# circletile/smvp-toolkit

Measured on AMD Instinct MI355X. Metric: fp64 CSR SpMV GFLOP/s (2*nnz flop per product; achieved HBM GB/s in roofline), higher is better.
Workload: dtype f64; 1 GPU; memplus.mtx x944 block-diagonal (substitute for the SURVEY 8(d) random model; that model: roofline.frac_sur...; format=csr, kernel=csr_stream_owner<8, 5, false>, nnz=119085600, rows=16763552, exchange=none

## Files before the change

include/smvp_amd.h:

```cpp
#ifndef SMVP_AMD_H
#define SMVP_AMD_H

#include <stddef.h>
#include <stdint.h>
#include <stdio.h>

#ifdef __cplusplus
extern "C" {
#endif

#define SMVP_VERSION_MAJOR 0
#define SMVP_VERSION_MINOR 6
#define SMVP_VERSION_REVISION 4

enum {
    SMVP_OK = 0,
    SMVP_ERR_INVALID = 1,
    SMVP_ERR_NO_DEVICE = 2,
    SMVP_ERR_HIP = 3,
    SMVP_ERR_ALLOC = 4,
    SMVP_ERR_IO = 5,
    SMVP_ERR_UNSUPPORTED = 6,
    SMVP_MM_COULD_NOT_READ_FILE = 11,
    SMVP_MM_PREMATURE_EOF = 12,
    SMVP_MM_NOT_MTX = 13,
    SMVP_MM_NO_HEADER = 14,
    SMVP_MM_UNSUPPORTED_TYPE = 15,
    SMVP_MM_LINE_TOO_LONG = 16,
    SMVP_MM_COULD_NOT_WRITE_FILE = 17
};
const char *smvp_last_error(void);
const char *smvp_version_string(void);
int smvp_set_option(const char *name, int value);
int smvp_get_option(const char *name, int *value);

typedef struct smvp_coo {
    int row;
    int col;
    double val;
} smvp_coo_t;

typedef char smvp_mm_typecode[4];

typedef struct smvp_time_stats {
    double time_total, time_avg, time_stdev, time_min, time_max;
} smvp_time_stats_t;

int smvp_mm_read_banner(FILE *f, smvp_mm_typecode *matcode);
int smvp_mm_read_mtx_crd_size(FILE *f, int *rows, int *cols, int *nnz);
int smvp_mm_read_coo_entries(FILE *f, const smvp_mm_typecode matcode, int nnz, smvp_coo_t *out);
int smvp_mm_read_header_path(const char *path, smvp_mm_typecode *matcode, int *rows, int *cols, int *nnz);
int smvp_mm_read_coo_path(const char *path, smvp_coo_t *out, int capacity,
                          smvp_mm_typecode *matcode, int *rows, int *cols, int *nnz);

int smvp_mm_expanded_count(const smvp_mm_typecode matcode, const smvp_coo_t *coo, int nnz, int *count);
int smvp_mm_expand_symmetric(const smvp_mm_typecode matcode, const smvp_coo_t *coo, int nnz, int rows, int cols,
                             smvp_coo_t *out, int capacity, int *nnz_out);

int smvp_cache_write_csr(const char *cache_path, const char *mtx_path, const smvp_mm_typecode matcode, int flags,
                         int rows, int cols, int nnz, const int *row_ptr, const int *col_ind, const double *val);
int smvp_cache_read_header(const char *cache_path, const char *mtx_path, smvp_mm_typecode *matcode, int *flags,
                           int *rows, int *cols, int *nnz);
int smvp_cache_read_csr(const char *cache_path, int rows, int nnz, int *row_ptr, int *col_ind, double *val);
int smvp_coo_from_csr(int rows, const int *row_ptr, const int *col_ind, const double *val, smvp_coo_t *out);

int smvp_csr_from_coo(const smvp_coo_t *coo, int rows, int nnz,
                      int *row_ptr, int *col_ind, double *val);
int smvp_tjds_from_coo(const smvp_coo_t *coo, int rows, int cols, int nnz,
                       int *perm, int *start_pos, int start_pos_capacity,
                       int *row_ind, double *val,
                       int *num_diag, int *ref_num_tjdiag, int *last_diag_single);

int smvp_csr_from_coo_device(const smvp_coo_t *d_coo, int rows, int cols, int nnz,
                             int *d_row_ptr, int *d_col_ind, double *d_val, void *stream);
int smvp_tjds_from_coo_device(const smvp_coo_t *d_coo, int rows, int cols, int nnz,
                              int *d_perm, int *d_start_pos, int start_pos_capacity,
                              int *d_row_ind, double *d_val,
                              int *num_diag, int *ref_num_tjdiag, int *last_diag_single, void *stream);

int smvp_device_count(int *count);
int smvp_device_info(int device, char *name, size_t name_cap, int *compute_units,
                     size_t *hbm_bytes);

enum {
    SMVP_CSR_KERNEL_AUTO = 0,
    SMVP_CSR_KERNEL_VECTOR = 1,
    SMVP_CSR_KERNEL_STREAM = 2,
    SMVP_CSR_KERNEL_STREAM_CARRY = 3,
    SMVP_CSR_KERNEL_COLSWEEP = 4,
    SMVP_CSR_KERNEL_BINNED = 5
};
enum {
    SMVP_MEM_HOST = 0,
    SMVP_MEM_DEVICE = 1
};

typedef struct smvp_csr smvp_csr_t;
typedef struct smvp_tjds smvp_tjds_t;

int smvp_csr_create(smvp_csr_t **out, int device, int rows, int cols, int nnz,
                    const int *row_ptr, const int *col_ind, const double *val,
                    int mem_kind, const int *host_row_ptr);
int smvp_csr_create_block(smvp_csr_t **out, int device, int rows, int cols, int nnz,
                          const int *row_ptr, const int *col_ind, const double *val,
                          int mem_kind, const int *host_row_ptr, long long first_row);
int smvp_csr_set_kernel(smvp_csr_t *h, int kernel, int param);
int smvp_csr_get_kernel(const smvp_csr_t *h, int *kernel, int *param);
int smvp_csr_gather_spread(smvp_csr_t *h, double *spread);
int smvp_csr_far_share(smvp_csr_t *h, double *share);
int smvp_csr_spmv(smvp_csr_t *h, const double *d_x, double *d_y, void *stream);
int smvp_csr_describe(const smvp_csr_t *h, char *kernel_name, size_t cap, double *alg_bytes);
int smvp_csr_plan_launches(const smvp_csr_t *h, int *launches);
typedef struct smvp_plan_info {
    double matrix_bytes;
    double plan_bytes;
    double build_ms;
} smvp_plan_info_t;
int smvp_csr_plan_info(const smvp_csr_t *h, smvp_plan_info_t *out);
int smvp_csr_spmm(smvp_csr_t *h, int k, const double *d_X, long long ldx, double *d_Y, long long ldy, void *stream);
int smvp_csr_spmm_describe(const smvp_csr_t *h, int k, char *kernel_name, size_t cap, double *alg_bytes, smvp_plan_info_t *plan);
int smvp_csr_create_transposed(smvp_csr_t **out, const smvp_csr_t *h, void *stream);
int smvp_csr_device_arrays(const smvp_csr_t *h, const int **d_row_ptr, const int **d_col_ind, const double **d_val);
void smvp_csr_destroy(smvp_csr_t *h);

int smvp_tjds_create(smvp_tjds_t **out, int device, int rows, int cols, int nnz, int num_diag,
                     const int *perm, const int *start_pos, const int *row_ind,
                     const double *val, int mem_kind);
int smvp_tjds_set_x(smvp_tjds_t *h, const double *d_x, void *stream);
int smvp_tjds_zero_y(smvp_tjds_t *h, double *d_y, void *stream);
int smvp_tjds_spmv(smvp_tjds_t *h, double *d_y, void *stream);
enum {
    SMVP_TJDS_MODE_AUTO = 0,
    SMVP_TJDS_MODE_ATOMIC = 1,
    SMVP_TJDS_MODE_TWO_PHASE = 2,
    SMVP_TJDS_MODE_ROW_GATHER = 3
};
int smvp_tjds_set_mode(smvp_tjds_t *h, int mode);
int smvp_tjds_set_tile(smvp_tjds_t *h, int entries_per_tile);
int smvp_tjds_set_value_cache(smvp_tjds_t *h, int min_tiles);
int smvp_tjds_get_value_cache(const smvp_tjds_t *h, int *min_tiles, long long *cached_entries);
int smvp_tjds_set_ref_quirks(smvp_tjds_t *h, int enable, int ref_num_tjdiag, int last_diag_single);
int smvp_tjds_describe(const smvp_tjds_t *h, char *kernel_name, size_t cap, double *alg_bytes);
int smvp_tjds_plan_info(const smvp_tjds_t *h, smvp_plan_info_t *out);
int smvp_tjds_spmv_transposed(smvp_tjds_t *h, const double *d_x, double *d_y, void *stream);
int smvp_tjds_transposed_describe(const smvp_tjds_t *h, char *kernel_name, size_t cap, double *alg_bytes);
int smvp_tjds_spmm_transposed(smvp_tjds_t *h, int k, const double *d_X, long long ldx, double *d_Y, long long ldy, void *stream);
int smvp_tjds_spmm_transposed_describe(const smvp_tjds_t *h, int k, char *kernel_name, size_t cap, double *alg_bytes);
int smvp_tjds_spmm(smvp_tjds_t *h, int k, const double *d_X, long long ldx, double *d_Y, long long ldy, void *stream);
int smvp_tjds_spmm_describe(const smvp_tjds_t *h, int k, char *kernel_name, size_t cap, double *alg_bytes, smvp_plan_info_t *plan);
void smvp_tjds_destroy(smvp_tjds_t *h);

enum { SMVP_POWER_CONVERGED = 0, SMVP_POWER_MAX_STEPS = 1, SMVP_POWER_ZERO = 2, SMVP_POWER_NONFINITE = 3 };
typedef struct smvp_power_opts {
    unsigned struct_size;
    int max_steps;
    int check_every;
    double tol;
} smvp_power_opts_t;
void smvp_power_opts_default(smvp_power_opts_t *o);
typedef struct smvp_power_result {
    int steps;
    int reason;
    int index;
    double eigenvalue;
    double residual;
    double scale;
} smvp_power_result_t;
int smvp_csr_power_method(smvp_csr_t *h, const smvp_power_opts_t *opts, const double *d_x0, double *d_x,
                          smvp_power_result_t *result, double *lambda_each, double *residual_each, void *stream);
int smvp_tjds_power_method(smvp_tjds_t *h, const smvp_power_opts_t *opts, const double *d_x0, double *d_x,
                           smvp_power_result_t *result, double *lambda_each, double *residual_each, void *stream);

int smvp_vector_dot(int device, int n, const double *d_a, const double *d_b, double *result, void *stream);

enum { SMVP_CG_CONVERGED = 0, SMVP_CG_MAX_STEPS = 1, SMVP_CG_BREAKDOWN = 2, SMVP_CG_NONFINITE = 3 };
typedef struct smvp_cg_opts {
    unsigned struct_size;
    int max_steps;
    int check_every;
    double tol;
} smvp_cg_opts_t;
void smvp_cg_opts_default(smvp_cg_opts_t *o);
typedef struct smvp_cg_result {
    int steps;
    int updates;
    int reason;
    int pad;
    double rr;
    double bb;
} smvp_cg_result_t;
int smvp_csr_cg(smvp_csr_t *h, const smvp_cg_opts_t *opts, const double *d_b, const double *d_x0, double *d_x,
                smvp_cg_result_t *result, double *rr_each, double *sigma_each, void *stream);
int smvp_tjds_cg(smvp_tjds_t *h, const smvp_cg_opts_t *opts, const double *d_b, const double *d_x0, double *d_x,
                 smvp_cg_result_t *result, double *rr_each, double *sigma_each, void *stream);

int smvp_csr_diagonal(const smvp_csr_t *h, double *d_diag, void *stream);
int smvp_tjds_diagonal(const smvp_tjds_t *h, double *d_diag, void *stream);

typedef struct smvp_pcg_result {
    int steps;
    int updates;
    int reason;
    int pad;
    double rr;
    double rz;
    double bb;
} smvp_pcg_result_t;
int smvp_csr_pcg(smvp_csr_t *h, const smvp_cg_opts_t *opts, const double *d_b, const double *d_x0, double *d_x, const double *d_m,
                 smvp_pcg_result_t *result, double *rr_each, double *rz_each, double *sigma_each, void *stream);
int smvp_tjds_pcg(smvp_tjds_t *h, const smvp_cg_opts_t *opts, const double *d_b, const double *d_x0, double *d_x, const double *d_m,
                  smvp_pcg_result_t *result, double *rr_each, double *rz_each, double *sigma_each, void *stream);

int smvp_csr_cg_multi(smvp_csr_t *h, const smvp_cg_opts_t *opts, int k, const double *d_B, long long ldb, const double *d_X0,
                      long long ldx0, double *d_X, long long ldx, const double *d_m, smvp_pcg_result_t *results, double *rr_each,
                      double *rz_each, double *sigma_each, void *stream);
int smvp_tjds_cg_multi(smvp_tjds_t *h, const smvp_cg_opts_t *opts, int k, const double *d_B, long long ldb, const double *d_X0,
                       long long ldx0, double *d_X, long long ldx, const double *d_m, smvp_pcg_result_t *results, double *rr_each,
                       double *rz_each, double *sigma_each, void *stream);

enum { SMVP_TRSV_LOWER = 0, SMVP_TRSV_UPPER = 1 };
enum { SMVP_TRSV_DIAG_STORED = 0, SMVP_TRSV_DIAG_UNIT = 1 };
typedef struct smvp_trsv smvp_trsv_t;
typedef struct smvp_trsv_info {
    unsigned struct_size;
    int levels;
    int max_level_width;
    int launches;
    int chains;
    int chain_width;
    int missing_diagonals;
    int lanes_per_row;
    long long entries;
    double plan_bytes;
    double build_ms;
} smvp_trsv_info_t;
int smvp_csr_trsv_create(smvp_trsv_t **out, const smvp_csr_t *h, int uplo, int diag, void *stream);
int smvp_trsv_solve(smvp_trsv_t *t, const double *d_b, double *d_x, void *stream);
int smvp_trsv_info(const smvp_trsv_t *t, smvp_trsv_info_t *out);
int smvp_trsv_schedule(const smvp_trsv_t *t, int *level_ptr, int *order);
void smvp_trsv_destroy(smvp_trsv_t *t);
int smvp_csr_trsv_levels(int rows, const int *row_ptr, const int *col_ind, int uplo, int *level_of_row, int *levels);

enum { SMVP_TRSV_MAX_SWEEPS = 4096 };
// ... 207 lines not shown
```

smvp-toolkit_amd/csrc/smvp_common.h:

```cpp
#pragma once
#include "smvp_amd.h"

#include <cstdarg>
#include <cstdio>
#include <vector>

namespace smvp {
constexpr long long kMaxEntries = 2147483647ll - 65536;

int fail(int code, const char *fmt, ...) __attribute__((format(printf, 2, 3)));
void clear_error();
int option(const char *name, int fallback);

struct TrsvSchedule {
    std::vector<int> level_of_row, level_ptr, order;
    int levels = 0, max_level_width = 0, missing_diagonals = 0, max_row_entries = 0;
    long long off_entries = 0, diag_entries = 0;
};
struct TrsvLaunch {
    int first, last;
    bool chain;
};
int trsv_analyse(int rows, const int *row_ptr, const int *col_ind, int uplo, TrsvSchedule *out);
void trsv_launches(const std::vector<int> &level_ptr, int chain_width, std::vector<TrsvLaunch> *out, int *chains);
void trsv_ranges(int rows, const int *row_ptr, const int *col_ind, int uplo, int diag, std::vector<int> *begin, std::vector<int> *end,
                 long long *entries, int *longest);

int ilu0_check(const char *fn, int rows, const int *row_ptr, const int *col_ind, int *diag_pos, int *bad_row);

int lsqr_check_args(const char *fn, const void *h, const void *ht, bool needs_ht, const smvp_lsqr_opts_t *opts, const void *result,
                    const double *d_b);
}

struct ihipStream_t;
namespace smvp {
int build_row_inverse(const int *d_row_ind, int nnz, int rows, int *d_inv_ptr, int *d_inv_pos, ihipStream_t *stream);
int build_row_gather_plan(const int *d_row_ind, const int *d_start_pos, int num_diag, int nnz, int rows,
                          int *d_seg_ptr, int *d_pos, int *d_kcol, ihipStream_t *stream);
int build_colsweep_plan(const int *d_row_ptr, const int *d_col_ind, const double *d_val, int rows, int cols, int nnz, int strip_rows,
                        int parts, int chunk, int row_bits, int turn_cap, long long *d_strip_ptr, int *d_e_col, double *d_e_val,
                        unsigned short *d_e_row, ihipStream_t *stream);
int sort_tile_windows(const int *d_pos, int nnz, int tile, const int *d_start_pos, int num_diag, int slot_bits,
                      const double *d_val, int cache_min_tiles, int *d_pos_sorted, int *d_meta, int *d_cache_ptr,
                      double **d_val_cache, int *cached_total, ihipStream_t *stream);
int build_tile_half_streams(const int *d_pos, int nnz, int tile, const int *d_start_pos, int num_diag, const double *d_val,
                            int cache_min_tiles, unsigned *d_word32, int *d_cache_ptr, int *d_run_ptr,
                            double **d_val_cache, int **d_run_tab, unsigned short **d_group_run, int *cached_total,
                            int *runs_total, ihipStream_t *stream);
int build_column_offsets(const int *d_col_ind, int nnz, int tile, int *d_col_base, unsigned short *d_col16, int *fits,
                         ihipStream_t *stream);
int build_tile_overflow(const int *d_pos, const int *d_ovf_ptr, int total, int ntiles, int tile, int nnz,
                        const int *d_start_pos, int num_diag, const double *d_val, double *d_ovf_val, int *d_ovf_k, int positions,
                        ihipStream_t *stream);
}
```

smvp-toolkit_amd/csrc/smvp_convert_device.hip:

```cpp
#include "smvp_common.h"
#include "smvp_prim.h"
#include "smvp_tile_map.h"

#include <hip/hip_runtime.h>

#include <cstring>

#include <algorithm>
#include <vector>

#define HIP_TRY(expr)                                                                       \
    do {                                                                                    \
        hipError_t e_ = (expr);                                                             \
        if (e_ != hipSuccess)                                                               \
            return smvp::fail(SMVP_ERR_HIP, "%s failed: %s", #expr, hipGetErrorString(e_)); \
    } while (0)

namespace {

typedef unsigned long long u64;

struct Scratch {
    std::vector<void *> ptrs;
    ~Scratch()
// ... 800 lines not shown
                                                   unsigned short *__restrict__ e_row)
{
    const int i = blockIdx.x * 256 + threadIdx.x;
    if (i >= nnz)
        return;
    const long long a = strip_ptr[(unsigned)(key[i] >> 32) * (unsigned)parts + (unsigned)(key[i] & 0xffffffffu) / part_width];
    const long long first = a + ((long long)i - a) / chunk * chunk;
    const unsigned short mine = row_sorted[i];
    int turn = 0;
    for (long long q = first; q < i; ++q)
        turn += row_sorted[q] == mine ? 1 : 0;
    e_row[i] = (unsigned short)(mine | ((turn < turn_cap ? turn : turn_cap) << row_bits));
}

__global__ __launch_bounds__(256) void sweep_strip_bounds(const int *__restrict__ row_ptr, int rows, int strip_rows, int nstrips,
                                                          long long *__restrict__ strip_ptr)
{
    const int b = blockIdx.x * 256 + threadIdx.x;
    if (b > nstrips)
        return;
    const long long r = (long long)b * strip_rows;
    strip_ptr[b] = row_ptr[r < rows ? r : rows];
}

__global__ __launch_bounds__(256) void sweep_part_bounds(const u64 *__restrict__ key, const int *__restrict__ row_ptr, int rows, int nnz,
                                                         int strip_rows, int nstrips, int parts, unsigned part_width,
                                                         long long *__restrict__ stream_ptr)
{
    const int v = blockIdx.x * 256 + threadIdx.x;
    if (v > nstrips * parts)
        return;
    if (v == nstrips * parts) {
        stream_ptr[v] = nnz;
        return;
    }
    const int strip = v / parts, part = v % parts;
    const long long r0 = (long long)strip * strip_rows, r1 = r0 + strip_rows;
    long long lo = row_ptr[r0 < rows ? r0 : rows], hi = row_ptr[r1 < rows ? r1 : rows];
    const unsigned first_col = (unsigned)part * part_width;
    while (lo < hi) {
        const long long mid = (lo + hi) >> 1;
        if ((unsigned)(key[mid] & 0xffffffffu) < first_col)
            lo = mid + 1;
        else
            hi = mid;
    }
    stream_ptr[v] = lo;
}

}

namespace smvp {

int build_colsweep_plan(const int *d_row_ptr, const int *d_col_ind, const double *d_val, int rows, int cols, int nnz, int strip_rows,
                        int parts, int chunk, int row_bits, int turn_cap, long long *d_strip_ptr, int *d_e_col, double *d_e_val,
                        unsigned short *d_e_row, hipStream_t st)
{
    if (strip_rows < 1 || strip_rows > (1 << row_bits) || row_bits < 1 || row_bits > 15 || chunk < 64 ||
        turn_cap != (1 << (16 - row_bits)) - 1 || (parts != 1 && parts != 2 && parts != 4 && parts != 8))
        return smvp::fail(SMVP_ERR_INVALID, "build_colsweep_plan: bad strip shape");
    const unsigned part_width = (unsigned)std::max(1, (int)(((long long)std::max(cols, 1) + parts - 1) / parts));
    const int nstrips = (rows + strip_rows - 1) / strip_rows;
    hipLaunchKernelGGL(sweep_strip_bounds, dim3(blocks_for((long long)nstrips + 1)), dim3(256), 0, st, d_row_ptr, rows,
                       strip_rows, nstrips, d_strip_ptr);
    HIP_TRY(hipGetLastError());
    if (nnz > 0) {
        Scratch sc;
        u64 *k0, *k1;
        unsigned *i0, *i1;
        unsigned short *lr, *lr_sorted;
        HIP_TRY(sc.get(&k0, (size_t)nnz));
        HIP_TRY(sc.get(&k1, (size_t)nnz));
        HIP_TRY(sc.get(&i0, (size_t)nnz));
        HIP_TRY(sc.get(&i1, (size_t)nnz));
        HIP_TRY(sc.get(&lr, (size_t)nnz));
        HIP_TRY(sc.get(&lr_sorted, (size_t)nnz));
        hipLaunchKernelGGL(sweep_keys, dim3(blocks_for(nnz)), dim3(256), 0, st, d_row_ptr, d_col_ind, rows, nnz, strip_rows, k0, i0, lr);
        HIP_TRY(hipGetLastError());
        const unsigned bits = 32u + (unsigned)bits_for(nstrips + 1);
        size_t tmp_bytes = 0;
        HIP_TRY(smvp::prim::radix_sort_pairs(nullptr, tmp_bytes, k0, k1, i0, i1, (size_t)nnz, 0u, bits, st));
        char *tmp;
        HIP_TRY(sc.get(&tmp, tmp_bytes));
        HIP_TRY(smvp::prim::radix_sort_pairs(tmp, tmp_bytes, k0, k1, i0, i1, (size_t)nnz, 0u, bits, st));
        hipLaunchKernelGGL(sweep_gather, dim3(blocks_for(nnz)), dim3(256), 0, st, k1, i1, d_val, lr, nnz, d_e_col, d_e_val, lr_sorted);
        HIP_TRY(hipGetLastError());
        if (parts > 1) {
            hipLaunchKernelGGL(sweep_part_bounds, dim3(blocks_for((long long)nstrips * parts + 1)), dim3(256), 0, st, k1, d_row_ptr, rows, nnz,
                               strip_rows, nstrips, parts, part_width, d_strip_ptr);
            HIP_TRY(hipGetLastError());
        }
        hipLaunchKernelGGL(sweep_turns, dim3(blocks_for(nnz)), dim3(256), 0, st, k1, d_strip_ptr, lr_sorted, nnz, chunk, row_bits,
                           turn_cap, parts, part_width, d_e_row);
        HIP_TRY(hipGetLastError());
        HIP_TRY(hipStreamSynchronize(st));
    } else if (parts > 1) {
        HIP_TRY(hipMemsetAsync(d_strip_ptr, 0, sizeof(long long) * ((size_t)nstrips * parts + 1), st));
    }
    HIP_TRY(hipStreamSynchronize(st));
    return SMVP_OK;
}

}

namespace {

__global__ __launch_bounds__(256) void tile_column_spans(const int *__restrict__ col_ind, int nnz, int tile,
                                                         int *__restrict__ col_base, int *__restrict__ narrow)
{
    __shared__ int lo_s[4], hi_s[4];
    const long long s = (long long)blockIdx.x * tile;
    int lo = 0x7fffffff, hi = -1;
    for (int i = threadIdx.x; i < tile && s + i < nnz; i += 256) {
        const int c = col_ind[s + i];
        lo = c < lo ? c : lo;
        hi = c > hi ? c : hi;
    }
#pragma unroll
    for (int off = 32; off > 0; off >>= 1) {
        const int ol = __shfl_down(lo, off, 64), oh = __shfl_down(hi, off, 64);
        lo = ol < lo ? ol : lo;
        hi = oh > hi ? oh : hi;
    }
    if ((threadIdx.x & 63) == 0) {
        lo_s[threadIdx.x >> 6] = lo;
        hi_s[threadIdx.x >> 6] = hi;
    }
    __syncthreads();
    if (threadIdx.x == 0) {
        for (int w = 1; w < 4; ++w) {
            lo = lo_s[w] < lo ? lo_s[w] : lo;
            hi = hi_s[w] > hi ? hi_s[w] : hi;
        }
        const bool fits = hi < 0 || hi - lo < 65536;
        col_base[blockIdx.x] = !fits ? -1 : (hi < 0 ? 0 : lo);
        if (fits)
            atomicAdd(narrow, 1);
    }
}

__global__ __launch_bounds__(256) void column_offsets(const int *__restrict__ col_ind, int nnz, int tile,
                                                      const int *__restrict__ col_base, unsigned short *__restrict__ col16)
{
    const int j = blockIdx.x * 256 + threadIdx.x;
    if (j < nnz) {
        const int b = j / tile, s = b * tile;
        const int base = col_base[b];
        const bool lane_order = tile == smvp::kCol16LaneOrderTile && base >= 0 && (long long)s + tile <= (long long)nnz;
        const int at = lane_order ? s + smvp::col16_slot(j - s, tile / 256) : j;
        col16[at] = base < 0 ? (unsigned short)0 : (unsigned short)(col_ind[j] - base);
    }
}

}

namespace smvp {

int build_column_offsets(const int *d_col_ind, int nnz, int tile, int *d_col_base, unsigned short *d_col16, int *fits,
                         hipStream_t st)
{
    *fits = 0;
    if (nnz <= 0)
        return SMVP_OK;
    const int ntiles = (int)(((long long)nnz + tile - 1) / tile);
    Scratch sc;
    int *narrow;
    HIP_TRY(sc.get(&narrow, 1));
    HIP_TRY(hipMemsetAsync(narrow, 0, sizeof(int), st));
    hipLaunchKernelGGL(tile_column_spans, dim3((unsigned)ntiles), dim3(256), 0, st, d_col_ind, nnz, tile, d_col_base, narrow);
    HIP_TRY(hipGetLastError());
    int h_narrow = 0;
    HIP_TRY(hipMemcpyAsync(&h_narrow, narrow, sizeof(int), hipMemcpyDeviceToHost, st));
    HIP_TRY(hipStreamSynchronize(st));
    if (2 * (long long)h_narrow < (long long)ntiles)
        return SMVP_OK;
    hipLaunchKernelGGL(column_offsets, dim3(blocks_for(nnz)), dim3(256), 0, st, d_col_ind, nnz, tile, d_col_base, d_col16);
    HIP_TRY(hipGetLastError());
    HIP_TRY(hipStreamSynchronize(st));
    *fits = 1;
    return SMVP_OK;
}

}
```

smvp-toolkit_amd/csrc/smvp_engine.hip:

```cpp
#include "smvp_engine.h"

#include <cmath>
#include <cstring>

using smvp::check_block_operands;
using smvp::check_device_indices;
using smvp::DeviceScope;
using smvp::kMaxEntries;
using smvp::refuse_capture;
using smvp::TjdsSource;
using smvp::to_device;
using smvp::upload;
using smvp::usable_device;
using smvp::wall_ms;

int smvp::usable_device(int device)
{
    int n = 0;
    if (hipGetDeviceCount(&n) != hipSuccess || n <= 0)
        return smvp::fail(SMVP_ERR_NO_DEVICE, "no HIP device is visible (this engine has no CPU path)");
    if (device < 0 || device >= n)
        return smvp::fail(SMVP_ERR_INVALID, "device %d out of range (%d visible)", device, n);
    return SMVP_OK;
}


struct TilePlan {
    int ntiles = 0;
    int *d_tile_row = nullptr;
    int *d_tile_next = nullptr;
    unsigned short *d_col16 = nullptr;
    int *d_col_base = nullptr;
    int col16_tile = 0;
    unsigned short *d_row_rel = nullptr;
    int *d_carry_row = nullptr;
    double *d_carry = nullptr;
    int *d_pos_sorted = nullptr, *d_meta = nullptr, *d_ovf_ptr = nullptr, *d_ovf_k = nullptr;
    double *d_ovf_val = nullptr;
    int *d_cache_ptr = nullptr;
    double *d_val_cache = nullptr;
    int cached_total = 0, ovf_total = 0;
    unsigned short *d_group_run = nullptr;
    unsigned *d_word32 = nullptr;
    int *d_run_ptr = nullptr, *d_run_tab = nullptr;
    int runs_total = 0;
    int sweep_alternate = 1, sweep_backward = 0;
    int read_once = 0;
};

struct SweepPlan {
    int rb = 0, per_launch = 0;
    int parts = 1;
    int g = 0;
    long long *d_ptr = nullptr;
    int *d_col = nullptr;
    double *d_val = nullptr;
    unsigned short *d_row = nullptr;
    double *d_part = nullptr;
};

struct BinnedSide {
    smvp::BinnedPlan bin;
    smvp_csr *near = nullptr;
    hipStream_t side = nullptr;
    hipEvent_t ev_fork = nullptr, ev_join = nullptr;
};

struct SpmmPlan {
    int *d_order = nullptr;
    bool planned = false;
    double build_ms = 0.0;
};

struct smvp_csr {
    int device = 0;
    int rows = 0, cols = 0, nnz = 0;
    long long row0 = 0;
    int *d_row_ptr = nullptr;
    int *d_col_ind = nullptr;
    double *d_val = nullptr;
    bool own_row_ptr = false, own_col_ind = false, own_val = false;
    std::vector<int> h_row_ptr;
    int max_row_len = 0;

    int flavor = smvp::kFlavorCsr;
    TjdsSource src;
    int cache_min_tiles = 2;
    bool plain_only = false;

    int kernel = SMVP_CSR_KERNEL_AUTO;
    int lanes_per_row = 64;
    int vpt = 4;
    bool tile_chosen = false;
    double spread = -2.0;
    double far_share = -2.0;
    double plan_build_ms = 0.0;

    TilePlan tile;
    SweepPlan sweep;
    BinnedSide binned;
    SpmmPlan spmm;
};

namespace {

void free_tile_plan(TilePlan *p)
{
    for (void *q : {(void *)p->d_tile_row, (void *)p->d_tile_next, (void *)p->d_col16, (void *)p->d_col_base, (void *)p->d_row_rel,
                    (void *)p->d_carry_row, (void *)p->d_carry, (void *)p->d_pos_sorted, (void *)p->d_meta, (void *)p->d_ovf_ptr,
                    (void *)p->d_ovf_k, (void *)p->d_ovf_val, (void *)p->d_cache_ptr, (void *)p->d_val_cache, (void *)p->d_group_run,
                    (void *)p->d_word32, (void *)p->d_run_ptr, (void *)p->d_run_tab})
        if (q)
            (void)hipFree(q);
    *p = TilePlan{};
}

void free_sweep_plan(SweepPlan *p)
{
    for (void *q : {(void *)p->d_ptr, (void *)p->d_col, (void *)p->d_val, (void *)p->d_row, (void *)p->d_part})
        if (q)
            (void)hipFree(q);
    *p = SweepPlan{};
}

void free_binned_side(BinnedSide *p)
{
    smvp_csr_destroy(p->near);
    smvp::free_binned_plan(&p->bin);
    if (p->side)
        (void)hipStreamDestroy(p->side);
    for (hipEvent_t e : {p->ev_fork, p->ev_join})
        if (e)
            (void)hipEventDestroy(e);
    *p = BinnedSide{};
}

void free_spmm_plan(SpmmPlan *p)
{
    if (p->d_order)
        (void)hipFree(p->d_order);
    *p = SpmmPlan{};
}

inline bool tile_ordered(int flavor) { return flavor == smvp::kFlavorTjdsS || flavor == smvp::kFlavorTjdsH; }
inline bool runs_on_tile_plan(int k) { return k != SMVP_CSR_KERNEL_VECTOR && k != SMVP_CSR_KERNEL_COLSWEEP && k != SMVP_CSR_KERNEL_BINNED; }
inline int owner_flavor(const smvp_csr *h) { return h->tile.d_col16 ? smvp::kFlavorCsr16 : h->flavor; }
inline double csr_matrix_bytes(const smvp_csr *h) { return 12.0 * h->nnz + 4.0 * (h->rows + 1.0); }
inline int sweep_strip_rows(const SweepPlan &s) { return (s.parts == smvp::kSweepXcdParts ? s.rb : s.rb * s.parts) / smvp::kSweepWaves; }

constexpr int kSweepMaxRb = 20480;
double sweep_rate(int rb)
{
    const struct { double lg, rate; } pts[] = {{10.0, 0.70}, {11.0, 0.80}, {12.0, 0.86}, {13.0, 1.0}, {14.32, 1.10}};
    constexpr int N = (int)(sizeof pts / sizeof pts[0]);
    const double lg = std::log2((double)std::max(rb, 1));
    if (lg <= pts[0].lg)
        return pts[0].rate * std::max(0.25, lg / pts[0].lg);
    for (int i = 0; i + 1 < N; ++i)
        if (lg <= pts[i + 1].lg)
            return pts[i].rate + (pts[i + 1].rate - pts[i].rate) * (lg - pts[i].lg) / (pts[i + 1].lg - pts[i].lg);
    return pts[N - 1].rate;
}

void choose_sweep_shape(int rows, int cols, int nnz, int want_rb, int *rb, int *per_launch)
{
    const double mean = rows > 0 ? std::max(1.0, (double)nnz / rows) : 1.0;
    int floor_rb = 1024;
    while (floor_rb < 8192 && (double)floor_rb * mean * 160.0 < (double)cols)
        floor_rb <<= 1;
    auto generations = [](int nrb) { return (nrb + 255) / 256; };
    std::vector<int> heights;
    for (int hgt : {kSweepMaxRb, 16384, 8192, 4096, 2048, 1024})
        if (hgt >= floor_rb)
            heights.push_back(hgt);
    for (int g = 1; g <= 16 && rows > 0; ++g) {
        const long long want = ((long long)rows + 256ll * g - 1) / (256ll * g);
        const int h4 = (int)std::min<long long>(kSweepMaxRb, (want + 3) / 4 * 4);
        if (h4 >= std::max(1024, floor_rb / 2))
            heights.push_back(h4);
    }
    int r = floor_rb;
    double best = -1.0;
    int best_gen = 1 << 30;
    for (int hgt : heights) {
        const int nrb = (rows + hgt - 1) / hgt;
        const int gen = std::max(1, generations(nrb));
        const double score = (double)nrb / (gen * 256.0) * sweep_rate(hgt);
        if (score > best * 1.01 || (score > best * 0.99 && gen < best_gen)) {
            best = std::max(best, score);
            best_gen = gen;
            r = hgt;
        }
    }
    if (want_rb > 0)
        r = want_rb;
    const int nrb = (rows + r - 1) / r;
    const int gen = std::max(1, generations(nrb));
    *rb = r;
    *per_launch = std::max(1, (nrb + gen - 1) / gen);
}

constexpr int kSweepPartsShift = 24, kSweepChunksShift = 26;
inline int sweep_param_rb(int param) { return param & ((1 << kSweepPartsShift) - 1); }
inline int sweep_param_parts(int param) { return 1 << ((param >> kSweepPartsShift) & 3); }
inline int sweep_param_chunks(int param) { const int c = (param >> kSweepChunksShift) & 3; return c == 3 ? 4 : c; }
bool sweep_param_ok(int param)
{
    const int rb = sweep_param_rb(param), parts = sweep_param_parts(param);
    if (param < 0 || (param >> (kSweepChunksShift + 2)) != 0)
        return false;
    if (rb == 0)
        return true;
    if (parts == smvp::kSweepXcdParts)
        return rb >= 256 && rb % 4 == 0 && rb <= kSweepMaxRb;
    return rb >= 256 && rb % 4 == 0 && (long long)rb * parts <= kSweepMaxRb;
}

int build_sweep_plan(smvp_csr *h, int want)
{
    SweepPlan &s = h->sweep;
    free_sweep_plan(&s);
    const int want_rb = sweep_param_rb(want);
    s.parts = sweep_param_parts(want);
    const bool xcd = s.parts == smvp::kSweepXcdParts;
    if (xcd) {
        int rb = want_rb;
        if (rb == 0) {
            const long long per_gen_max = 32ll * kSweepMaxRb;
            const long long gens = std::max<long long>(1, ((long long)h->rows + per_gen_max - 1) / per_gen_max);
            rb = (int)std::min<long long>(kSweepMaxRb, std::max<long long>(256, (((long long)h->rows + 32 * gens - 1) / (32 * gens) + 3) / 4 * 4));
        }
        s.rb = rb;
        s.per_launch = 256;
    } else {
        choose_sweep_shape(h->rows, h->cols, h->nnz, want_rb, &s.rb, &s.per_launch);
        while (s.parts > 1 && (long long)s.rb * s.parts > kSweepMaxRb)
            s.parts >>= 1;
    }
    const int strip_rows = sweep_strip_rows(s);
    s.g = smvp::sweep_chunks_in_flight(strip_rows, sweep_param_chunks(want));
    if (const hipError_t pe = smvp::prepare_csr_colsweep(); pe != hipSuccess)
        return smvp::fail(SMVP_ERR_HIP, "the column sweep cannot have its LDS: %s", hipGetErrorString(pe));
    const int nstrips = (h->rows + strip_rows - 1) / strip_rows;
    const size_t n = (size_t)std::max(h->nnz, 4);
    if (hipMalloc((void **)&s.d_ptr, ((size_t)nstrips * s.parts + 2) * sizeof(long long)) != hipSuccess ||
        hipMalloc((void **)&s.d_col, n * sizeof(int)) != hipSuccess ||
        hipMalloc((void **)&s.d_val, n * sizeof(double)) != hipSuccess ||
        hipMalloc((void **)&s.d_row, n * sizeof(unsigned short)) != hipSuccess ||
        (xcd && hipMalloc((void **)&s.d_part, sizeof(double) * smvp::kSweepXcdParts * (size_t)std::max(h->rows, 1)) != hipSuccess))
        return smvp::fail(SMVP_ERR_ALLOC, "cannot allocate the column-sweep plan (%d entries)", h->nnz);
    return smvp::build_colsweep_plan(h->d_row_ptr, h->d_col_ind, h->d_val, h->rows, h->cols, h->nnz, strip_rows, s.parts, smvp::kSweepChunk,
                                     smvp::kSweepRowBits, smvp::kSweepTurnCap, s.d_ptr, s.d_col, s.d_val, s.d_row, nullptr);
}

constexpr int kSpreadSamples = 64;
double csr_gather_spread(const smvp_csr *h)
{
    if ((long long)h->nnz < (long long)kSpreadSamples * smvp::kSpreadSpan || !h->d_col_ind)
        return -1.0;
    int *d_bits = nullptr;
    if (hipMalloc((void **)&d_bits, sizeof(int) * kSpreadSamples) != hipSuccess)
        return -1.0;
    int bits[kSpreadSamples];
    hipError_t e = smvp::launch_csr_line_spread(h->d_col_ind, h->nnz, kSpreadSamples, d_bits, nullptr);
    if (e == hipSuccess)
        e = hipMemcpy(bits, d_bits, sizeof bits, hipMemcpyDeviceToHost);
    (void)hipFree(d_bits);
    if (e != hipSuccess) {
        (void)hipGetLastError();
        return -1.0;
    }
    const double m = 512.0 * 1024.0;
    double lines = 0.0;
    for (int b : bits)
        lines += -m * std::log(std::max(1.0 - b / m, 1.0 / m));
    return std::min(1.0, lines / ((double)kSpreadSamples * smvp::kSpreadSpan));
}

constexpr double kSweepMinSpread = 0.6;

double measured_spread(smvp_csr *h)
{
    if (h->spread < -1.5)
        h->spread = h->flavor == smvp::kFlavorCsr ? csr_gather_spread(h) : -1.0;
    return h->spread;
}

double measured_far_share(smvp_csr *h)
{
    if (h->far_share < -1.5) {
        double share = -1.0;
        if (h->flavor != smvp::kFlavorCsr ||
            smvp::csr_far_share(h->d_row_ptr, h->d_col_ind, h->rows, h->nnz, smvp::kBinNearBand, h->row0, &share, nullptr) != SMVP_OK) {
            (void)hipGetLastError();
            share = -1.0;
        }
        h->far_share = share;
    }
    return h->far_share;
}

bool sweep_suits(smvp_csr *h)
{
    if (h->plain_only || h->flavor != smvp::kFlavorCsr || h->nnz < 4 * 1024 * 1024 || h->rows < 4096)
        return false;
    const double mean = (double)h->nnz / h->rows;
    if (mean < 4.0 || (double)h->cols * 8.0 < 8.0 * 1024 * 1024 || 8192.0 * mean * 160.0 < (double)h->cols ||
        (double)h->max_row_len > 256.0 * mean)
        return false;
    return measured_spread(h) >= kSweepMinSpread;
}

constexpr double kBinnedMinSpread = 0.2, kBinnedMinFarShare = 0.1;
bool binned_suits(smvp_csr *h)
{
    if (h->plain_only || h->flavor != smvp::kFlavorCsr || h->nnz < 4 * 1024 * 1024 || h->rows < 4096 ||
        (double)h->cols * 8.0 < 16.0 * 1024 * 1024)
        return false;
    return measured_spread(h) >= kBinnedMinSpread && measured_far_share(h) >= kBinnedMinFarShare;
}

int try_column_offsets(smvp_csr *h)
{
    if (h->flavor != smvp::kFlavorCsr || h->kernel != SMVP_CSR_KERNEL_STREAM || h->vpt < 4 || h->nnz <= 0 ||
        smvp::option("csr_col16", 1) == 0)
        return SMVP_OK;
    std::vector<int> tiles;
    if (!h->tile_chosen && h->nnz >= 12 * 1024 * 1024)
        tiles.push_back(2048);
    tiles.push_back(smvp::kStreamBlock * h->vpt);
    const size_t max_tiles = ((size_t)h->nnz + 1023) / 1024 + 1;
    int *col_base = nullptr;
    unsigned short *col16 = nullptr;
    int rc = SMVP_OK;
    if (hipMalloc((void **)&col_base, max_tiles * sizeof(int)) != hipSuccess ||
        hipMalloc((void **)&col16, ((size_t)h->nnz + 8) * sizeof(unsigned short)) != hipSuccess)
        rc = smvp::fail(SMVP_ERR_ALLOC, "cannot allocate the 16-bit column offsets (%d entries)", h->nnz);
    for (size_t i = 0; i < tiles.size() && rc == SMVP_OK; ++i) {
        int fits = 0;
        rc = smvp::build_column_offsets(h->d_col_ind, h->nnz, tiles[i], col_base, col16, &fits, nullptr);
        if (rc == SMVP_OK && fits) {
            h->vpt = tiles[i] / smvp::kStreamBlock;
            h->tile.d_col_base = col_base;
            h->tile.d_col16 = col16;
            h->tile.col16_tile = tiles[i];
            return SMVP_OK;
        }
    }
    (void)hipGetLastError();
    for (void *p : {(void *)col16, (void *)col_base})
        if (p)
            (void)hipFree(p);
    return rc;
}

constexpr double kSweepAlternateMinBytes = 256.0 * 1024 * 1024;

constexpr double kReadOnceMinBytes = 1024.0 * 1024 * 1024;

int build_tile_plan_parts(smvp_csr *h)
{
    TilePlan &t = h->tile;
    free_tile_plan(&t);
    if (int rc = try_column_offsets(h))
        return rc;
    const int tile = smvp::kStreamBlock * h->vpt;
    const long long nnz = h->nnz;
    const int ntiles = (int)std::max<long long>(1, (nnz + tile - 1) / tile);
    std::vector<int> tile_row((size_t)ntiles + 1), carry_row((size_t)ntiles), tile_next((size_t)ntiles);
    const int *rp = h->h_row_ptr.data();
    int r = 0;
    for (int b = 0; b < ntiles; ++b) {
        const long long s = (long long)b * tile;
        const long long e = std::min(s + tile, nnz);
        while (r < h->rows && rp[r] < s)
            ++r;
        tile_row[(size_t)b] = r;
        const long long first = r < h->rows ? rp[r] : nnz;
        carry_row[(size_t)b] = (std::min(first, e) > s) ? r - 1 : -1;
    }
    tile_row[(size_t)ntiles] = h->rows;
    for (int b = 0; b < ntiles; ++b)
        tile_next[(size_t)b] = rp[tile_row[(size_t)b + 1]];
    if (int rc = upload(&t.d_tile_row, tile_row))
        return rc;
    if (h->kernel == SMVP_CSR_KERNEL_STREAM) {
        if (int rc = upload(&t.d_tile_next, tile_next))
            return rc;
        if (h->rows > 0 && smvp::option("csr_rowrel", 1) != 0) {
            std::vector<unsigned short> rel((size_t)h->rows);
            for (int b = 0; b < ntiles; ++b) {
                const long long s0 = (long long)b * tile;
                for (int rr = tile_row[(size_t)b]; rr < tile_row[(size_t)b + 1]; ++rr)
                    rel[(size_t)rr] = (unsigned short)(rp[rr] - s0);
            }
            if (int rc = upload(&t.d_row_rel, rel))
                return rc;
        }
    } else {
        if (int rc = upload(&t.d_carry_row, carry_row))
            return rc;
        HIP_TRY(hipMalloc((void **)&t.d_carry, std::max(ntiles, 1) * sizeof(double)));
        HIP_TRY(hipMemset(t.d_carry, 0, std::max(ntiles, 1) * sizeof(double)));
    }
    t.ntiles = ntiles;
    const int alternate = smvp::option("csr_sweep_alternate", -1);
    const double product_bytes = 12.0 * (double)h->nnz + 12.0 * h->rows + 8.0 * h->cols;
    t.sweep_alternate = alternate < 0 ? product_bytes > kSweepAlternateMinBytes : alternate != 0;
    const int read_once = smvp::option("csr_read_once", -1);
    t.read_once = h->flavor != smvp::kFlavorCsr ? 0 : read_once < 0 ? product_bytes > kReadOnceMinBytes : read_once != 0;
    if (tile_ordered(h->flavor)) {
        std::vector<int> ovf_ptr((size_t)ntiles + 1, 0);
        for (int b = 0; b < ntiles; ++b) {
            const long long e = std::min((long long)(b + 1) * tile, nnz);
            const bool owns = tile_row[(size_t)b] != tile_row[(size_t)b + 1];
            ovf_ptr[(size_t)b + 1] = ovf_ptr[(size_t)b] + (owns ? (int)(tile_next[(size_t)b] - e) : 0);
        }
        const int total = ovf_ptr[(size_t)ntiles];
        t.ovf_total = total;
        if (int rc = upload(&t.d_ovf_ptr, ovf_ptr))
            return rc;
        const size_t n = (size_t)std::max(h->nnz, 4), m = (size_t)std::max(total, 4);
        const bool half = h->flavor == smvp::kFlavorTjdsH;
        const TjdsSource &src = h->src;
        if (hipMalloc((void **)&t.d_ovf_val, m * sizeof(double)) != hipSuccess ||
            hipMalloc((void **)&t.d_ovf_k, m * sizeof(int)) != hipSuccess ||
            hipMalloc((void **)&t.d_cache_ptr, ((size_t)ntiles + 2) * sizeof(int)) != hipSuccess ||
            hipMalloc(half ? (void **)&t.d_word32 : (void **)&t.d_pos_sorted, n * sizeof(int)) != hipSuccess ||
            hipMalloc(half ? (void **)&t.d_run_ptr : (void **)&t.d_meta, (half ? (size_t)ntiles + 2 : n) * sizeof(int)) != hipSuccess)
            return smvp::fail(SMVP_ERR_ALLOC, "cannot allocate the tile-ordered TJDS streams");
        if (int rc = half ? smvp::build_tile_half_streams(src.pos, h->nnz, tile, src.start_pos, src.num_diag, h->d_val, h->cache_min_tiles,
                                                          t.d_word32, t.d_cache_ptr, t.d_run_ptr, &t.d_val_cache, &t.d_run_tab,
                                                          &t.d_group_run, &t.cached_total, &t.runs_total, nullptr)
                          : smvp::sort_tile_windows(src.pos, h->nnz, tile, src.start_pos, src.num_diag, smvp::kSlotBits, h->d_val,
                                                    h->cache_min_tiles, t.d_pos_sorted, t.d_meta, t.d_cache_ptr, &t.d_val_cache,
                                                    &t.cached_total, nullptr))
            return rc;
        if (int rc = smvp::build_tile_overflow(src.pos, t.d_ovf_ptr, total, ntiles, tile, h->nnz, src.start_pos, src.num_diag, h->d_val,
                                               t.d_ovf_val, t.d_ovf_k, src.unit_operand ? 1 : 0, nullptr))
            return rc;
    }
    return SMVP_OK;
}

int build_tile_plan(smvp_csr *h)
{
    const int rc = build_tile_plan_parts(h);
    if (rc != SMVP_OK)
        free_tile_plan(&h->tile);
    return rc;
}

int pow2_at_least(double v)
{
    int p = 2;
    while (p < 64 && p < v)
        p <<= 1;
    return p;
}

constexpr int kOwnerMaxRow = 16 * 1024;

bool choose_csr_kernel(smvp_csr *h, int kernel, int param)
{
    const double mean = h->rows > 0 ? (double)h->nnz / h->rows : 0.0;
    if (kernel == SMVP_CSR_KERNEL_AUTO)
        kernel = h->max_row_len > kOwnerMaxRow ? SMVP_CSR_KERNEL_STREAM_CARRY
                 : sweep_suits(h)              ? SMVP_CSR_KERNEL_COLSWEEP
                 : binned_suits(h)             ? SMVP_CSR_KERNEL_BINNED
                                               : SMVP_CSR_KERNEL_STREAM;
    if (kernel == SMVP_CSR_KERNEL_STREAM && param != 0 && param != 256 && param != 1024 && param != 2048)
        return false;
    if (kernel == SMVP_CSR_KERNEL_STREAM_CARRY && param != 0 && param != 1024 && param != 2048)
        return false;
    if (kernel == SMVP_CSR_KERNEL_COLSWEEP && !sweep_param_ok(param))
        return false;
    if (kernel == SMVP_CSR_KERNEL_BINNED && param < 0)
        return false;
    h->kernel = kernel;
    if (kernel == SMVP_CSR_KERNEL_COLSWEEP || kernel == SMVP_CSR_KERNEL_BINNED)
        return true;
    if (kernel == SMVP_CSR_KERNEL_VECTOR) {
        h->lanes_per_row = param > 0 ? param : pow2_at_least(mean);
    } else {
        int tile = param > 0 ? param : 0;
        h->tile_chosen = param > 0;
        if (tile == 0) {
            tile = (kernel == SMVP_CSR_KERNEL_STREAM && h->nnz < 512 * 1024) ? 256 : 1024;
            if ((tile_ordered(h->flavor)) && tile == 1024 && h->nnz >= 12 * 1024 * 1024)
                tile = 2048;
        }
        h->vpt = tile / smvp::kStreamBlock;
    }
    return true;
}

}

static int csr_create_impl(smvp_csr_t **out, int device, int rows, int cols, int nnz, const int *row_ptr, const int *col_ind, const double *val,
                           int mem_kind, const int *host_row_ptr, int flavor, const TjdsSource *src = nullptr, bool plain_only = false,
                           long long first_row = 0);

static int build_binned(smvp_csr *h, int band)
{
    free_binned_side(&h->binned);
    if (hipError_t le = smvp::binned_reserve_lds(); le != hipSuccess) {
        (void)hipGetLastError();
        return smvp::fail(SMVP_ERR_UNSUPPORTED, "the binned plan needs 154 KB of LDS per workgroup: %s", hipGetErrorString(le));
    }
    const bool window = smvp::option("binned_near", 0) == 0;
    if (int rc = smvp::build_binned_plan(h->d_row_ptr, h->d_col_ind, h->d_val, h->rows, h->cols, h->nnz, band, h->row0, window, &h->binned.bin, nullptr))
        return rc;
    if (h->binned.bin.nw.on) {
        if (smvp::option("binned_overlap", 1) != 0 && h->binned.bin.nf > 0) {
            HIP_TRY(hipStreamCreateWithFlags(&h->binned.side, hipStreamNonBlocking));
            HIP_TRY(hipEventCreateWithFlags(&h->binned.ev_fork, hipEventDisableTiming));
            HIP_TRY(hipEventCreateWithFlags(&h->binned.ev_join, hipEventDisableTiming));
        }
        return SMVP_OK;
    }
    return csr_create_impl(&h->binned.near, h->device, h->rows, h->cols, h->binned.bin.nnz_near, h->binned.bin.near_ptr, h->binned.bin.near_col, h->binned.bin.near_val,
                           SMVP_MEM_DEVICE, nullptr, smvp::kFlavorCsr, nullptr, true, h->row0);
}

static int plan_csr(smvp_csr *h, int kernel, int param, bool silent_fallback)
{
    if (!choose_csr_kernel(h, kernel, param))
        return smvp::fail(SMVP_ERR_INVALID, "entries per tile must be 256 (stream only), 1024 or 2048 for the kernel "
                                            "this matrix resolves to (column sweep: 256 ... 20480 rows per block, a multiple of 4; binned: the near band, >= 0)");
    const double t0 = wall_ms();
    free_sweep_plan(&h->sweep);
    free_binned_side(&h->binned);
    int rc = SMVP_OK;
    if (runs_on_tile_plan(h->kernel)) {
        rc = build_tile_plan(h);
    } else {
        free_tile_plan(&h->tile);
        if (h->kernel != SMVP_CSR_KERNEL_VECTOR)
            rc = h->kernel == SMVP_CSR_KERNEL_COLSWEEP ? build_sweep_plan(h, param) : build_binned(h, param);
        if (rc != SMVP_OK) {
            const std::string why = smvp_last_error();
            (void)hipGetLastError();
            free_sweep_plan(&h->sweep);
            free_binned_side(&h->binned);
            h->spread = -1.0;
            choose_csr_kernel(h, SMVP_CSR_KERNEL_STREAM, 0);
            const int tile_rc = build_tile_plan(h);
            rc = silent_fallback ? tile_rc : smvp::fail(rc, "%s", why.c_str());
        }
    }
    h->plan_build_ms = wall_ms() - t0;
    return rc;
}

static int csr_create_impl(smvp_csr_t **out, int device, int rows, int cols, int nnz, const int *row_ptr, const int *col_ind, const double *val,
                           int mem_kind, const int *host_row_ptr, int flavor, const TjdsSource *src, bool plain_only, long long first_row)
{
    const bool plain = flavor == smvp::kFlavorCsr;
    if (!out || rows < 0 || cols < 0 || nnz < 0 || !row_ptr ||
        (nnz > 0 && ((!col_ind && !tile_ordered(flavor)) || !val)))
        return smvp::fail(SMVP_ERR_INVALID, "smvp_csr_create: bad argument");
    if (mem_kind != SMVP_MEM_HOST && mem_kind != SMVP_MEM_DEVICE)
        return smvp::fail(SMVP_ERR_INVALID, "smvp_csr_create: bad mem_kind");
    if (nnz > kMaxEntries)
        return smvp::fail(SMVP_ERR_UNSUPPORTED, "smvp_csr_create: %d entries: shard blocks this large by rows", nnz);
    if (int rc = usable_device(device))
        return rc;
    DeviceScope on(device);

    smvp_csr *h = new smvp_csr;
    h->device = device;
    h->flavor = flavor;
    h->plain_only = plain_only;
    h->row0 = first_row;
    if (src)
        h->src = *src;
    if (h->src.unit_operand)
        h->cache_min_tiles = 0;
    h->rows = rows, h->cols = cols, h->nnz = nnz;
    h->h_row_ptr.resize((size_t)rows + 1);
    int rc = SMVP_OK;
    if (mem_kind == SMVP_MEM_HOST || host_row_ptr) {
        memcpy(h->h_row_ptr.data(), mem_kind == SMVP_MEM_HOST ? row_ptr : host_row_ptr, sizeof(int) * ((size_t)rows + 1));
    } else if (hipMemcpy(h->h_row_ptr.data(), row_ptr, sizeof(int) * ((size_t)rows + 1), hipMemcpyDeviceToHost) != hipSuccess) {
        rc = smvp::fail(SMVP_ERR_HIP, "smvp_csr_create: cannot read row_ptr back from the device");
    }
    if (rc == SMVP_OK) {
        const std::vector<int> &rp = h->h_row_ptr;
        bool ok = rp[0] == 0 && rp[(size_t)rows] == nnz;
        for (int r = 0; r < rows && ok; ++r) {
            ok = rp[(size_t)r] <= rp[(size_t)r + 1];
            h->max_row_len = std::max(h->max_row_len, rp[(size_t)r + 1] - rp[(size_t)r]);
        }
        if (!ok)
            rc = smvp::fail(SMVP_ERR_INVALID, "smvp_csr_create: row_ptr is not a non-decreasing 0..nnz sequence");
    }
    if (rc == SMVP_OK && mem_kind == SMVP_MEM_HOST) {
        for (int j = 0; j < nnz; ++j)
            if (col_ind[j] < 0 || col_ind[j] >= cols) {
                rc = smvp::fail(SMVP_ERR_INVALID, "smvp_csr_create: col_ind[%d] = %d outside [0, %d)", j, col_ind[j], cols);
                break;
            }
    }
    if (rc == SMVP_OK && mem_kind == SMVP_MEM_DEVICE &&
        (((uintptr_t)col_ind | (plain ? (uintptr_t)val : 0)) & 15u) != 0)
        rc = smvp::fail(SMVP_ERR_INVALID, "smvp_csr_create: adopted device arrays must be 16-byte aligned");
    if (rc == SMVP_OK && mem_kind == SMVP_MEM_DEVICE && col_ind)
        rc = check_device_indices(col_ind, nnz, cols, "smvp_csr_create: col_ind");
    if (rc == SMVP_OK)
        rc = to_device(&h->d_row_ptr, row_ptr, (size_t)rows + 1, mem_kind, &h->own_row_ptr);
    if (rc == SMVP_OK && col_ind)
        rc = to_device(&h->d_col_ind, col_ind, (size_t)nnz, mem_kind, &h->own_col_ind);
    if (rc == SMVP_OK)
        rc = to_device(&h->d_val, val, (size_t)nnz, mem_kind, &h->own_val);
    if (rc == SMVP_OK) {
        const double t0 = wall_ms();
        rc = plan_csr(h, plain ? SMVP_CSR_KERNEL_AUTO : SMVP_CSR_KERNEL_STREAM, 0, true);
        h->plan_build_ms = wall_ms() - t0;
    }
    if (rc != SMVP_OK) {
        smvp_csr_destroy(h);
        return rc;
    }
    *out = h;
    return SMVP_OK;
}

int smvp::csr_create_tjds(smvp_csr_t **out, int device, int rows, int cols, int nnz, const int *d_row_ptr, const int *d_col_ind,
                          const double *d_val, int flavor, const TjdsSource &src)
{
    return csr_create_impl(out, device, rows, cols, nnz, d_row_ptr, d_col_ind, d_val, SMVP_MEM_DEVICE, nullptr, flavor, &src);
}

bool smvp::csr_value_cache(const smvp_csr_t *h, int *min_tiles, long long *cached_entries)
{
    const bool on = h && tile_ordered(h->flavor);
    if (min_tiles)
        *min_tiles = on ? h->cache_min_tiles : 0;
    if (cached_entries)
        *cached_entries = on ? h->tile.cached_total : 0;
    return on;
}

int smvp::csr_replan_value_cache(smvp_csr_t *h, int min_tiles)
{
    h->cache_min_tiles = min_tiles;
    return build_tile_plan(h);
}

extern "C" int smvp_csr_create(smvp_csr_t **out, int device, int rows, int cols, int nnz,
                               const int *row_ptr, const int *col_ind, const double *val,
                               int mem_kind, const int *host_row_ptr)
{
    return csr_create_impl(out, device, rows, cols, nnz, row_ptr, col_ind, val, mem_kind, host_row_ptr, smvp::kFlavorCsr);
}

extern "C" int smvp_csr_create_block(smvp_csr_t **out, int device, int rows, int cols, int nnz,
                                     const int *row_ptr, const int *col_ind, const double *val,
                                     int mem_kind, const int *host_row_ptr, long long first_row)
{
    if (first_row < 0)
        return smvp::fail(SMVP_ERR_INVALID, "smvp_csr_create_block: first_row < 0");
    return csr_create_impl(out, device, rows, cols, nnz, row_ptr, col_ind, val, mem_kind, host_row_ptr, smvp::kFlavorCsr, nullptr,
                           false, first_row);
}

extern "C" int smvp_csr_far_share(smvp_csr_t *h, double *share)
{
    if (!h || !share)
        return smvp::fail(SMVP_ERR_INVALID, "smvp_csr_far_share: bad argument");
    DeviceScope on(h->device);
    *share = measured_far_share(h);
    return SMVP_OK;
}

extern "C" int smvp_csr_set_kernel(smvp_csr_t *h, int kernel, int param)
{
    if (!h)
        return smvp::fail(SMVP_ERR_INVALID, "null handle");
    if (h->flavor != smvp::kFlavorCsr && kernel != SMVP_CSR_KERNEL_STREAM)
        return smvp::fail(SMVP_ERR_UNSUPPORTED, "this matrix flavour runs on the stream kernel only");
    if (kernel < SMVP_CSR_KERNEL_AUTO || kernel > SMVP_CSR_KERNEL_BINNED)
        return smvp::fail(SMVP_ERR_INVALID, "unknown CSR kernel %d", kernel);
    if (kernel == SMVP_CSR_KERNEL_VECTOR && param != 0 &&
        (param < 2 || param > 64 || (param & (param - 1)) != 0))
        return smvp::fail(SMVP_ERR_INVALID, "lanes per row must be a power of two in [2, 64]");
    DeviceScope on(h->device);
    h->spread = h->far_share = -2.0;
    return plan_csr(h, kernel, param, false);
}

extern "C" int smvp_csr_get_kernel(const smvp_csr_t *h, int *kernel, int *param)
{
    if (!h)
        return smvp::fail(SMVP_ERR_INVALID, "null handle");
    if (kernel)
        *kernel = h->kernel;
    if (param)
        *param = h->kernel == SMVP_CSR_KERNEL_VECTOR ? h->lanes_per_row
                 : h->kernel == SMVP_CSR_KERNEL_COLSWEEP ? (h->sweep.rb | ((h->sweep.parts == 8 ? 3 : h->sweep.parts == 4 ? 2 : h->sweep.parts == 2 ? 1 : 0) << kSweepPartsShift))
                 : h->kernel == SMVP_CSR_KERNEL_BINNED   ? h->binned.bin.band
                                                         : h->vpt * smvp::kStreamBlock;
    return SMVP_OK;
}

extern "C" int smvp_csr_gather_spread(smvp_csr_t *h, double *spread)
{
    if (!h || !spread)
        return smvp::fail(SMVP_ERR_INVALID, "smvp_csr_gather_spread: bad argument");
    DeviceScope on(h->device);
    *spread = measured_spread(h);
    return SMVP_OK;
}

static int fill_owner_launch(const smvp_csr_t *h, const double *d_x, double *d_y, unsigned long long *stamps, smvp::OwnerLaunch *out)
{
    if (h->tile.d_col16 && h->tile.col16_tile != smvp::kStreamBlock * h->vpt)
        return smvp::fail(SMVP_ERR_INVALID, "the 16-bit column offsets were laid out for %d-entry tiles, the launch has %d-entry tiles",
                          h->tile.col16_tile, smvp::kStreamBlock * h->vpt);
    smvp::OwnerLaunch &l = *out;
    l.row_ptr = h->d_row_ptr, l.col_ind = h->d_col_ind, l.val = h->d_val, l.x = d_x, l.y = d_y;
    l.tile_row = h->tile.d_tile_row, l.tile_next = h->tile.d_tile_next;
    l.pos = h->src.pos, l.start_pos = h->src.start_pos;
    if (tile_ordered(h->flavor)) {
        l.pos = h->tile.d_pos_sorted, l.col_ind = h->tile.d_meta;
        l.ovf_ptr = h->tile.d_ovf_ptr, l.ovf_val = h->tile.d_ovf_val, l.ovf_k = h->tile.d_ovf_k;
        l.cache_ptr = h->tile.d_cache_ptr, l.val_cache = h->tile.d_val_cache;
        l.word32 = h->tile.d_word32, l.group_run = h->tile.d_group_run, l.run_ptr = h->tile.d_run_ptr, l.run_tab = h->tile.d_run_tab;
    }
    l.stamps = stamps;
    l.rows = h->rows, l.nnz = h->nnz, l.ntiles = h->tile.ntiles;
    l.col16 = h->tile.d_col16, l.col_base = h->tile.d_col_base;
    l.row_rel = h->tile.d_row_rel;
    l.read_once = h->tile.read_once;
    l.unit_x = h->src.unit_operand ? 1 : 0;
    return SMVP_OK;
}

int smvp::csr_repeat_grid(const smvp_csr_t *h)
{
    if (!h || h->kernel != SMVP_CSR_KERNEL_STREAM || !h->tile.d_tile_row || h->rows <= 0)
        return 0;
    DeviceScope on(h->device);
    return smvp::owner_repeat_grid(h->vpt, owner_flavor(h), h->tile.ntiles);
}

int smvp::csr_spmv_repeat(smvp_csr_t *h, const double *d_x, double *d_y, void *stream, unsigned long long *stamps, int reps, int grid,
                          unsigned *ctl_words, bool first_of_run, unsigned long long patience)
{
    DeviceScope on(h->device);
    smvp::OwnerLaunch l{};
    if (int rc = fill_owner_launch(h, d_x, d_y, stamps, &l))
        return rc;
    const hipError_t e = smvp::launch_csr_stream_owner_repeat(h->vpt, owner_flavor(h), l, reps, grid, ctl_words,
                                                              first_of_run, patience, (hipStream_t)stream);
    if (e != hipSuccess)
        return smvp::fail(SMVP_ERR_HIP, "repeating CSR launch failed: %s", hipGetErrorString(e));
    return SMVP_OK;
}

static int launched(hipError_t e)
{
    return e == hipSuccess ? (int)SMVP_OK : smvp::fail(SMVP_ERR_HIP, "CSR launch failed: %s", hipGetErrorString(e));
}

int smvp::csr_spmv_stamped(smvp_csr_t *h, const double *d_x, double *d_y, void *stream, unsigned long long *stamps)
{
    if (!h || (h->rows > 0 && !d_y) || (h->nnz > 0 && !d_x))
        return smvp::fail(SMVP_ERR_INVALID, "smvp_csr_spmv: bad argument");
    if ((h->kernel == SMVP_CSR_KERNEL_COLSWEEP && !h->sweep.d_ptr) || (h->kernel == SMVP_CSR_KERNEL_BINNED && !h->binned.near && !h->binned.bin.nw.on) ||
        (runs_on_tile_plan(h->kernel) && !h->tile.d_tile_row))
        return smvp::fail(SMVP_ERR_INVALID, "smvp_csr_spmv: the handle has no launch plan (a re-plan failed earlier)");
    DeviceScope on(h->device);
    hipStream_t st = (hipStream_t)stream;
    hipError_t e;
    if (h->kernel == SMVP_CSR_KERNEL_BINNED) {
        if (h->binned.bin.nw.on && h->binned.side) {
            HIP_TRY(hipEventRecord(h->binned.ev_fork, st));
            HIP_TRY(hipStreamWaitEvent(h->binned.side, h->binned.ev_fork, 0));
            if (int rc = launched(smvp::launch_binned_products(h->binned.bin, d_x, h->binned.side)))
                return rc;
            int rc = SMVP_OK;
            hipError_t je = hipEventRecord(h->binned.ev_join, h->binned.side);
            if (je == hipSuccess) {
                rc = launched(smvp::launch_near_window(h->binned.bin.nw, d_x, d_y, st));
                je = hipStreamWaitEvent(st, h->binned.ev_join, 0);
            }
            if (je != hipSuccess) {
                (void)hipStreamSynchronize(h->binned.side);
                return smvp::fail(SMVP_ERR_HIP, "joining the binned plan's side stream failed: %s", hipGetErrorString(je));
            }
            if (rc != SMVP_OK)
                return rc;
            return launched(smvp::launch_binned_sums(h->binned.bin, d_y, st));
        }
        if (h->binned.bin.nw.on) {
            if (int rc = launched(smvp::launch_near_window(h->binned.bin.nw, d_x, d_y, st)))
                return rc;
        } else if (int rc = smvp::csr_spmv_stamped(h->binned.near, d_x, d_y, stream, nullptr))
            return rc;
        if (int rc = launched(smvp::launch_binned_products(h->binned.bin, d_x, st)))
            return rc;
        e = smvp::launch_binned_sums(h->binned.bin, d_y, st);
    } else if (h->kernel == SMVP_CSR_KERNEL_COLSWEEP)
        e = smvp::launch_csr_colsweep(h->sweep.d_ptr, h->sweep.d_col, h->sweep.d_val, h->sweep.d_row, d_x, d_y, h->rows,
                                      sweep_strip_rows(h->sweep), h->sweep.parts, h->sweep.per_launch, h->sweep.g, h->sweep.d_part, st);
    else if (h->kernel == SMVP_CSR_KERNEL_VECTOR)
        e = smvp::launch_csr_vector(h->lanes_per_row, h->d_row_ptr, h->d_col_ind, h->d_val, d_x, d_y, h->rows, st);
    else if (h->kernel == SMVP_CSR_KERNEL_STREAM) {
        smvp::OwnerLaunch l{};
        if (int rc = fill_owner_launch(h, d_x, d_y, stamps, &l))
            return rc;
        l.backward = h->tile.sweep_backward;
        h->tile.sweep_backward = h->tile.sweep_alternate ? !l.backward : 0;
        e = smvp::launch_csr_stream_owner(h->vpt, owner_flavor(h), l, st);
    } else
        e = smvp::launch_csr_stream(h->vpt, h->d_row_ptr, h->d_col_ind, h->d_val, d_x, d_y, h->tile.d_tile_row,
                                    h->tile.d_carry_row, h->tile.d_carry, h->rows, h->nnz, h->tile.ntiles, st);
    return launched(e);
}

extern "C" int smvp_csr_spmv(smvp_csr_t *h, const double *d_x, double *d_y, void *stream)
{
    return smvp::csr_spmv_stamped(h, d_x, d_y, stream, nullptr);
}

static smvp::HandleProduct csr_product(smvp_csr_t *h, void *stream)
{
    return [h, stream](const double *x, double *y) { return smvp_csr_spmv(h, x, y, stream); };
}

static int refuse_tjds_flavor(const char *fn, const smvp_csr_t *h)
{
    if (h->flavor != smvp::kFlavorCsr)
        return smvp::fail(SMVP_ERR_UNSUPPORTED, "%s: plain CSR handles only (this one belongs to a TJDS matrix)", fn);
    return SMVP_OK;
}

extern "C" int smvp_csr_power_method(smvp_csr_t *h, const smvp_power_opts_t *opts, const double *d_x0, double *d_x,
                                     smvp_power_result_t *result, double *lambda_each, double *residual_each, void *stream)
{
    if (int rc = smvp::power_check_args("smvp_csr_power_method", h, opts, result))
        return rc;
    if (int rc = refuse_tjds_flavor("smvp_csr_power_method", h))
        return rc;
    return smvp::power_run("smvp_csr_power_method", h->device, h->rows, h->cols, opts, d_x0, d_x, result, lambda_each, residual_each, stream,
                           csr_product(h, stream));
}

extern "C" int smvp_csr_cg(smvp_csr_t *h, const smvp_cg_opts_t *opts, const double *d_b, const double *d_x0, double *d_x,
                           smvp_cg_result_t *result, double *rr_each, double *sigma_each, void *stream)
{
    if (int rc = smvp::cg_check_args("smvp_csr_cg", h, opts, result, d_b, smvp::Precond::none, {}))
        return rc;
    if (int rc = refuse_tjds_flavor("smvp_csr_cg", h))
        return rc;
    return smvp::cg_run("smvp_csr_cg", h->device, h->rows, h->cols, opts, d_b, d_x0, d_x, result, rr_each, sigma_each, stream,
                        csr_product(h, stream));
}

extern "C" int smvp_csr_pcg(smvp_csr_t *h, const smvp_cg_opts_t *opts, const double *d_b, const double *d_x0, double *d_x,
                            const double *d_m, smvp_pcg_result_t *result, double *rr_each, double *rz_each, double *sigma_each,
                            void *stream)
{
    const smvp::KrylovPrecond M{nullptr, d_m, nullptr};
    if (int rc = smvp::cg_check_args("smvp_csr_pcg", h, opts, result, d_b, smvp::Precond::diagonal, M))
        return rc;
    if (int rc = refuse_tjds_flavor("smvp_csr_pcg", h))
        return rc;
    return smvp::cg_run("smvp_csr_pcg", h->device, h->rows, h->cols, opts, d_b, d_x0, d_x, smvp::Precond::diagonal, M, result, rr_each, rz_each,
                        sigma_each, stream, csr_product(h, stream));
}

extern "C" int smvp_csr_pcg_tri(smvp_csr_t *h, const smvp_cg_opts_t *opts, const double *d_b, const double *d_x0, double *d_x,
                                smvp_trsv_t *first, const double *d_m, smvp_trsv_t *second, smvp_pcg_result_t *result, double *rr_each,
                                double *rz_each, double *sigma_each, void *stream)
{
    const smvp::KrylovPrecond M{first, d_m, second};
    if (int rc = smvp::cg_check_args("smvp_csr_pcg_tri", h, opts, result, d_b, smvp::Precond::stored, M))
        return rc;
    if (int rc = refuse_tjds_flavor("smvp_csr_pcg_tri", h))
        return rc;
    return smvp::cg_run("smvp_csr_pcg_tri", h->device, h->rows, h->cols, opts, d_b, d_x0, d_x, smvp::Precond::stored, M, result, rr_each, rz_each,
                        sigma_each, stream, csr_product(h, stream));
}

extern "C" int smvp_csr_diagonal(const smvp_csr_t *h, double *d_diag, void *stream)
{
    if (!h || (h->rows > 0 && !d_diag))
        return smvp::fail(SMVP_ERR_INVALID, "smvp_csr_diagonal: null %s", !h ? "handle" : "d_diag");
    if (int rc = refuse_tjds_flavor("smvp_csr_diagonal", h))
        return rc;
    DeviceScope on(h->device);
    const hipError_t e = smvp::launch_csr_diagonal(pow2_at_least(h->rows > 0 ? (double)h->nnz / h->rows : 0.0), h->d_row_ptr, h->d_col_ind,
                                                   h->d_val, d_diag, h->rows, h->cols, h->row0, (hipStream_t)stream);
    if (e != hipSuccess)
        return smvp::fail(SMVP_ERR_HIP, "smvp_csr_diagonal: launch failed: %s", hipGetErrorString(e));
    return SMVP_OK;
}

smvp::CsrView smvp::csr_view(const smvp_csr_t *h)
{
    return {h->device, h->rows, h->cols, h->nnz, h->flavor, h->row0, h->d_row_ptr, h->d_col_ind, h->d_val, h->h_row_ptr.data()};
}

extern "C" int smvp_csr_bicgstab(smvp_csr_t *h, const smvp_bicgstab_opts_t *opts, const double *d_b, const double *d_x0, double *d_x,
                                 smvp_bicgstab_result_t *result, double *rr_each, double *ss_each, void *stream)
{
    if (int rc = smvp::bicgstab_check_args("smvp_csr_bicgstab", h, opts, result, d_b))
        return rc;
    if (int rc = refuse_tjds_flavor("smvp_csr_bicgstab", h))
        return rc;
    return smvp::bicgstab_run("smvp_csr_bicgstab", h->device, h->rows, h->cols, opts, d_b, d_x0, d_x, nullptr, result, rr_each, ss_each, stream,
                              csr_product(h, stream));
}

extern "C" int smvp_csr_pbicgstab(smvp_csr_t *h, const smvp_bicgstab_opts_t *opts, const double *d_b, const double *d_x0, double *d_x,
                                  smvp_trsv_t *first, const double *d_m, smvp_trsv_t *second, smvp_bicgstab_result_t *result,
                                  double *rr_each, double *ss_each, void *stream)
{
    const smvp::KrylovPrecond M{first, d_m, second};
    if (int rc = smvp::pbicgstab_check_args("smvp_csr_pbicgstab", h, opts, result, d_b, M))
        return rc;
    if (int rc = refuse_tjds_flavor("smvp_csr_pbicgstab", h))
        return rc;
    return smvp::bicgstab_run("smvp_csr_pbicgstab", h->device, h->rows, h->cols, opts, d_b, d_x0, d_x, &M, result, rr_each, ss_each, stream,
                              csr_product(h, stream));
}

extern "C" int smvp_csr_gmres(smvp_csr_t *h, const smvp_gmres_opts_t *opts, const double *d_b, const double *d_x0, double *d_x,
                              smvp_trsv_t *first, const double *d_m, smvp_trsv_t *second, smvp_gmres_result_t *result, double *rr_each,
                              double *restart_each, void *stream)
{
    if (int rc = smvp::gmres_check_args("smvp_csr_gmres", h, opts, result, d_b))
        return rc;
    if (int rc = refuse_tjds_flavor("smvp_csr_gmres", h))
        return rc;
    return smvp::gmres_run("smvp_csr_gmres", h->device, h->rows, h->cols, opts, d_b, d_x0, d_x, smvp::KrylovPrecond{first, d_m, second}, result,
                           rr_each, restart_each, stream, csr_product(h, stream));
}

extern "C" int smvp_csr_lsqr(smvp_csr_t *h, smvp_csr_t *ht, const smvp_lsqr_opts_t *opts, const double *d_b, const double *d_x0, double *d_x,
                             smvp_lsqr_result_t *result, double *rnorm_each, double *arnorm_each, void *stream)
{
    const char *fn = "smvp_csr_lsqr";
    if (int rc = smvp::lsqr_check_args(fn, h, ht, true, opts, result, d_b))
        return rc;
    for (const smvp_csr_t *a : {(const smvp_csr_t *)h, (const smvp_csr_t *)ht}) {
        if (int rc = refuse_tjds_flavor(fn, a))
            return rc;
        if (a->row0 != 0)
            return smvp::fail(SMVP_ERR_UNSUPPORTED, "%s: %s is a row block (first_row = %lld): whole matrices only", fn, a == h ? "h" : "ht", a->row0);
    }
    if (ht->rows != h->cols || ht->cols != h->rows || ht->nnz != h->nnz)
        return smvp::fail(SMVP_ERR_INVALID, "%s: ht is %d x %d with %d entries, the transpose of h (%d x %d, %d entries) is not", fn, ht->rows,
                          ht->cols, ht->nnz, h->rows, h->cols, h->nnz);
    if (ht->device != h->device)
        return smvp::fail(SMVP_ERR_INVALID, "%s: ht lives on device %d, h on device %d", fn, ht->device, h->device);
    return smvp::lsqr_run(fn, h->device, h->rows, h->cols, opts, d_b, d_x0, d_x, result, rnorm_each, arnorm_each, stream, csr_product(h, stream),
                          csr_product(ht, stream));
}

int smvp::csr_stamp_slots(const smvp_csr_t *h)
{
    return h && h->kernel == SMVP_CSR_KERNEL_STREAM && h->tile.d_tile_row ? smvp::owner_stamp_slots(h->tile.ntiles, h->flavor) : 0;
}

std::string smvp::csr_owner_kernel_name(const smvp_csr_t *h)
{
    char name[64];
    snprintf(name, sizeof name, "csr_stream_owner<%d, %d, false>", h ? h->vpt : 0, h ? owner_flavor(h) : 0);
    return name;
}

extern "C" int smvp_csr_describe(const smvp_csr_t *h, char *kernel_name, size_t cap, double *alg_bytes)
{
    if (!h)
        return smvp::fail(SMVP_ERR_INVALID, "null handle");
    if (kernel_name && cap) {
        if (h->kernel == SMVP_CSR_KERNEL_BINNED && h->binned.bin.nw.on)
            snprintf(kernel_name, cap, "csr_binned: csr_near_window + csr_binned_far_products<2> + csr_binned_far_sums<%d, %d, 2>", h->binned.bin.slots,
                     h->binned.bin.threads_b);
        else if (h->kernel == SMVP_CSR_KERNEL_BINNED)
            snprintf(kernel_name, cap, "csr_binned: %s + csr_binned_far_products<2> + csr_binned_far_sums<%d, %d, 2>",
                     smvp::csr_owner_kernel_name(h->binned.near).c_str(), h->binned.bin.slots, h->binned.bin.threads_b);
        else if (h->kernel == SMVP_CSR_KERNEL_COLSWEEP)
            if (h->sweep.parts == smvp::kSweepXcdParts)
                snprintf(kernel_name, cap, "csr_colsweep<%d> (8 column parts, one per XCD) + sweep_combine", h->sweep.g);
            else if (h->sweep.parts > 1)
                snprintf(kernel_name, cap, "csr_colsweep<%d> (%d column parts)", h->sweep.g, h->sweep.parts);
            else
                snprintf(kernel_name, cap, "csr_colsweep<%d>", h->sweep.g);
        else if (h->kernel == SMVP_CSR_KERNEL_VECTOR)
            snprintf(kernel_name, cap, "csr_vector_rows<%d>", h->lanes_per_row);
        else if (h->kernel == SMVP_CSR_KERNEL_STREAM)
            snprintf(kernel_name, cap, "%s", smvp::csr_owner_kernel_name(h).c_str());
        else
            snprintf(kernel_name, cap, "csr_stream_tiles<%d>", h->vpt);
    }
    if (alg_bytes)
        *alg_bytes = csr_matrix_bytes(h) + 8.0 * h->cols + 8.0 * h->rows;
    return SMVP_OK;
}

extern "C" int smvp_csr_plan_launches(const smvp_csr_t *h, int *launches)
{
    if (!h || !launches)
        return smvp::fail(SMVP_ERR_INVALID, "smvp_csr_plan_launches: bad argument");
    *launches = 1;
    if (h->kernel == SMVP_CSR_KERNEL_COLSWEEP && h->sweep.rb > 0 && h->sweep.per_launch > 0) {
        const bool xcd = h->sweep.parts == smvp::kSweepXcdParts;
        const int nwg = (h->rows + h->sweep.rb - 1) / h->sweep.rb * (xcd ? smvp::kSweepXcdParts : 1);
        *launches = std::max(1, (nwg + h->sweep.per_launch - 1) / h->sweep.per_launch) + (xcd ? 1 : 0);
    } else if (h->kernel == SMVP_CSR_KERNEL_STREAM_CARRY && h->tile.ntiles > 1) {
        *launches = 2;
    } else if (h->kernel == SMVP_CSR_KERNEL_BINNED && h->binned.bin.nw.on) {
        *launches = 1 + (h->binned.bin.nw.n_out > 0 ? 1 : 0) + (h->binned.bin.nf > 0 ? 2 : 0);
    } else if (h->kernel == SMVP_CSR_KERNEL_BINNED && h->binned.near) {
        int near = 1;
        (void)smvp_csr_plan_launches(h->binned.near, &near);
        *launches = near + (h->binned.bin.nf > 0 ? 2 : 0);
    }
    return SMVP_OK;
}

double smvp::csr_plan_bytes(const smvp_csr_t *h)
{
    const double n = h->nnz, t = h->tile.ntiles;
    if (h->kernel == SMVP_CSR_KERNEL_BINNED)
        return (double)h->binned.bin.plan_bytes + (h->binned.near ? smvp::csr_plan_bytes(h->binned.near) : 0.0);
    if (h->kernel == SMVP_CSR_KERNEL_COLSWEEP) {
        const bool xcd = h->sweep.parts == smvp::kSweepXcdParts;
        const int strip_rows = std::max(1, sweep_strip_rows(h->sweep));
        return 14.0 * n + 8.0 * ((double)((h->rows + strip_rows - 1) / strip_rows) * h->sweep.parts + 2) + (xcd ? 64.0 * h->rows : 0.0);
    }
    if (h->kernel == SMVP_CSR_KERNEL_VECTOR)
        return 0.0;
    double b = 4.0 * (t + 1) + 4.0 * t;
    if (h->kernel == SMVP_CSR_KERNEL_STREAM_CARRY)
        b += 8.0 * t;
    if (h->tile.d_col16)
        b += 2.0 * n + 4.0 * (n / 1024 + 1);
    if (h->tile.d_row_rel)
        b += 2.0 * h->rows;
    if (tile_ordered(h->flavor)) {
        b += 4.0 * (t + 1) + 12.0 * h->tile.ovf_total + 4.0 * (t + 2) + 8.0 * h->tile.cached_total;
        b += h->flavor == smvp::kFlavorTjdsH ? 4.0 * n + 4.0 * (t + 2) + 8.0 * h->tile.runs_total + 2.0 * (n / 32 + 1) : 8.0 * n;
    }
    return b;
}

extern "C" int smvp_csr_plan_info(const smvp_csr_t *h, smvp_plan_info_t *out)
{
    if (!h || !out)
        return smvp::fail(SMVP_ERR_INVALID, "smvp_csr_plan_info: bad argument");
    out->matrix_bytes = csr_matrix_bytes(h);
    out->plan_bytes = smvp::csr_plan_bytes(h);
    out->build_ms = h->plan_build_ms;
    return SMVP_OK;
}

static int csr_spmm_enqueue(smvp_csr_t *h, int k, const double *d_X, long long ldx, double *d_Y, long long ldy, hipStream_t st)
{
    if (!h->spmm.planned) {
        if (int rc = refuse_capture(st, "smvp_csr_spmm: the first call on a handle builds its plan and cannot be captured "
                                        "(call it once outside the capture)"))
            return rc;
        const double t0 = wall_ms();
        int *order = h->spmm.d_order;
        if (h->rows > 0 && !order && hipMalloc((void **)&order, sizeof(int) * (size_t)h->rows) != hipSuccess)
            return smvp::fail(SMVP_ERR_ALLOC, "smvp_csr_spmm: cannot allocate the plan (%d rows)", h->rows);
        h->spmm.d_order = order;
        if (int rc = smvp::build_spmm_order(h->d_row_ptr, h->rows, h->max_row_len, h->spmm.d_order, st))
            return rc;
        h->spmm.planned = true;
        h->spmm.build_ms = wall_ms() - t0;
    }
    const hipError_t e = smvp::launch_csr_spmm(h->d_row_ptr, h->d_col_ind, h->d_val, h->spmm.d_order, d_X, ldx, d_Y, ldy, h->rows, k, st);
    if (e != hipSuccess)
        return smvp::fail(SMVP_ERR_HIP, "smvp_csr_spmm: launch failed: %s", hipGetErrorString(e));
    return SMVP_OK;
}

extern "C" int smvp_csr_spmm(smvp_csr_t *h, int k, const double *d_X, long long ldx, double *d_Y, long long ldy, void *stream)
{
    if (!h)
        return smvp::fail(SMVP_ERR_INVALID, "smvp_csr_spmm: null handle");
    if (h->flavor != smvp::kFlavorCsr)
        return smvp::fail(SMVP_ERR_UNSUPPORTED, "smvp_csr_spmm: plain CSR handles only (this one belongs to a TJDS matrix)");
    if (int rc = check_block_operands("smvp_csr_spmm", k, d_X, ldx, h->cols, d_Y, ldy, h->rows, h->nnz))
        return rc;
    DeviceScope on(h->device);
    return csr_spmm_enqueue(h, k, d_X, ldx, d_Y, ldy, (hipStream_t)stream);
}

extern "C" int smvp_csr_cg_multi(smvp_csr_t *h, const smvp_cg_opts_t *opts, int k, const double *d_B, long long ldb, const double *d_X0,
                                 long long ldx0, double *d_X, long long ldx, const double *d_m, smvp_pcg_result_t *results, double *rr_each,
                                 double *rz_each, double *sigma_each, void *stream)
{
    if (int rc = smvp::cg_multi_check_args("smvp_csr_cg_multi", h, opts, results, d_B))
        return rc;
    if (int rc = refuse_tjds_flavor("smvp_csr_cg_multi", h))
        return rc;
    return smvp::cg_multi_run("smvp_csr_cg_multi", h->device, h->rows, h->cols, opts, k, d_B, ldb, d_X0, ldx0, d_X, ldx, d_m, results, rr_each,
                              rz_each, sigma_each, stream, [h, k, stream](const double *X, long long ldX, double *Y, long long ldY) {
                                  return csr_spmm_enqueue(h, k, X, ldX, Y, ldY, (hipStream_t)stream);
                              });
}

extern "C" int smvp_csr_spmm_describe(const smvp_csr_t *h, int k, char *kernel_name, size_t cap, double *alg_bytes, smvp_plan_info_t *plan)
{
    if (!h)
        return smvp::fail(SMVP_ERR_INVALID, "smvp_csr_spmm_describe: null handle");
    if (h->flavor != smvp::kFlavorCsr)
        return smvp::fail(SMVP_ERR_UNSUPPORTED, "smvp_csr_spmm_describe: plain CSR handles only");
    if (k < 1)
        return smvp::fail(SMVP_ERR_INVALID, "smvp_csr_spmm_describe: k = %d (need k >= 1)", k);
    if (kernel_name && cap)
        smvp::spmm_kernel_name(k, kernel_name, cap);
    if (alg_bytes)
        *alg_bytes = csr_matrix_bytes(h) + 8.0 * k * ((double)h->cols + h->rows);
    if (plan) {
        plan->matrix_bytes = csr_matrix_bytes(h);
        plan->plan_bytes = h->spmm.planned ? 4.0 * h->rows : 0.0;
        plan->build_ms = h->spmm.planned ? h->spmm.build_ms : 0.0;
    }
    return SMVP_OK;
}

extern "C" int smvp_csr_device_arrays(const smvp_csr_t *h, const int **d_row_ptr, const int **d_col_ind, const double **d_val)
{
    if (!h)
        return smvp::fail(SMVP_ERR_INVALID, "smvp_csr_device_arrays: null handle");
    if (h->flavor != smvp::kFlavorCsr)
        return smvp::fail(SMVP_ERR_UNSUPPORTED, "smvp_csr_device_arrays: plain CSR handles only (this one belongs to a TJDS matrix)");
    if (d_row_ptr)
        *d_row_ptr = h->d_row_ptr;
    if (d_col_ind)
        *d_col_ind = h->d_col_ind;
    if (d_val)
        *d_val = h->d_val;
    return SMVP_OK;
}

extern "C" int smvp_csr_create_transposed(smvp_csr_t **out, const smvp_csr_t *h, void *stream)
{
    if (out)
        *out = nullptr;
    if (!out || !h)
        return smvp::fail(SMVP_ERR_INVALID, "smvp_csr_create_transposed: null %s", out ? "handle" : "out");
    if (h->flavor != smvp::kFlavorCsr)
        return smvp::fail(SMVP_ERR_UNSUPPORTED, "smvp_csr_create_transposed: plain CSR handles only (this one belongs to a TJDS matrix)");
    DeviceScope on(h->device);
    hipStream_t st = (hipStream_t)stream;
    if (int rc = refuse_capture(st, "smvp_csr_create_transposed: allocates and synchronises, so it cannot be captured "
                                    "(the stream is capturing)"))
        return rc;
    const int t_rows = h->cols, t_cols = h->rows, nnz = h->nnz;
    int *t_row_ptr = nullptr, *t_col_ind = nullptr;
    double *t_val = nullptr;
    smvp_coo_t *coo = nullptr;
    auto release = [&]() {
        for (void *p : {(void *)t_row_ptr, (void *)t_col_ind, (void *)t_val, (void *)coo})
            if (p)
                (void)hipFree(p);
    };
    if (hipMalloc((void **)&t_row_ptr, sizeof(int) * ((size_t)t_rows + 4)) != hipSuccess ||
        hipMalloc((void **)&t_col_ind, sizeof(int) * std::max<size_t>((size_t)nnz, 4)) != hipSuccess ||
        hipMalloc((void **)&t_val, sizeof(double) * std::max<size_t>((size_t)nnz, 4)) != hipSuccess ||
        hipMalloc((void **)&coo, sizeof(smvp_coo_t) * std::max<size_t>((size_t)nnz, 4)) != hipSuccess) {
        (void)hipGetLastError();
        release();
        return smvp::fail(SMVP_ERR_ALLOC, "smvp_csr_create_transposed: cannot allocate the transposed arrays and the entry list (%d entries)", nnz);
    }
    int rc = SMVP_OK;
    const hipError_t e = smvp::launch_csr_swapped_coo(h->d_row_ptr, h->d_col_ind, h->d_val, h->rows, nnz, coo, st);
    if (e != hipSuccess)
        rc = smvp::fail(SMVP_ERR_HIP, "smvp_csr_create_transposed: launch failed: %s", hipGetErrorString(e));
    if (rc == SMVP_OK) {
        rc = smvp_csr_from_coo_device(coo, t_rows, t_cols, nnz, t_row_ptr, t_col_ind, t_val, stream);
        if (rc == SMVP_ERR_HIP && strstr(smvp_last_error(), "out of memory")) {
            (void)hipGetLastError();
            rc = smvp::fail(SMVP_ERR_ALLOC, "smvp_csr_create_transposed: cannot allocate the sort's buffers (%d entries)", nnz);
        }
    }
    if (rc != SMVP_OK)
        (void)hipStreamSynchronize(st);
    (void)hipFree(coo);
    coo = nullptr;
    smvp_csr_t *t = nullptr;
    if (rc == SMVP_OK) {
        rc = csr_create_impl(&t, h->device, t_rows, t_cols, nnz, t_row_ptr, t_col_ind, t_val, SMVP_MEM_DEVICE, nullptr, smvp::kFlavorCsr);
        if (rc == SMVP_ERR_HIP && strstr(smvp_last_error(), "out of memory")) {
            (void)hipGetLastError();
            rc = smvp::fail(SMVP_ERR_ALLOC, "smvp_csr_create_transposed: cannot allocate the transposed handle's plan (%d entries)", nnz);
        }
    }
// ... 29 lines not shown
```

smvp-toolkit_amd/csrc/smvp_error.cpp:

```cpp
#include "smvp_common.h"

#include <atomic>
#include <cstring>

namespace {
thread_local char g_err[512] = "";
}

namespace smvp {
int fail(int code, const char *fmt, ...)
{
    va_list ap;
    va_start(ap, fmt);
    vsnprintf(g_err, sizeof g_err, fmt, ap);
    va_end(ap);
    return code;
}
void clear_error() { g_err[0] = '\0'; }
}

extern "C" const char *smvp_last_error(void) { return g_err; }

extern "C" const char *smvp_version_string(void)
{
    static char v[32];
    snprintf(v, sizeof v, "%d.%d.%d", SMVP_VERSION_MAJOR, SMVP_VERSION_MINOR, SMVP_VERSION_REVISION);
    return v;
}

namespace {
struct Option { const char *name; std::atomic<int> value; };
Option g_options[] = {
    {"csr_col16", {-1}},
    {"csr_rowrel", {-1}},
    {"csr_read_once", {-1}},
    {"csr_sweep_alternate", {-1}},
    {"binned_near", {-1}},
    {"binned_overlap", {-1}},
    {"tjds_index", {-1}},
    {"sharded_threads", {-1}},
    {"trsv_chain_width", {-1}},
    {"trsv_lanes_by_mean", {-1}},
    {"mm_threads", {-1}},
};
Option *find_option(const char *name)
{
    if (name)
        for (Option &o : g_options)
            if (!strcmp(o.name, name))
                return &o;
    return nullptr;
}
}

namespace smvp {
int option(const char *name, int fallback)
{
    const Option *o = find_option(name);
    const int v = o ? o->value.load(std::memory_order_relaxed) : -1;
    return v < 0 ? fallback : v;
}
}

extern "C" int smvp_set_option(const char *name, int value)
{
    Option *o = find_option(name);
    if (!o)
        return smvp::fail(SMVP_ERR_INVALID, "smvp_set_option: no option called '%s'", name ? name : "(null)");
    o->value.store(value < 0 ? -1 : value, std::memory_order_relaxed);
    return SMVP_OK;
}

extern "C" int smvp_get_option(const char *name, int *value)
{
    const Option *o = find_option(name);
    if (!o || !value)
        return smvp::fail(SMVP_ERR_INVALID, "smvp_get_option: no option called '%s'", name ? name : "(null)");
    *value = o->value.load(std::memory_order_relaxed);
    return SMVP_OK;
}
```

smvp-toolkit_amd/csrc/smvp_kernels.h:

```cpp
#pragma once
#include <hip/hip_runtime.h>

#include "smvp_amd.h"
#include "smvp_tile_map.h"

namespace smvp {

constexpr int kVectorBlock = 256;
constexpr int kStreamBlock = 256;
constexpr int kLongRow = 32;
constexpr int kStreamOver = 1024;
constexpr int kStreamTileGroup = 64;
constexpr int kTjdsTileGroup = 32;
constexpr int kSweepBlock = 256;
constexpr int kSweepWaves = kSweepBlock / 64;
constexpr int kSweepUnroll = 4;
constexpr int kSweepChunk = 64 * kSweepUnroll;
constexpr int kSweepXcdParts = 8;
constexpr int kSweepRowBits = 13;
constexpr int kSweepTurnCap = (1 << (16 - kSweepRowBits)) - 1;
constexpr int kTjdsBlock = 256;
constexpr int kTjdsDiagChunk = 8;

constexpr int kSpmmMaxVectors = 16;
constexpr int kSpmmBlockRows = 4096;
int build_spmm_order(const int *row_ptr, int rows, int longest_row, int *order, hipStream_t stream);
hipError_t launch_csr_spmm(const int *row_ptr, const int *col_ind, const double *val, const int *order, const double *X,
                           long long ldx, double *Y, long long ldy, int rows, int k, hipStream_t stream);
int build_tjds_spmm_plan(const int *row_ind, const int *start_pos, const int *perm, int num_diag, int nnz, int rows, int *ptr,
                         int *pos, int *col, int *order, hipStream_t stream);
hipError_t launch_tjds_spmm(const int *ptr, const int *pos, const int *col, const double *val, const int *order, const double *X,
                            long long ldx, double *Y, long long ldy, int rows, int k, hipStream_t stream);
hipError_t launch_tjds_transposed(const int *start_pos, const int *row_ind, const double *val, const int *perm, const double *x,
                                  double *y, int cols, int num_diag, hipStream_t stream);
hipError_t launch_tjds_spmm_transposed(const int *start_pos, const int *row_ind, const double *val, const int *perm, const double *X,
                                       long long ldx, double *Y, long long ldy, int cols, int num_diag, int k, hipStream_t stream);
void spmm_kernel_name(int k, char *name, size_t cap);
void tjds_spmm_kernel_name(int k, char *name, size_t cap);
void tjds_spmm_transposed_kernel_name(int k, char *name, size_t cap);
const char *tjds_transposed_kernel_name();

hipError_t launch_csr_diagonal(int lanes_per_row, const int *row_ptr, const int *col_ind, const double *val, double *d, int rows,
                               int cols, long long first_row, hipStream_t stream);
hipError_t launch_tjds_diagonal(const int *start_pos, const int *row_ind, const double *val, const int *perm, double *d, int rows,
                                int cols, int num_diag, hipStream_t stream);
hipError_t launch_csr_swapped_coo(const int *row_ptr, const int *col_ind, const double *val, int rows, int nnz, smvp_coo_t *coo,
                                  hipStream_t stream);

hipError_t launch_csr_vector(int lanes_per_row, const int *row_ptr, const int *col_ind, const double *val,
                             const double *x, double *y, int rows, hipStream_t stream);
hipError_t launch_csr_stream(int vpt, const int *row_ptr, const int *col_ind, const double *val,
                             const double *x, double *y, const int *tile_row, const int *carry_row,
                             double *carry, int rows, int nnz, int ntiles, hipStream_t stream);
inline int tile_group(int ntiles, int wanted = kStreamTileGroup) { return tile_group_of(ntiles, wanted); }
constexpr int kFlavorCsr = 0;
constexpr int kFlavorTjdsK = 2;
constexpr int kFlavorTjdsS = 3;
constexpr int kFlavorTjdsH = 4;
constexpr int kFlavorCsr16 = 5;
constexpr int kSlotBits = 11;

struct OwnerLaunch {
    const int *row_ptr = nullptr, *col_ind = nullptr;
    const double *val = nullptr, *x = nullptr;
    double *y = nullptr;
    const int *tile_row = nullptr, *tile_next = nullptr;
    const int *pos = nullptr;
    const int *start_pos = nullptr;
    unsigned long long *stamps = nullptr;
    const int *ovf_ptr = nullptr, *ovf_k = nullptr;
    const double *ovf_val = nullptr;
    const int *cache_ptr = nullptr;
    const double *val_cache = nullptr;
    const unsigned short *col16 = nullptr;
    const int *col_base = nullptr;
    const unsigned short *group_run = nullptr;
    const unsigned *word32 = nullptr;
    int unit_x = 0;
    const int *run_ptr = nullptr, *run_tab = nullptr;
    const unsigned short *row_rel = nullptr;
    int rows = 0, nnz = 0, ntiles = 0;
    int read_once = 0;
    int backward = 0;
};
hipError_t launch_csr_stream_owner(int vpt, int flavor, const OwnerLaunch &l, hipStream_t stream);
void debug_owner_phases();
void debug_binned_phases();
int owner_stamp_slots(int ntiles, int flavor);
constexpr int kRepeatCtlWords = 32 * 66;
constexpr unsigned kRepeatPatienceDefaultUs = 50000;
int owner_repeat_grid(int vpt, int flavor, int ntiles);
hipError_t launch_csr_stream_owner_repeat(int vpt, int flavor, const OwnerLaunch &l, int reps, int grid, unsigned *ctl_words,
                                          bool first_of_run, unsigned long long patience_ticks, hipStream_t stream);
inline unsigned long long repeat_patience_ticks(int us) { return us < 0 ? 0ull : 100ull * (unsigned)(us ? us : (int)kRepeatPatienceDefaultUs); }
hipError_t launch_stamp_reduce(const unsigned long long *stamps, int slots_per_product, int products,
                               unsigned long long *first_last, hipStream_t stream);
hipError_t launch_tjds_products(const int *start_pos, const double *val, const double *x_perm, double *prod,
                                const int4 *work, int nwork, int cols, hipStream_t stream);
hipError_t launch_tjds_scatter(bool operand_by_row, const int *start_pos, const int *row_ind, const double *val,
                               const double *x_perm, double *y, const int4 *work, int nwork, int cols,
                               hipStream_t stream);
hipError_t launch_tjds_permute(const int *perm, const double *x, double *x_perm, int cols, hipStream_t stream);
hipError_t launch_find_out_of_range(const int *a, long long n, int limit, int *bad, hipStream_t stream);
hipError_t launch_normalize_max(double *v, long long n, unsigned long long *scratch, hipStream_t stream);
hipError_t launch_fill(double *p, double v, long long n, hipStream_t stream);

hipError_t launch_csr_colsweep(const long long *strip_ptr, const int *e_col, const double *e_val, const unsigned short *e_row,
                               const double *x, double *y, int rows, int strip_rows, int parts, int per_launch, int g, double *ypart,
                               hipStream_t stream);
hipError_t prepare_csr_colsweep();
int sweep_chunks_in_flight(int strip_rows, int asked);
constexpr int kSpreadSpan = 64 * 1024;
hipError_t launch_csr_line_spread(const int *col_ind, long long nnz, int samples, int *distinct, hipStream_t stream);

constexpr int kBinColBits = 14;
constexpr int kBinSlots = 8192;
constexpr int kBinRowCap = 1024;
constexpr int kBinBucket = kBinSlots - kBinRowCap;
constexpr int kBinThreads = 1024;
constexpr int kBinShiftCap = 1024;
constexpr int kBinNearBand = 4096;

struct BinnedStream {
    int groups = 0, padded = 0, cells = 0;
    unsigned short *word = nullptr;
    int *chunk = nullptr;
    int *ptr = nullptr;
    int *shift_ptr = nullptr;
    int *shift = nullptr;
};

constexpr int kNwRowBlock = 8192;
constexpr int kNwBand = 4096;
constexpr int kNwShortCap = 16;
constexpr int kNwLongCap = 1024;
struct NearWindow {
    bool on = false;
    int rows = 0, cols = 0, nblocks = 0, n_out = 0;
    long long row0 = 0;
    long long slots = 0;
    int *wave_ptr = nullptr;
    int *wave_n1 = nullptr, *wave_n2 = nullptr;
    unsigned short *perm16 = nullptr;
    double *sval = nullptr;
    unsigned short *sword = nullptr;
    int *blk_long_ptr = nullptr;
    unsigned short *long_row16 = nullptr;
    int *out_row = nullptr, *out_ptr = nullptr, *out_col = nullptr;
    double *out_val = nullptr;
    size_t plan_bytes = 0;
};
void free_near_window(NearWindow *p);
int build_near_window(const int *near_ptr, const int *near_col, const double *near_val, const int *capped, int rows, int cols,
                      int nnz_near, int band, long long row0, NearWindow *out, hipStream_t stream);
hipError_t launch_near_window(const NearWindow &p, const double *x, double *y, hipStream_t stream);

struct BinnedPlan {
    int band = kBinNearBand;
    long long row0 = 0;
    int rows = 0, cols = 0, nnz = 0, nnz_near = 0, nf = 0;
    int ncb = 0, nrb = 0, q = 1, nfr = 0, splits = 1;
    int slots = kBinSlots, threads_b = kBinThreads;
    int *near_ptr = nullptr, *near_col = nullptr;
    double *near_val = nullptr;
    NearWindow nw;
    double *a_val = nullptr;
    BinnedStream a, b;
    double *bins = nullptr;
    int *fr_row = nullptr, *fr_ptr = nullptr, *blk_fr = nullptr;
    int4 *b_desc = nullptr;
    unsigned *fr32 = nullptr;
    size_t plan_bytes = 0;
};
void free_binned_plan(BinnedPlan *p);
int build_binned_plan(const int *d_row_ptr, const int *d_col_ind, const double *d_val, int rows, int cols, int nnz, int band,
                      long long row0, bool near_window, BinnedPlan *out, hipStream_t stream);
hipError_t binned_reserve_lds();
hipError_t near_window_reserve_lds();
hipError_t launch_binned_products(const BinnedPlan &p, const double *x, hipStream_t stream);
hipError_t launch_binned_sums(const BinnedPlan &p, double *y, hipStream_t stream);
int csr_far_share(const int *d_row_ptr, const int *d_col_ind, int rows, int nnz, int band, long long row0, double *share, hipStream_t stream);

template <int N>
__device__ __forceinline__ double dpp_row_shl(double v)
{
    int lo = __double2loint(v), hi = __double2hiint(v);
    lo = __builtin_amdgcn_update_dpp(0, lo, 0x100 + N, 0xf, 0xf, true);
    hi = __builtin_amdgcn_update_dpp(0, hi, 0x100 + N, 0xf, 0xf, true);
    return __hiloint2double(hi, lo);
}

__device__ __forceinline__ double wave_sum_dpp(double v)
{
#if defined(__HIP_DEVICE_COMPILE__) && !defined(__GFX9__)
#error "wave_sum_dpp: four DPP rows of 16 lanes = one wave64 (gfx9 / CDNA only)"
#endif
    v += dpp_row_shl<8>(v);
    v += dpp_row_shl<4>(v);
    v += dpp_row_shl<2>(v);
    v += dpp_row_shl<1>(v);
    const int lo = __double2loint(v), hi = __double2hiint(v);
    double r[4];
#pragma unroll
    for (int k = 0; k < 4; ++k)
        r[k] = __hiloint2double(__builtin_amdgcn_readlane(hi, 16 * k), __builtin_amdgcn_readlane(lo, 16 * k));
    return (r[0] + r[1]) + (r[2] + r[3]);
}

template <int WIDTH>
__device__ __forceinline__ double shfl_down_sum(double v)
{
#pragma unroll
    for (int off = WIDTH / 2; off > 0; off >>= 1)
        v += __shfl_down(v, off, WIDTH);
    return v;
}

}
```

smvp-toolkit_amd/csrc/smvp_owner.hip:

```cpp
#include "smvp_owner_kernel.h"

#include <cstdio>

namespace smvp {

__attribute__((used)) __device__ double shfl_any_width(double v, int width) { return __shfl_down(v, 1, width); }

constexpr int kRepeatMaxShards = 32;
constexpr unsigned kRepeatAbort = 0x80000000u;

struct RepeatCtl {
    unsigned *sticky = nullptr;
    unsigned *shard = nullptr;
    unsigned *top = nullptr;
    unsigned *go = nullptr;
    unsigned long long *stamps = nullptr;
    int reps = 0, grid_virtual = 0, slots_per_product = 0;
    int shards = 1;
    unsigned long long patience = 0;
};

template <int VPT, int FLAVOR>
__global__ __launch_bounds__(kStreamBlock) void csr_stream_owner_repeat(
    const int *__restrict__ row_ptr, const int *__restrict__ col_ind, const double *__restrict__ val,
    const double *__restrict__ x, double *__restrict__ y, const int *__restrict__ tile_row,
    const int *__restrict__ tile_next, int rows, int nnz_arg, int ntiles, int tile_group_arg, const OwnerExtra ex, const RepeatCtl ctl)
{
    __shared__ unsigned go;
    const int t = threadIdx.x;
    const unsigned nwg = gridDim.x, me = blockIdx.x;
    const unsigned S = (unsigned)ctl.shards;
    const unsigned sh = me % S;
    const unsigned members = (nwg - sh + S - 1) / S;
    const unsigned arrivals = S > 1 ? (nwg < S ? nwg : S) : nwg;
    unsigned long long *stamp = ctl.stamps + 2 * ((size_t)me * (kStreamBlock / 64) + (t >> 6));
    if (t == 0) {
        go = __hip_atomic_load(ctl.sticky, __ATOMIC_RELAXED, __HIP_MEMORY_SCOPE_AGENT) ? 0u : 1u;
        if (!go)
            atomicOr(ctl.top, kRepeatAbort);
    }
    __syncthreads();
    if (!go)
        return;
    for (int rep = 0; rep < ctl.reps; ++rep) {
        __syncthreads();
        if (t == 0) {
            const unsigned gen = (unsigned)rep + 1u;
            const unsigned long long t0 = wall_clock64();
            unsigned seen = 0;
            if (S > 1) {
                const unsigned before = atomicAdd(ctl.shard + 32 * sh, 1u);
                if (before + 1u == members * gen) {
                    const unsigned tb = atomicAdd(ctl.top, 1u);
                    if ((tb & ~kRepeatAbort) + 1u == arrivals * gen)
                        for (unsigned q = 0; q < S; ++q)
                            __hip_atomic_fetch_max(ctl.go + 32 * q, gen, __ATOMIC_RELAXED, __HIP_MEMORY_SCOPE_AGENT);
                }
                for (;;) {
                    const unsigned g = __hip_atomic_load(ctl.go + 32 * sh, __ATOMIC_RELAXED, __HIP_MEMORY_SCOPE_AGENT);
                    if (g >= gen && g != kRepeatAbort)
                        break;
                    if (g == kRepeatAbort) {
                        seen = kRepeatAbort;
                        break;
                    }
                    if (wall_clock64() - t0 > ctl.patience) {
                        atomicOr(ctl.top, kRepeatAbort);
                        __hip_atomic_store(ctl.sticky, 1u, __ATOMIC_RELAXED, __HIP_MEMORY_SCOPE_AGENT);
                        for (unsigned q = 0; q < S; ++q)
                            __hip_atomic_fetch_max(ctl.go + 32 * q, kRepeatAbort, __ATOMIC_RELAXED, __HIP_MEMORY_SCOPE_AGENT);
                        seen = kRepeatAbort;
                        break;
                    }
                    __builtin_amdgcn_s_sleep(2);
                }
            } else {
                atomicAdd(ctl.top, 1u);
                for (;;) {
                    seen = __hip_atomic_load(ctl.top, __ATOMIC_RELAXED, __HIP_MEMORY_SCOPE_AGENT);
                    if ((seen & kRepeatAbort) || (seen & ~kRepeatAbort) >= arrivals * gen)
                        break;
                    if (wall_clock64() - t0 > ctl.patience) {
                        atomicOr(ctl.top, kRepeatAbort);
                        __hip_atomic_store(ctl.sticky, 1u, __ATOMIC_RELAXED, __HIP_MEMORY_SCOPE_AGENT);
                        seen = kRepeatAbort;
                        break;
                    }
                    __builtin_amdgcn_s_sleep(1);
                }
            }
            go = seen & kRepeatAbort ? 0u : 1u;
        }
        __syncthreads();
        if (!go)
            return;
        if ((t & 63) == 0)
            stamp[0] = wall_clock64();
        for (int vb = (int)me; vb < ctl.grid_virtual; vb += (int)nwg) {
            if (vb != (int)me)
                __syncthreads();
            int salt = 0;
            asm volatile("" : "+v"(salt));
            owner_body<VPT, FLAVOR, false>(row_ptr, col_ind, val, x, y, tile_row, tile_next, rows, nnz_arg, ntiles, tile_group_arg, ex, vb, salt);
        }
        asm volatile("s_waitcnt vmcnt(0)" ::: "memory");
        if ((t & 63) == 0)
            stamp[1] = wall_clock64();
        stamp += 2 * (size_t)ctl.slots_per_product;
    }
}

__global__ __launch_bounds__(256) void stamp_reduce(const unsigned long long *__restrict__ stamps, int slots_per_product,
                                                    unsigned long long *__restrict__ first_last)
{
    __shared__ unsigned long long lo_s[256 / 64], hi_s[256 / 64];
    const unsigned long long *s = stamps + (size_t)blockIdx.x * slots_per_product * 2;
    unsigned long long lo = ~0ull, hi = 0ull;
    for (int i = threadIdx.x; i < slots_per_product; i += 256) {
        const unsigned long long f = s[2 * i], l = s[2 * i + 1];
        lo = f < lo ? f : lo;
        hi = l > hi ? l : hi;
    }
#pragma unroll
    for (int off = 32; off > 0; off >>= 1) {
        const unsigned long long ol = __shfl_down(lo, off, 64), oh = __shfl_down(hi, off, 64);
        lo = ol < lo ? ol : lo;
        hi = oh > hi ? oh : hi;
    }
    if ((threadIdx.x & 63) == 0) {
        lo_s[threadIdx.x >> 6] = lo;
        hi_s[threadIdx.x >> 6] = hi;
    }
    __syncthreads();
    if (threadIdx.x == 0) {
        for (int w = 1; w < 256 / 64; ++w) {
            lo = lo_s[w] < lo ? lo_s[w] : lo;
            hi = hi_s[w] > hi ? hi_s[w] : hi;
        }
        first_last[2 * blockIdx.x] = lo;
        first_last[2 * blockIdx.x + 1] = hi;
    }
}

static unsigned owner_grid(int ntiles, int group) { return tile_grid_of(ntiles, group); }

static int flavor_group(int flavor) { return flavor == kFlavorTjdsS || flavor == kFlavorTjdsH ? kTjdsTileGroup : kStreamTileGroup; }

int owner_stamp_slots(int ntiles, int flavor)
{
    return (int)owner_grid(ntiles, tile_group(ntiles, flavor_group(flavor))) * (kStreamBlock / 64);
}

hipError_t launch_csr_stream_owner(int vpt, int flavor, const OwnerLaunch &l, hipStream_t stream)
{
    if (l.rows <= 0)
        return hipSuccess;
    const int group = tile_group(l.ntiles, flavor_group(flavor));
    const dim3 grid(owner_grid(l.ntiles, group));
    OwnerExtra ex = owner_extra_of(l, l.stamps);
    ex.back_grid = l.backward ? (int)grid.x : 0;
#define SMVP_OWNER_ST(V, F, S)                                                                                     \
    hipLaunchKernelGGL((csr_stream_owner<V, F, S>), grid, dim3(kStreamBlock), 0, stream, l.row_ptr, l.col_ind, l.val, \
                       l.x, l.y, l.tile_row, l.tile_next, l.rows, l.nnz, l.ntiles, group, ex)
#define SMVP_OWNER(V, F)                  \
    if (vpt == V && flavor == F) {        \
        if (l.stamps)                     \
            SMVP_OWNER_ST(V, F, true);    \
        else                              \
            SMVP_OWNER_ST(V, F, false);   \
        return hipGetLastError();         \
    }
#ifdef SMVP_PHASE_STAMPS
    SMVP_OWNER_CSR_FORMS(SMVP_OWNER)
#else
    if (flavor == kFlavorCsr || flavor == kFlavorCsr16)
        return launch_owner_csr(vpt, flavor, l, ex, grid.x, group, stream);
#endif
    SMVP_OWNER_TJDS_FORMS(SMVP_OWNER)
#undef SMVP_OWNER
#undef SMVP_OWNER_ST
    return hipErrorInvalidValue;
}

template <int V, int F>
static int repeat_capacity()
{
    int per_cu = 0, dev = 0, cus = 0;
    if (hipOccupancyMaxActiveBlocksPerMultiprocessor(&per_cu, csr_stream_owner_repeat<V, F>, kStreamBlock, 0) != hipSuccess ||
        hipGetDevice(&dev) != hipSuccess || hipDeviceGetAttribute(&cus, hipDeviceAttributeMultiprocessorCount, dev) != hipSuccess) {
        (void)hipGetLastError();
        return 0;
    }
    return per_cu > 1 ? (per_cu - 1) * cus * 3 / 4 : 0;
}

int owner_repeat_grid(int vpt, int flavor, int ntiles)
{
    if (ntiles <= 0)
        return 0;
    int cap = 0;
#define X(V, F)                     \
    if (vpt == V && flavor == F)    \
        cap = repeat_capacity<V, F>();
    SMVP_OWNER_REPEAT_FORMS(X)
#undef X
    if (cap <= 0)
        return 0;
    const int full = (int)owner_grid(ntiles, tile_group(ntiles, flavor_group(flavor)));
    return full <= cap ? full : 0;
}

hipError_t launch_csr_stream_owner_repeat(int vpt, int flavor, const OwnerLaunch &l, int reps, int grid, unsigned *ctl_words,
                                          bool first_of_run, unsigned long long patience_ticks, hipStream_t stream)
{
    if (l.rows <= 0)
        return hipSuccess;
    const int group = tile_group(l.ntiles, flavor_group(flavor));
    RepeatCtl ctl{};
    ctl.sticky = ctl_words;
    ctl.shard = ctl_words + 32, ctl.go = ctl_words + 32 * (1 + kRepeatMaxShards), ctl.top = ctl_words + kRepeatCtlWords - 32;
    ctl.shards = grid <= 24 ? 1 : grid <= 640 ? 8 : 16;
    ctl.stamps = l.stamps;
    ctl.reps = reps, ctl.grid_virtual = (int)owner_grid(l.ntiles, group), ctl.slots_per_product = grid * (kStreamBlock / 64);
    ctl.patience = patience_ticks;
    if (reps <= 0 || grid <= 0 || ctl.grid_virtual <= 0 || !ctl.stamps || !ctl_words)
        return hipErrorInvalidValue;
    static_assert(kRepeatCtlWords == 32 * (2 + 2 * kRepeatMaxShards), "sticky + shards + go words + top, one 128-byte line each");
    hipError_t e = first_of_run ? hipMemsetAsync(ctl_words, 0, sizeof(unsigned) * kRepeatCtlWords, stream)
                                : hipMemsetAsync(ctl_words + 32, 0, sizeof(unsigned) * (kRepeatCtlWords - 32), stream);
    if (e != hipSuccess)
        return e;
    const OwnerExtra ex = owner_extra_of(l, nullptr);
#define X(V, F)                                                                                                                    \
    if (vpt == V && flavor == F) {                                                                                                 \
        hipLaunchKernelGGL((csr_stream_owner_repeat<V, F>), dim3((unsigned)grid), dim3(kStreamBlock), 0, stream, l.row_ptr, l.col_ind, \
                           l.val, l.x, l.y, l.tile_row, l.tile_next, l.rows, l.nnz, l.ntiles, group, ex, ctl);                     \
        return hipGetLastError();                                                                                                  \
    }
    SMVP_OWNER_REPEAT_FORMS(X)
#undef X
    return hipErrorInvalidValue;
}

#ifdef SMVP_PHASE_STAMPS
void debug_owner_phases()
{
    unsigned long long h[8] = {0, 0, 0, 0, 0, 0, 0, 0}, z[8] = {0, 0, 0, 0, 0, 0, 0, 0};
    if (hipMemcpyFromSymbol(h, HIP_SYMBOL(g_owner_phase), sizeof h) != hipSuccess || h[7] == 0)
        return;
    const double n = (double)h[7];
    fprintf(stderr, "[owner dbg] mean us per workgroup over %.0f: loads + gathers + LDS writes %.2f | barrier %.2f | lane-per-row sums %.2f | "
                    "barrier %.2f | long rows %.2f\n", n, h[0] * 0.01 / n, h[1] * 0.01 / n, h[2] * 0.01 / n, h[3] * 0.01 / n, h[4] * 0.01 / n);
    (void)hipMemcpyToSymbol(HIP_SYMBOL(g_owner_phase), z, sizeof z);
}
#else
void debug_owner_phases() {}
#endif

hipError_t launch_stamp_reduce(const unsigned long long *stamps, int slots_per_product, int products,
                               unsigned long long *first_last, hipStream_t stream)
{
    if (products <= 0)
        return hipSuccess;
    hipLaunchKernelGGL(stamp_reduce, dim3(products), dim3(256), 0, stream, stamps, slots_per_product, first_last);
    return hipGetLastError();
}

}
```

smvp-toolkit_amd/csrc/smvp_owner_csr.hip:

```cpp
#include "smvp_owner_kernel.h"

namespace smvp {

#ifdef SMVP_PHASE_STAMPS
hipError_t launch_owner_csr(int, int, const OwnerLaunch &, const OwnerExtra &, unsigned, int, hipStream_t) { return hipErrorInvalidValue; }
#else
hipError_t launch_owner_csr(int vpt, int flavor, const OwnerLaunch &l, const OwnerExtra &ex, unsigned grid_x, int group, hipStream_t stream)
{
    const dim3 grid(grid_x);
#define SMVP_OWNER_ST(K, V, F, S)                                                                                  \
    hipLaunchKernelGGL((K<V, F, S>), grid, dim3(kStreamBlock), 0, stream, l.row_ptr, l.col_ind, l.val, \
                       l.x, l.y, l.tile_row, l.tile_next, l.rows, l.nnz, l.ntiles, group, ex)
#define SMVP_OWNER(K, V, F)               \
    if (vpt == V && flavor == F) {        \
        if (l.stamps)                     \
            SMVP_OWNER_ST(K, V, F, true); \
        else                              \
            SMVP_OWNER_ST(K, V, F, false);\
        return hipGetLastError();         \
    }
#define SMVP_OWNER_ONCE(V, F) SMVP_OWNER(read_once::csr_stream_owner, V, F)
#define SMVP_OWNER_PLAIN(V, F) SMVP_OWNER(csr_stream_owner, V, F)
    if (l.read_once) {
        SMVP_OWNER_CSR_WIDE_FORMS(SMVP_OWNER_ONCE)
    }
    SMVP_OWNER_CSR_FORMS(SMVP_OWNER_PLAIN)
#undef SMVP_OWNER_PLAIN
#undef SMVP_OWNER_ONCE
#undef SMVP_OWNER
#undef SMVP_OWNER_ST
    return hipErrorInvalidValue;
}
#endif

}
```

smvp-toolkit_amd/csrc/smvp_owner_kernel.h:

```cpp
#pragma once
#include "smvp_kernels.h"

namespace smvp {


typedef int int4v __attribute__((ext_vector_type(4)));
typedef int int2v __attribute__((ext_vector_type(2)));
typedef double double2v __attribute__((ext_vector_type(2)));

struct OwnerExtra {
    const int *pos = nullptr;
    const int *start_pos = nullptr;
    const int *ovf_ptr = nullptr;
    const double *ovf_val = nullptr;
    const int *ovf_k = nullptr;
    const int *cache_ptr = nullptr;
    const double *val_cache = nullptr;
    const unsigned short *col16 = nullptr;
    const int *col_base = nullptr;
    const unsigned *word32 = nullptr;
    const unsigned short *group_run = nullptr;
    const int *run_ptr = nullptr;
    const int *run_tab = nullptr;
    int unit_x = 0;
    const unsigned short *row_rel = nullptr;
    unsigned long long *stamps = nullptr;
    int back_grid = 0;
};

inline OwnerExtra owner_extra_of(const OwnerLaunch &l, unsigned long long *stamps)
{
    OwnerExtra ex{};
    ex.pos = l.pos, ex.start_pos = l.start_pos, ex.ovf_ptr = l.ovf_ptr, ex.ovf_val = l.ovf_val, ex.ovf_k = l.ovf_k;
    ex.cache_ptr = l.cache_ptr, ex.val_cache = l.val_cache;
    ex.col16 = l.col16, ex.col_base = l.col_base;
    ex.unit_x = l.unit_x, ex.word32 = l.word32, ex.group_run = l.group_run, ex.run_ptr = l.run_ptr, ex.run_tab = l.run_tab;
    ex.row_rel = l.row_rel;
    ex.stamps = stamps;
    return ex;
}

struct OwnerArgs {
    const int *__restrict__ col_ind;
    const double *__restrict__ val;
    const double *__restrict__ x;
    const int *__restrict__ pos;
    const int *__restrict__ start_pos;
    const double *__restrict__ ovf_val;
    const int *__restrict__ ovf_k;
    int unit_x;
};

template <int FLAVOR>
__device__ __forceinline__ double owner_product_slow(const OwnerArgs &a, long long j)
{
    if constexpr (FLAVOR == kFlavorCsr || FLAVOR == kFlavorCsr16)
        return a.val[j] * a.x[a.col_ind[j]];
    else if constexpr (FLAVOR == kFlavorTjdsK)
        return a.val[a.pos[j]] * a.x[a.col_ind[j]];
    else {
        const int p = a.pos[j];
        return a.val[p] * a.x[p - a.start_pos[(unsigned)a.col_ind[j] >> kSlotBits]];
    }
}

template <int FLAVOR>
__device__ __forceinline__ double owner_overflow_product(const OwnerArgs &a, int ovf_base, int e, int i)
{
    if constexpr (FLAVOR == kFlavorTjdsS || FLAVOR == kFlavorTjdsH)
        return a.unit_x ? a.val[a.ovf_k[ovf_base + i]] : a.ovf_val[ovf_base + i] * a.x[a.ovf_k[ovf_base + i]];
    else
        return owner_product_slow<FLAVOR>(a, (long long)e + i);
}

#ifdef SMVP_PHASE_STAMPS
[[maybe_unused]] static __device__ unsigned long long g_owner_phase[8];
#define SMVP_PHASE(n)                                                                        \
    do {                                                                                     \
        if (threadIdx.x == 0 && (blockIdx.x & 127) == 5) {                                   \
            const unsigned long long now_ = wall_clock64();                                  \
            if ((n) > 0)                                                                     \
                atomicAdd(&g_owner_phase[(n)-1], now_ - phase_prev_);                        \
            else                                                                             \
                atomicAdd(&g_owner_phase[7], 1ull);                                          \
            phase_prev_ = now_;                                                              \
        }                                                                                    \
    } while (0)
#else
#define SMVP_PHASE(n) do { } while (0)
#endif

#ifndef SMVP_TJDS_NEUTRALISE
#define SMVP_TJDS_NEUTRALISE 0
#endif

template <int VPT, int FLAVOR, bool STAMPED, bool STREAMED = false>
__device__ __forceinline__ void owner_body(
    const int *__restrict__ row_ptr, const int *__restrict__ col_ind, const double *__restrict__ val,
    const double *__restrict__ x, double *__restrict__ y, const int *__restrict__ tile_row,
    const int *__restrict__ tile_next, int rows, int nnz_arg, int ntiles, int tile_group_arg, const OwnerExtra &ex, const int block, const int lane_salt = 0)
{
    const OwnerArgs a = {col_ind, val, x, ex.pos, ex.start_pos, ex.ovf_val, ex.ovf_k, FLAVOR == kFlavorTjdsH ? ex.unit_x : 0};
    constexpr int TILE = kStreamBlock * VPT;
    constexpr int QCAP = (TILE + kStreamOver) / kLongRow + 1;
    constexpr bool CSR = FLAVOR == kFlavorCsr || FLAVOR == kFlavorCsr16;
    constexpr bool COL16 = FLAVOR == kFlavorCsr16;
    constexpr bool HALF = FLAVOR == kFlavorTjdsH;
    constexpr bool TJDS = FLAVOR == kFlavorTjdsK || FLAVOR == kFlavorTjdsS || HALF;
    constexpr bool SORTED = FLAVOR == kFlavorTjdsS || HALF;
    static_assert(TILE <= (1 << kSlotBits), "slot bits");
    __shared__ double prod[TILE + kStreamOver];
    __shared__ int long_rows[QCAP];
    __shared__ int long_a[QCAP];
    __shared__ int long_z[QCAP];
    __shared__ int long_count;
    __shared__ double wave_sum[kStreamBlock / 64];

    const int t = threadIdx.x;
#ifdef SMVP_PHASE_STAMPS
    unsigned long long phase_prev_ = 0;
#endif
    unsigned long long *stamp = nullptr;
    if constexpr (STAMPED) {
        stamp = ex.stamps + 2 * ((size_t)block * (kStreamBlock / 64) + (t >> 6));
        if ((t & 63) == 0)
            stamp[0] = wall_clock64();
    }
#define SMVP_OWNER_EXIT()                                         \
    do {                                                          \
        if constexpr (STAMPED) {                                  \
            asm volatile("s_waitcnt vmcnt(0)" ::: "memory");      \
            if ((t & 63) == 0)                                    \
                stamp[1] = wall_clock64();                        \
        }                                                         \
        return;                                                   \
    } while (0)

    const int b = tile_of_block_swept(block, tile_group_arg, ex.back_grid);
    if (b >= ntiles)
        SMVP_OWNER_EXIT();
    const int nnz = nnz_arg;
    const long long s = (long long)b * TILE;

    const int e0 = (t >> 6) * (64 * VPT) + (VPT > 1 ? 2 : 1) * (t & 63) + lane_salt;
    auto lane_entry = [e0](int k) { return e0 + 128 * (k >> 1) + (k & 1); };
    const long long j0 = s + e0;
    int c[VPT];
    int pj[VPT];
    double v[VPT];
    const bool full_tile = s + TILE <= (long long)nnz;
    int grp[HALF ? VPT : 1];
    int run0 = 0;
    int2 run_tbl = make_int2(0, 0);
    if constexpr (HALF) {
        if (full_tile) {
            run0 = ex.run_ptr[b];
            const int nruns = ex.run_ptr[b + 1] - run0;
            const int ln = t & 63;
            if (ln < nruns)
                run_tbl = reinterpret_cast<const int2 *>(ex.run_tab)[run0 + ln];
        }
    }
    if constexpr (HALF) {
        if (full_tile) {
#pragma unroll
            for (int k = 0; k < VPT; ++k) {
                if constexpr (VPT == 1) {
                    pj[k] = (int)ex.word32[s + k * kStreamBlock + t];
                } else {
                    pj[k] = (int)__builtin_nontemporal_load(ex.word32 + s + k * kStreamBlock + t);
                }
                const unsigned gw = reinterpret_cast<const unsigned *>(ex.group_run)[((size_t)b * (TILE / 32) + k * (kStreamBlock / 32) +
                                                                                     2 * __builtin_amdgcn_readfirstlane(t >> 6)) >> 1];
                grp[k] = (t & 32) ? (int)(gw >> 16) : (int)(gw & 0xffffu);
            }
        }
    } else if constexpr (SORTED) {
        if (full_tile) {
#pragma unroll
            for (int k = 0; k < VPT; ++k) {
                if constexpr (VPT > 1) {
                    pj[k] = __builtin_nontemporal_load(a.pos + s + k * kStreamBlock + t);
                    c[k] = __builtin_nontemporal_load(a.col_ind + s + k * kStreamBlock + t);
                } else {
                    pj[k] = a.pos[s + k * kStreamBlock + t];
                    c[k] = a.col_ind[s + k * kStreamBlock + t];
                }
            }
        }
    } else if (full_tile) {
        if constexpr (VPT >= 4) {
            auto load_cols = [&]() {
#pragma unroll
                for (int k = 0; k < VPT; k += 2)
                    *reinterpret_cast<int2 *>(&c[k]) = *reinterpret_cast<const int2 *>(a.col_ind + s + lane_entry(k));
            };
            if constexpr (COL16) {
                const int base = ex.col_base[b];
                if (base >= 0) {
                    if constexpr (VPT == 8) {
                        const unsigned short *mine = ex.col16 + s + ((t >> 6) * (64 * VPT) + (t & 63) * VPT + lane_salt);
                        unsigned w[VPT / 2];
                        if constexpr (STREAMED)
                            *reinterpret_cast<int4v *>(w) = __builtin_nontemporal_load(reinterpret_cast<const int4v *>(mine));
                        else
                            *reinterpret_cast<int4v *>(w) = *reinterpret_cast<const int4v *>(mine);
#pragma unroll
                        for (int k = 0; k < VPT; k += 2)
                            c[k] = base + (int)(w[k / 2] & 0xffffu), c[k + 1] = base + (int)(w[k / 2] >> 16);
                    } else {
#pragma unroll
                        for (int k = 0; k < VPT; k += 2) {
                            const unsigned w = *reinterpret_cast<const unsigned *>(ex.col16 + s + lane_entry(k));
                            c[k] = base + (int)(w & 0xffffu), c[k + 1] = base + (int)(w >> 16);
                        }
                    }
                } else {
                    load_cols();
                }
            } else {
                load_cols();
            }
            if constexpr (TJDS) {
#pragma unroll
                for (int k = 0; k < VPT; k += 2)
                    *reinterpret_cast<int2v *>(&pj[k]) = __builtin_nontemporal_load(reinterpret_cast<const int2v *>(a.pos + s + lane_entry(k)));
            }
            if constexpr (CSR) {
#pragma unroll
                for (int k = 0; k < VPT; k += 2) {
                    if constexpr (STREAMED)
                        *reinterpret_cast<double2v *>(&v[k]) = __builtin_nontemporal_load(reinterpret_cast<const double2v *>(a.val + s + lane_entry(k)));
                    else
                        *reinterpret_cast<double2 *>(&v[k]) = *reinterpret_cast<const double2 *>(a.val + s + lane_entry(k));
                }
            }
        } else {
            c[0] = a.col_ind[j0];
            if constexpr (TJDS)
                pj[0] = a.pos[j0];
            if constexpr (CSR)
                v[0] = a.val[j0];
        }
    }
    const int rlo = tile_row[b];
    const int rhi = tile_row[b + 1];
    if (rlo == rhi)
        SMVP_OWNER_EXIT();
    SMVP_PHASE(0);
    const int lo = (int)s;
    const int e = (int)(s + TILE < (long long)nnz ? s + TILE : (long long)nnz);
    const int zend = tile_next[b];
    const int ext = zend - e;
    const unsigned short *__restrict__ row_rel = ex.row_rel;
    auto row_bounds = [&](int r, int &ra, int &rz) {
        if (row_rel) {
            ra = row_rel[r];
            rz = r + 1 < rhi ? (int)row_rel[r + 1] : zend - lo;
        } else {
            ra = row_ptr[r] - lo;
            rz = row_ptr[r + 1] - lo;
        }
    };
    const bool giant = ext > kStreamOver;
    if (t == 0)
        long_count = 0;
    const bool over0 = !giant && t < ext;
    double p[VPT];
    double po = 0.0;
    int rp_a = 0, rp_b = 0, rp_a2 = 0, rp_b2 = 0;
    int ovf_base = 0, cache0 = 0, in_place = 0;
    if constexpr (SORTED) {
        ovf_base = ex.ovf_ptr[b];
        cache0 = ex.cache_ptr[b];
        in_place = (e - lo) - (ex.cache_ptr[b + 1] - cache0);
    }
    if constexpr (SORTED) {
        if (full_tile && rlo + t < rhi)
            row_bounds(rlo + t, rp_a, rp_b);
        if (full_tile && rlo + t + kStreamBlock < rhi)
            row_bounds(rlo + t + kStreamBlock, rp_a2, rp_b2);
        int co = 0;
        double vo = 0.0;
        const bool unit_x = HALF && ex.unit_x;
        if (over0 && !(SMVP_TJDS_NEUTRALISE & 8)) {
            co = a.ovf_k[ovf_base + t];
            if (!unit_x)
                vo = a.ovf_val[ovf_base + t];
        }
        if (full_tile) {
            int slot[VPT];
#pragma unroll
            for (int k = 0; k < VPT; ++k) {
                if constexpr (HALF)
                    c[k] = (int)((unsigned)pj[k] >> 16), pj[k] &= 0xffff;
                slot[k] = c[k] & ((1 << kSlotBits) - 1);
                if constexpr (HALF) {
                    const int r = grp[k] + (((c[k] >> kSlotBits) - grp[k]) & 31);
                    int base = __shfl(run_tbl.x, r & 63), sub = __shfl(run_tbl.y, r & 63);
                    if (r >= 64) {
                        const int2 w = reinterpret_cast<const int2 *>(ex.run_tab)[run0 + r];
                        base = w.x, sub = w.y;
                    }
                    pj[k] += base;
                    c[k] = pj[k] - sub;
                } else {
                    c[k] = pj[k] - a.start_pos[(unsigned)c[k] >> kSlotBits];
                }
            }
            double xk[VPT];
#pragma unroll
            for (int k = 0; k < VPT; ++k) {
                const int idx = k * kStreamBlock + t;
                const double *src = idx < in_place ? a.val + pj[k] : ex.val_cache + (cache0 + (idx - in_place));
                if ((SMVP_TJDS_NEUTRALISE & 2) && idx < in_place)
                    v[k] = 1.0;
                else if ((SMVP_TJDS_NEUTRALISE & 4) && idx >= in_place)
                    v[k] = 1.0;
                else
                    v[k] = *src;
            }
            double xo = 0.0;
            if (unit_x) {
#pragma unroll
                for (int k = 0; k < VPT; ++k)
                    xk[k] = 1.0;
                if (over0)
                    vo = a.val[co], xo = 1.0;
            } else {
#pragma unroll
                for (int k = 0; k < VPT; ++k)
                    xk[k] = (SMVP_TJDS_NEUTRALISE & 1) ? 1.0 : a.x[c[k]];
                xo = over0 && !(SMVP_TJDS_NEUTRALISE & 8) ? a.x[co] : 0.0;
            }
#pragma unroll
            for (int k = 0; k < VPT; ++k)
                prod[slot[k]] = v[k] * xk[k];
            po = vo * xo;
        } else {
            for (int k = 0; k < VPT; ++k) {
                const int idx = k * kStreamBlock + t;
                if (s + idx < (long long)nnz) {
                    if constexpr (HALF) {
                        const unsigned w32 = ex.word32[s + idx];
                        const int m = (int)(w32 >> 16), g = ex.group_run[(size_t)b * (TILE / 32) + (idx >> 5)];
                        const int r = g + (((m >> kSlotBits) - g) & 31);
                        const int2 w = reinterpret_cast<const int2 *>(ex.run_tab)[ex.run_ptr[b] + r];
                        const int pw = w.x + (int)(w32 & 0xffffu);
                        const double vv = idx < in_place ? a.val[pw] : ex.val_cache[cache0 + (idx - in_place)];
                        prod[m & ((1 << kSlotBits) - 1)] = unit_x ? vv : vv * a.x[pw - w.y];
                    } else {
                        const int pw = a.pos[s + idx];
                        const double vv = idx < in_place ? a.val[pw] : ex.val_cache[cache0 + (idx - in_place)];
                        const int m = a.col_ind[s + idx];
                        prod[m & ((1 << kSlotBits) - 1)] = vv * a.x[pw - a.start_pos[(unsigned)m >> kSlotBits]];
                    }
                }
            }
            if (over0)
                po = unit_x ? a.val[co] : vo * a.x[co];
        }
    } else if (full_tile) {
        if (rlo + t < rhi)
            row_bounds(rlo + t, rp_a, rp_b);
        if (rlo + t + kStreamBlock < rhi)
            row_bounds(rlo + t + kStreamBlock, rp_a2, rp_b2);
        int co = 0, pjo = 0;
        double vo = 0.0;
        if (over0) {
            co = a.col_ind[e + t];
            if constexpr (TJDS)
                pjo = a.pos[e + t];
            if constexpr (CSR)
                vo = a.val[e + t];
        }
        double xk[VPT];
        if constexpr (TJDS) {
#pragma unroll
            for (int k = 0; k < VPT; ++k)
                v[k] = a.val[pj[k]];
            if (over0)
                vo = a.val[pjo];
        }
#pragma unroll
        for (int k = 0; k < VPT; ++k)
            xk[k] = a.x[c[k]];
        const double xo = over0 ? a.x[co] : 0.0;
#pragma unroll
        for (int k = 0; k < VPT; ++k)
            p[k] = v[k] * xk[k];
        po = vo * xo;
    } else {
#pragma unroll
        for (int k = 0; k < VPT; ++k)
            p[k] = (s + lane_entry(k) < (long long)nnz) ? owner_product_slow<FLAVOR>(a, s + lane_entry(k)) : 0.0;
        if (over0)
            po = owner_product_slow<FLAVOR>(a, e + t);
    }
    if constexpr (!SORTED) {
        if constexpr (VPT >= 2) {
#pragma unroll
            for (int k = 0; k < VPT; k += 2)
                *reinterpret_cast<double2 *>(&prod[lane_entry(k)]) = make_double2(p[k], p[k + 1]);
        } else {
            prod[t] = p[0];
        }
    }
    if (over0)
        prod[e - lo + t] = po;
    if (!giant)
        for (int i = t + kStreamBlock; i < ext; i += kStreamBlock)
            prod[e - lo + i] = owner_overflow_product<FLAVOR>(a, ovf_base, e, i);
    SMVP_PHASE(1);
    __syncthreads();
    SMVP_PHASE(2);

    const int last = rhi - 1;
    auto finish_row = [&](int r, int ra, int rz) {
        if (rz - ra <= kLongRow) {
            double acc = 0.0;
            for (int i = ra; i < rz; i += 4) {
                const double v0 = prod[i], v1 = prod[i + 1 < rz ? i + 1 : i], v2 = prod[i + 2 < rz ? i + 2 : i],
                             v3 = prod[i + 3 < rz ? i + 3 : i];
                acc += v0;
                if (i + 1 < rz)
                    acc += v1;
                if (i + 2 < rz)
                    acc += v2;
                if (i + 3 < rz)
                    acc += v3;
            }
            if constexpr (VPT == 1)
                y[r] = acc;
            else
                __builtin_nontemporal_store(acc, &y[r]);
        } else {
            const int q = atomicAdd(&long_count, 1);
            long_rows[q] = r;
            long_a[q] = ra;
            long_z[q] = rz;
        }
    };
    int r_next = rlo + t;
    if (full_tile) {
        if (r_next < rhi && !(giant && r_next == last))
            finish_row(r_next, rp_a, rp_b);
        r_next += kStreamBlock;
        if (r_next < rhi && !(giant && r_next == last))
            finish_row(r_next, rp_a2, rp_b2);
        r_next += kStreamBlock;
    }
    for (int r = r_next; r < rhi; r += kStreamBlock) {
        if (giant && r == last)
            continue;
        int ra, rz;
        row_bounds(r, ra, rz);
        finish_row(r, ra, rz);
    }
    SMVP_PHASE(3);
    __syncthreads();
    SMVP_PHASE(4);

    const int nlong = long_count;
    const int lane = t & 63;
    for (int q = t >> 6; q < nlong; q += kStreamBlock / 64) {
        const int zq = long_z[q];
        double acc = 0.0;
        for (int i = long_a[q] + lane; i < zq; i += 64)
            acc += prod[i];
        acc = wave_sum_dpp(acc);
        if (lane == 0)
            y[long_rows[q]] = acc;
    }
    SMVP_PHASE(5);

    if (giant) {
        const int ra = row_ptr[last];
        double acc = 0.0;
        for (int i = ra - lo + t; i < e - lo; i += kStreamBlock)
            acc += prod[i];
        for (int j = e + t; j < zend; j += 4 * kStreamBlock) {
            double pg[4];
#pragma unroll
            for (int u = 0; u < 4; ++u) {
                const int jj = j + u * kStreamBlock;
                pg[u] = jj < zend ? owner_overflow_product<FLAVOR>(a, ovf_base, e, jj - e) : 0.0;
            }
#pragma unroll
            for (int u = 0; u < 4; ++u)
                acc += pg[u];
        }
        acc = shfl_down_sum<64>(acc);
        if (lane == 0)
            wave_sum[t >> 6] = acc;
        __syncthreads();
        if (t == 0) {
            double total = 0.0;
#pragma unroll
            for (int w = 0; w < kStreamBlock / 64; ++w)
                total += wave_sum[w];
            y[last] = total;
        }
    }
    SMVP_OWNER_EXIT();
#undef SMVP_OWNER_EXIT
}

template <int VPT, int FLAVOR, bool STAMPED>
__global__ __launch_bounds__(kStreamBlock) void csr_stream_owner(
    const int *__restrict__ row_ptr, const int *__restrict__ col_ind, const double *__restrict__ val,
    const double *__restrict__ x, double *__restrict__ y, const int *__restrict__ tile_row,
    const int *__restrict__ tile_next, int rows, int nnz_arg, int ntiles, int tile_group_arg, const OwnerExtra ex)
{
    owner_body<VPT, FLAVOR, STAMPED>(row_ptr, col_ind, val, x, y, tile_row, tile_next, rows, nnz_arg, ntiles, tile_group_arg, ex,
                                     (int)blockIdx.x);
}

namespace read_once {
template <int VPT, int FLAVOR, bool STAMPED>
__global__ __launch_bounds__(kStreamBlock) void csr_stream_owner(
    const int *__restrict__ row_ptr, const int *__restrict__ col_ind, const double *__restrict__ val,
    const double *__restrict__ x, double *__restrict__ y, const int *__restrict__ tile_row,
    const int *__restrict__ tile_next, int rows, int nnz_arg, int ntiles, int tile_group_arg, const OwnerExtra ex)
{
    owner_body<VPT, FLAVOR, STAMPED, true>(row_ptr, col_ind, val, x, y, tile_row, tile_next, rows, nnz_arg, ntiles, tile_group_arg, ex,
                                           (int)blockIdx.x);
}
}

#define SMVP_OWNER_CSR_WIDE_FORMS(X) X(4, kFlavorCsr) X(8, kFlavorCsr) X(4, kFlavorCsr16) X(8, kFlavorCsr16)
#define SMVP_OWNER_CSR_FORMS(X) X(1, kFlavorCsr) SMVP_OWNER_CSR_WIDE_FORMS(X)
#define SMVP_OWNER_TJDS_TILE_FORMS(X) \
    X(1, kFlavorTjdsS) X(4, kFlavorTjdsS) X(8, kFlavorTjdsS) X(1, kFlavorTjdsH) X(4, kFlavorTjdsH) X(8, kFlavorTjdsH)
#define SMVP_OWNER_TJDS_FORMS(X) X(1, kFlavorTjdsK) X(4, kFlavorTjdsK) X(8, kFlavorTjdsK) SMVP_OWNER_TJDS_TILE_FORMS(X)
#define SMVP_OWNER_REPEAT_FORMS(X) SMVP_OWNER_CSR_FORMS(X) SMVP_OWNER_TJDS_TILE_FORMS(X)

hipError_t launch_owner_csr(int vpt, int flavor, const OwnerLaunch &l, const OwnerExtra &ex, unsigned grid_x, int group, hipStream_t stream);

}
```

smvp-toolkit_amd/csrc/smvp_tile_map.h:

```cpp
#pragma once

#if defined(__HIPCC__)
#define SMVP_HOST_DEVICE __host__ __device__
#else
#define SMVP_HOST_DEVICE
#endif

namespace smvp {

inline int tile_group_of(int ntiles, int wanted)
{
    const int fit = ntiles / 64;
    return fit < 1 ? 1 : (fit < wanted ? fit : wanted);
}

inline unsigned tile_grid_of(int ntiles, int group) { return (unsigned)((ntiles + 8 * group - 1) / (8 * group)) * 8u * group; }

SMVP_HOST_DEVICE inline __attribute__((always_inline)) int tile_of_block(int block, int group)
{
    const int xcd = block & 7, seq = block >> 3;
    return (seq / group) * (8 * group) + xcd * group + seq % group;
}

SMVP_HOST_DEVICE inline __attribute__((always_inline)) int tile_of_block_swept(int block, int group, int back_grid)
{
    return tile_of_block(back_grid ? back_grid - 1 - block : block, group);
}

SMVP_HOST_DEVICE inline __attribute__((always_inline)) int tile_lane_entry(int t, int k, int vpt)
{
    return (t >> 6) * (64 * vpt) + 2 * (t & 63) + 128 * (k >> 1) + (k & 1);
}

constexpr int kCol16LaneOrderTile = 2048;
SMVP_HOST_DEVICE inline __attribute__((always_inline)) int col16_slot(int o, int vpt)
{
    const int chunk = 64 * vpt;
    const int w = o / chunk, q = o % chunk, l = (q % 128) / 2, k = 2 * (q / 128) + (q & 1);
    return w * chunk + l * vpt + k;
}

}
```

smvp-toolkit_amd/python/smvp_toolkit_amd/__init__.py:

```python
import ctypes as C
import os

import numpy as np

_HERE = os.path.dirname(os.path.abspath(__file__))
PKG_ROOT = os.path.dirname(os.path.dirname(_HERE))
REPO_ROOT = os.path.dirname(PKG_ROOT)
LIB_PATH = os.environ.get("SMVP_LIB_PATH") or os.path.join(PKG_ROOT, "lib", "libsmvp_amd.so")
CLI_PATH = os.path.join(PKG_ROOT, "bin", "smvp-toolkit-cli")

OK = 0
ERR_INVALID, ERR_NO_DEVICE, ERR_HIP, ERR_ALLOC, ERR_IO, ERR_UNSUPPORTED = 1, 2, 3, 4, 5, 6
MM_COULD_NOT_READ_FILE, MM_PREMATURE_EOF, MM_NOT_MTX, MM_NO_HEADER, MM_UNSUPPORTED_TYPE = 11, 12, 13, 14, 15
CSR_KERNEL_AUTO, CSR_KERNEL_VECTOR, CSR_KERNEL_STREAM, CSR_KERNEL_STREAM_CARRY, CSR_KERNEL_COLSWEEP = 0, 1, 2, 3, 4
CSR_KERNEL_BINNED = 5
MEM_HOST, MEM_DEVICE = 0, 1
SYNTH_MEMPLUS_SHAPED, SYNTH_UNIFORM = 1, 2
TJDS_MODE_AUTO, TJDS_MODE_ATOMIC, TJDS_MODE_TWO_PHASE, TJDS_MODE_ROW_GATHER = 0, 1, 2, 3
TIMING_AUTO, TIMING_EVENTS, TIMING_DEVICE, TIMING_DEVICE_GRAPH = 0, 1, 2, 3
MAX_ENTRIES = 2 ** 31 - 1 - 65536

COO_DTYPE = np.dtype([("row", "<i4"), ("col", "<i4"), ("val", "<f8")], align=True)


def set_option(name, value):
    _check(lib().smvp_set_option(name.encode(), -1 if value is None else int(value)), "smvp_set_option")


def get_option(name):
    v = C.c_int()
    _check(lib().smvp_get_option(name.encode(), C.byref(v)), "smvp_get_option")
    return v.value


class option:

    def __init__(self, name, value):
        self.name, self.value = name, value

    def __enter__(self):
        self.old = get_option(self.name)
        set_option(self.name, self.value)
        return self

    def __exit__(self, *exc):
        set_option(self.name, self.old)
        return False


def sweep_parts(rows_per_block, parts, chunks=0):
    return int(rows_per_block) | ({1: 0, 2: 1, 4: 2, 8: 3}[int(parts)] << 24) | ({0: 0, 1: 1, 2: 2, 4: 3}[int(chunks)] << 26)


class TimeStats(C.Structure):
    _fields_ = [(n, C.c_double) for n in ("time_total", "time_avg", "time_stdev", "time_min", "time_max")]


class RunOpts(C.Structure):
    _fields_ = [("struct_size", C.c_uint), ("device", C.c_int), ("csr_kernel", C.c_int), ("csr_param", C.c_int),
                ("tjds_ref_quirks", C.c_int), ("convert_on_device", C.c_int), ("ngpus", C.c_int),
                ("iterate", C.c_int), ("normalize", C.c_int), ("tjds_mode", C.c_int), ("timing", C.c_int),
                ("shard_exchange", C.c_int), ("repeat_patience_us", C.c_int), ("x", C.c_void_p)]


class PlanInfo(C.Structure):
    _fields_ = [("matrix_bytes", C.c_double), ("plan_bytes", C.c_double), ("build_ms", C.c_double)]


class RunInfo(C.Structure):
    _fields_ = [("timing", C.c_int), ("graph_replays", C.c_int), ("wall_ms", C.c_double), ("device_clock_khz", C.c_double),
                ("repeat_launches", C.c_int), ("repeat_gave_up", C.c_int)]


class ShardOpts(C.Structure):
    _fields_ = [("struct_size", C.c_uint), ("chunks", C.c_int), ("balance", C.c_int), ("exchange", C.c_int)]


class PowerOpts(C.Structure):
    _fields_ = [("struct_size", C.c_uint), ("max_steps", C.c_int), ("check_every", C.c_int), ("tol", C.c_double)]


class PowerResult(C.Structure):
    _fields_ = [("steps", C.c_int), ("reason", C.c_int), ("index", C.c_int), ("eigenvalue", C.c_double),
                ("residual", C.c_double), ("scale", C.c_double)]


class CgOpts(C.Structure):
    _fields_ = [("struct_size", C.c_uint), ("max_steps", C.c_int), ("check_every", C.c_int), ("tol", C.c_double)]


class CgResult(C.Structure):
    _fields_ = [("steps", C.c_int), ("updates", C.c_int), ("reason", C.c_int), ("pad", C.c_int), ("rr", C.c_double), ("bb", C.c_double)]


class PcgResult(C.Structure):
    _fields_ = [("steps", C.c_int), ("updates", C.c_int), ("reason", C.c_int), ("pad", C.c_int), ("rr", C.c_double), ("rz", C.c_double),
                ("bb", C.c_double)]


class BicgstabOpts(C.Structure):
    _fields_ = [("struct_size", C.c_uint), ("max_steps", C.c_int), ("check_every", C.c_int), ("tol", C.c_double)]


class BicgstabResult(C.Structure):
    _fields_ = [("steps", C.c_int), ("full", C.c_int), ("half", C.c_int), ("reason", C.c_int), ("rr", C.c_double), ("bb", C.c_double)]


class GmresOpts(C.Structure):
    _fields_ = [("struct_size", C.c_uint), ("max_steps", C.c_int), ("check_every", C.c_int), ("restart", C.c_int), ("tol", C.c_double)]


class GmresResult(C.Structure):
    _fields_ = [("steps", C.c_int), ("cycles", C.c_int), ("columns", C.c_int), ("reason", C.c_int), ("rr", C.c_double), ("bb", C.c_double)]


class LsqrOpts(C.Structure):
    _fields_ = [("struct_size", C.c_uint), ("max_steps", C.c_int), ("check_every", C.c_int), ("pad", C.c_int), ("tol", C.c_double),
                ("atol", C.c_double)]


class LsqrResult(C.Structure):
    _fields_ = [("steps", C.c_int), ("updates", C.c_int), ("reason", C.c_int), ("pad", C.c_int), ("rnorm", C.c_double),
                ("arnorm", C.c_double), ("anorm", C.c_double), ("bnorm", C.c_double)]


class TrsvInfo(C.Structure):
    _fields_ = [("struct_size", C.c_uint), ("levels", C.c_int), ("max_level_width", C.c_int), ("launches", C.c_int), ("chains", C.c_int),
                ("chain_width", C.c_int), ("missing_diagonals", C.c_int), ("lanes_per_row", C.c_int), ("entries", C.c_longlong),
                ("plan_bytes", C.c_double), ("build_ms", C.c_double)]


class Ilu0Info(C.Structure):
    _fields_ = [("struct_size", C.c_uint), ("levels", C.c_int), ("max_level_width", C.c_int), ("launches", C.c_int), ("chains", C.c_int),
                ("chain_width", C.c_int), ("lanes_per_row", C.c_int), ("entries", C.c_longlong), ("pivots", C.c_longlong),
                ("plan_bytes", C.c_double), ("build_ms", C.c_double)]


POWER_CONVERGED, POWER_MAX_STEPS, POWER_ZERO, POWER_NONFINITE = 0, 1, 2, 3
TRSV_LOWER, TRSV_UPPER = 0, 1
TRSV_DIAG_STORED, TRSV_DIAG_UNIT = 0, 1
CG_CONVERGED, CG_MAX_STEPS, CG_BREAKDOWN, CG_NONFINITE = 0, 1, 2, 3
BICGSTAB_CONVERGED, BICGSTAB_MAX_STEPS, BICGSTAB_BREAKDOWN, BICGSTAB_NONFINITE = 0, 1, 2, 3
GMRES_CONVERGED, GMRES_MAX_STEPS, GMRES_BREAKDOWN, GMRES_NONFINITE = 0, 1, 2, 3
LSQR_CONVERGED, LSQR_LEAST_SQUARES, LSQR_MAX_STEPS, LSQR_NONFINITE = 0, 1, 2, 3
GATHER_NONE, GATHER_OVERLAPPED, GATHER_AFTER = 0, 1, 2
EXCHANGE_RCCL, EXCHANGE_COPIES, EXCHANGE_DIRECT, EXCHANGE_AUTO = 0, 1, 2, 3
EXCHANGE_NAMES = {EXCHANGE_RCCL: "rccl", EXCHANGE_COPIES: "copies", EXCHANGE_DIRECT: "direct", EXCHANGE_AUTO: "auto"}


class SmvpError(RuntimeError):
    def __init__(self, code, where, msg=None):
        self.code = code
        if msg is None:
            msg = lib().smvp_last_error().decode(errors="replace")
        super().__init__("%s failed with status %d: %s" % (where, code, msg))


def _check_entries(nnz, where):
    if nnz > MAX_ENTRIES:
        raise SmvpError(ERR_UNSUPPORTED, where, "%d entries: more than the %d a matrix may hold" % (nnz, MAX_ENTRIES))


_lib = None

EXPORTS = [
    "smvp_last_error", "smvp_version_string", "smvp_set_option", "smvp_get_option",
    "smvp_mm_read_banner", "smvp_mm_read_mtx_crd_size", "smvp_mm_read_coo_entries",
    "smvp_mm_read_header_path", "smvp_mm_read_coo_path", "smvp_mm_expanded_count", "smvp_mm_expand_symmetric",
# ... 1158 lines not shown
```

Baseline: 944.3 GFLOP/s.

## Add packed CSR stream kernel with 8-bit hot-value codes and escape values

Adds a stream kernel flavor that replaces the fp64 value array with per-entry 8-bit codes into a 64-entry table of the most frequent values. Values not in the table are stored in a compact per-wave escape array. The table is built from a sampled radix sort at plan build time, and decoding uses ballot/mbcnt prefix counts and ds_bpermute. This aims to cut HBM traffic for matrix values, at the cost of extra decode work, LDS staging, and a preprocessing pass. Packing is bounded so it is skipped when escapes are too common.

```diff
diff --git a/include/smvp_amd.h b/include/smvp_amd.h
--- a/include/smvp_amd.h
+++ b/include/smvp_amd.h
@@ -88,7 +88,8 @@
     SMVP_CSR_KERNEL_STREAM = 2,
     SMVP_CSR_KERNEL_STREAM_CARRY = 3,
     SMVP_CSR_KERNEL_COLSWEEP = 4,
-    SMVP_CSR_KERNEL_BINNED = 5
+    SMVP_CSR_KERNEL_BINNED = 5,
+    SMVP_CSR_KERNEL_STREAM_PACKED = 6
 };
 enum {
     SMVP_MEM_HOST = 0,
diff --git a/smvp-toolkit_amd/csrc/smvp_common.h b/smvp-toolkit_amd/csrc/smvp_common.h
--- a/smvp-toolkit_amd/csrc/smvp_common.h
+++ b/smvp-toolkit_amd/csrc/smvp_common.h
@@ -49,6 +49,8 @@
                             int *runs_total, ihipStream_t *stream);
 int build_column_offsets(const int *d_col_ind, int nnz, int tile, int *d_col_base, unsigned short *d_col16, int *fits,
                          ihipStream_t *stream);
+int build_packed_values(const double *d_val, int nnz, const int *d_col_base, unsigned char **d_code8, double **d_hot, int **d_esc_ptr,
+                        double **d_esc_val, long long *doubles_read, long long *esc_slots, long long max_doubles, ihipStream_t *stream);
 int build_tile_overflow(const int *d_pos, const int *d_ovf_ptr, int total, int ntiles, int tile, int nnz,
                         const int *d_start_pos, int num_diag, const double *d_val, double *d_ovf_val, int *d_ovf_k, int positions,
                         ihipStream_t *stream);
diff --git a/smvp-toolkit_amd/csrc/smvp_convert_device.hip b/smvp-toolkit_amd/csrc/smvp_convert_device.hip
--- a/smvp-toolkit_amd/csrc/smvp_convert_device.hip
+++ b/smvp-toolkit_amd/csrc/smvp_convert_device.hip
@@ -976,9 +976,216 @@
     }
 }
 
+constexpr int kPackedTile = smvp::kCol16LaneOrderTile, kPackedVpt = kPackedTile / 256;
+constexpr int kPackedSampleMax = 1 << 20;
+
+__global__ __launch_bounds__(256) void sample_value_bits(const double *__restrict__ val, int nnz, int stride, int n, u64 *__restrict__ key,
+                                                         unsigned *__restrict__ idx)
+{
+    const int i = blockIdx.x * 256 + threadIdx.x;
+    if (i < n) {
+        key[i] = (u64)__double_as_longlong(val[(long long)i * stride]);
+        idx[i] = (unsigned)i;
+    }
+}
+
+__device__ __forceinline__ unsigned hot_code(const u64 *tab, int nhot, u64 bits)
+{
+    int lo = 0, hi = nhot;
+    while (lo < hi) {
+        const int mid = (lo + hi) >> 1;
+        if (tab[mid] < bits)
+            lo = mid + 1;
+        else
+            hi = mid;
+    }
+    return lo < nhot && tab[lo] == bits ? (unsigned)lo : (unsigned)smvp::kEscapeCode;
+}
+
+__device__ __forceinline__ void escape_places(const unsigned (&code)[kPackedVpt], int *before, int *total)
+{
+    int b = 0, n = 0;
+#pragma unroll
+    for (int k = 0; k < kPackedVpt; ++k) {
+        const u64 mask = __ballot(code[k] == (unsigned)smvp::kEscapeCode);
+        b = (int)__builtin_amdgcn_mbcnt_hi((unsigned)(mask >> 32), __builtin_amdgcn_mbcnt_lo((unsigned)mask, (unsigned)b));
+        n += __popcll(mask);
+    }
+    *before = b, *total = n;
+}
+
+__global__ __launch_bounds__(256) void packed_codes(const double *__restrict__ val, int nnz, const int *__restrict__ col_base,
+                                                    const u64 *__restrict__ hot_bits, int nhot, unsigned char *__restrict__ code8,
+                                                    int *__restrict__ run_len, u64 *__restrict__ doubles_read)
+{
+    __shared__ u64 tab[smvp::kHotValues];
+    const int b = blockIdx.x, t = threadIdx.x;
+    const long long s = (long long)b * kPackedTile;
+    if (col_base[b] < 0 || s + kPackedTile > (long long)nnz) {
+        if (t < 4)
+            run_len[4 * b + t] = 0;
+        if (t == 0)
+            atomicAdd(doubles_read, (u64)((long long)nnz - s < kPackedTile ? (long long)nnz - s : kPackedTile));
+        return;
+    }
+    if (t < smvp::kHotValues)
+        tab[t] = t < nhot ? hot_bits[t] : 0;
+    __syncthreads();
+    unsigned code[kPackedVpt];
+#pragma unroll
+    for (int k = 0; k < kPackedVpt; ++k)
+        code[k] = hot_code(tab, nhot, (u64)__double_as_longlong(val[s + smvp::tile_lane_entry(t, k, kPackedVpt)]));
+    uint2 w = make_uint2(0, 0);
+#pragma unroll
+    for (int k = 0; k < 4; ++k)
+        w.x |= code[k] << (8 * k), w.y |= code[k + 4] << (8 * k);
+    *reinterpret_cast<uint2 *>(code8 + s + (t >> 6) * (64 * kPackedVpt) + (t & 63) * kPackedVpt) = w;
+    int before, total;
+    escape_places(code, &before, &total);
+    if ((t & 63) == 0) {
+        run_len[4 * b + (t >> 6)] = (total + 1) & ~1;
+        atomicAdd(doubles_read, (u64)total);
+    }
+}
+
+__global__ __launch_bounds__(256) void packed_escapes(const double *__restrict__ val, int nnz, const int *__restrict__ col_base,
+                                                      const unsigned char *__restrict__ code8, int *__restrict__ esc_ptr,
+                                                      double *__restrict__ esc_val)
+{
+    const int b = blockIdx.x, t = threadIdx.x;
+    const long long s = (long long)b * kPackedTile;
+    if (col_base[b] < 0 || s + kPackedTile > (long long)nnz) {
+        if (t < 4)
+            esc_ptr[4 * b + t] = ~esc_ptr[4 * b + t];
+        return;
+    }
+    const uint2 w = *reinterpret_cast<const uint2 *>(code8 + s + (t >> 6) * (64 * kPackedVpt) + (t & 63) * kPackedVpt);
+    unsigned code[kPackedVpt];
+#pragma unroll
+    for (int k = 0; k < 4; ++k)
+        code[k] = (w.x >> (8 * k)) & 0xffu, code[k + 4] = (w.y >> (8 * k)) & 0xffu;
+    int before, total;
+    escape_places(code, &before, &total);
+    const int start = esc_ptr[4 * b + (t >> 6)];
+    int at = start + before;
+#pragma unroll
+    for (int k = 0; k < kPackedVpt; ++k)
+        if (code[k] == (unsigned)smvp::kEscapeCode)
+            esc_val[at++] = val[s + smvp::tile_lane_entry(t, k, kPackedVpt)];
+    if ((t & 63) == 0 && (total & 1))
+        esc_val[start + total] = 0.0;
+}
+
 }
 
 namespace smvp {
+
+int build_packed_values(const double *d_val, int nnz, const int *d_col_base, unsigned char **d_code8, double **d_hot, int **d_esc_ptr,
+                        double **d_esc_val, long long *doubles_read, long long *esc_slots, long long max_doubles, hipStream_t st)
+{
+    *d_code8 = nullptr, *d_hot = nullptr, *d_esc_ptr = nullptr, *d_esc_val = nullptr;
+    *doubles_read = nnz, *esc_slots = 0;
+    if (nnz <= 0)
+        return fail(SMVP_ERR_INVALID, "build_packed_values: no entries");
+    const int ntiles = (int)(((long long)nnz + kPackedTile - 1) / kPackedTile);
+    Scratch sc;
+    const int stride = (int)(((long long)nnz + kPackedSampleMax - 1) / kPackedSampleMax);
+    const int n = (int)(((long long)nnz + stride - 1) / stride);
+    u64 *k0, *k1;
+    unsigned *i0, *i1;
+    HIP_TRY(sc.get(&k0, (size_t)n));
+    HIP_TRY(sc.get(&k1, (size_t)n));
+    HIP_TRY(sc.get(&i0, (size_t)n));
+    HIP_TRY(sc.get(&i1, (size_t)n));
+    hipLaunchKernelGGL(sample_value_bits, dim3(blocks_for(n)), dim3(256), 0, st, d_val, nnz, stride, n, k0, i0);
+    HIP_TRY(hipGetLastError());
+    {
+        size_t tmp_bytes = 0;
+        HIP_TRY(prim::radix_sort_pairs(nullptr, tmp_bytes, k0, k1, i0, i1, (size_t)n, 0u, 64u, st));
+        char *tmp;
+        HIP_TRY(sc.get(&tmp, tmp_bytes));
+        HIP_TRY(prim::radix_sort_pairs(tmp, tmp_bytes, k0, k1, i0, i1, (size_t)n, 0u, 64u, st));
+    }
+    std::vector<u64> sorted((size_t)n);
+    HIP_TRY(hipMemcpyAsync(sorted.data(), k1, sizeof(u64) * (size_t)n, hipMemcpyDeviceToHost, st));
+    HIP_TRY(hipStreamSynchronize(st));
+    std::vector<std::pair<int, u64>> runs;
+    for (size_t i = 0; i < sorted.size();) {
+        size_t j = i + 1;
+        while (j < sorted.size() && sorted[j] == sorted[i])
+            ++j;
+        runs.push_back({(int)(j - i), sorted[i]});
+        i = j;
+    }
+    const size_t nhot = std::min<size_t>(runs.size(), (size_t)kHotValues);
+    std::partial_sort(runs.begin(), runs.begin() + (std::ptrdiff_t)nhot, runs.end(),
+                      [](const std::pair<int, u64> &a, const std::pair<int, u64> &b) { return a.first != b.first ? a.first > b.first : a.second < b.second; });
+    u64 hot_bits[kHotValues] = {};
+    for (size_t i = 0; i < nhot; ++i)
+        hot_bits[i] = runs[i].second;
+    std::sort(hot_bits, hot_bits + nhot);
+
+    unsigned char *code8 = nullptr;
+    double *hot = nullptr, *esc_val = nullptr;
+    int *esc_ptr = nullptr;
+    auto release = [&]() {
+        for (void *p : {(void *)code8, (void *)hot, (void *)esc_ptr, (void *)esc_val})
+            if (p)
+                (void)hipFree(p);
+    };
+    if (hipMalloc((void **)&code8, (size_t)nnz + 8) != hipSuccess || hipMalloc((void **)&hot, sizeof hot_bits) != hipSuccess ||
+        hipMalloc((void **)&esc_ptr, ((size_t)4 * ntiles + 4) * sizeof(int)) != hipSuccess) {
+        (void)hipGetLastError();
+        release();
+        return fail(SMVP_ERR_ALLOC, "cannot allocate the packed values (%d entries)", nnz);
+    }
+    int rc = SMVP_OK;
+    auto tried = [&](hipError_t e, const char *what) {
+        if (e != hipSuccess && rc == SMVP_OK)
+            rc = fail(SMVP_ERR_HIP, "build_packed_values: %s failed: %s", what, hipGetErrorString(e));
+        return rc == SMVP_OK;
+    };
+    u64 *count = nullptr;
+    u64 h_count = 0;
+    int h_slots = 0;
+    char *scan_tmp = nullptr;
+    size_t scan_bytes = 0;
+    (void)prim::exclusive_scan(nullptr, scan_bytes, esc_ptr, esc_ptr, 0, (size_t)4 * ntiles + 1, st);
+    if (tried(sc.get(&count, 1), "hipMalloc") && tried(sc.get(&scan_tmp, scan_bytes), "hipMalloc") &&
+        tried(hipMemcpyAsync(hot, hot_bits, sizeof hot_bits, hipMemcpyHostToDevice, st), "hipMemcpyAsync") &&
+        tried(hipMemsetAsync(count, 0, sizeof(u64), st), "hipMemsetAsync") &&
+        tried(hipMemsetAsync(esc_ptr + (size_t)4 * ntiles, 0, sizeof(int), st), "hipMemsetAsync")) {
+        hipLaunchKernelGGL(packed_codes, dim3((unsigned)ntiles), dim3(256), 0, st, d_val, nnz, d_col_base, reinterpret_cast<const u64 *>(hot),
+                           (int)nhot, code8, esc_ptr, count);
+        if (tried(hipGetLastError(), "packed_codes") &&
+            tried(prim::exclusive_scan(scan_tmp, scan_bytes, esc_ptr, esc_ptr, 0, (size_t)4 * ntiles + 1, st), "exclusive_scan") &&
+            tried(hipMemcpyAsync(&h_slots, esc_ptr + (size_t)4 * ntiles, sizeof(int), hipMemcpyDeviceToHost, st), "hipMemcpyAsync") &&
+            tried(hipMemcpyAsync(&h_count, count, sizeof(u64), hipMemcpyDeviceToHost, st), "hipMemcpyAsync"))
+            (void)tried(hipStreamSynchronize(st), "hipStreamSynchronize");
+    }
+    if (rc == SMVP_OK && max_doubles >= 0 && (long long)h_count > max_doubles) {
+        release();
+        *doubles_read = (long long)h_count;
+        return SMVP_OK;
+    }
+    if (rc == SMVP_OK) {
+        if (hipMalloc((void **)&esc_val, ((size_t)h_slots + 4) * sizeof(double)) != hipSuccess) {
+            (void)hipGetLastError();
+            rc = fail(SMVP_ERR_ALLOC, "cannot allocate the packed values' escapes (%d values)", h_slots);
+        } else if (tried(hipMemsetAsync(esc_val + h_slots, 0, 4 * sizeof(double), st), "hipMemsetAsync")) {
+            hipLaunchKernelGGL(packed_escapes, dim3((unsigned)ntiles), dim3(256), 0, st, d_val, nnz, d_col_base, code8, esc_ptr, esc_val);
+            if (tried(hipGetLastError(), "packed_escapes"))
+                (void)tried(hipStreamSynchronize(st), "hipStreamSynchronize");
+        }
+    }
+    if (rc != SMVP_OK) {
+        release();
+        return rc;
+    }
+    *d_code8 = code8, *d_hot = hot, *d_esc_ptr = esc_ptr, *d_esc_val = esc_val;
+    *doubles_read = (long long)h_count, *esc_slots = h_slots;
+    return SMVP_OK;
+}
 
 int build_column_offsets(const int *d_col_ind, int nnz, int tile, int *d_col_base, unsigned short *d_col16, int *fits,
                          hipStream_t st)
diff --git a/smvp-toolkit_amd/csrc/smvp_engine.hip b/smvp-toolkit_amd/csrc/smvp_engine.hip
--- a/smvp-toolkit_amd/csrc/smvp_engine.hip
+++ b/smvp-toolkit_amd/csrc/smvp_engine.hip
@@ -46,6 +46,11 @@
     int runs_total = 0;
     int sweep_alternate = 1, sweep_backward = 0;
     int read_once = 0;
+    unsigned char *d_code8 = nullptr;
+    double *d_hot = nullptr, *d_esc_val = nullptr;
+    int *d_esc_ptr = nullptr;
+    long long packed_doubles = 0, esc_slots = 0;
+    int packed_bounded = 0;
 };
 
 struct SweepPlan {
@@ -109,7 +114,8 @@
     for (void *q : {(void *)p->d_tile_row, (void *)p->d_tile_next, (void *)p->d_col16, (void *)p->d_col_base, (void *)p->d_row_rel,
                     (void *)p->d_carry_row, (void *)p->d_carry, (void *)p->d_pos_sorted, (void *)p->d_meta, (void *)p->d_ovf_ptr,
                     (void *)p->d_ovf_k, (void *)p->d_ovf_val, (void *)p->d_cache_ptr, (void *)p->d_val_cache, (void *)p->d_group_run,
-                    (void *)p->d_word32, (void *)p->d_run_ptr, (void *)p->d_run_tab})
+                    (void *)p->d_word32, (void *)p->d_run_ptr, (void *)p->d_run_tab, (void *)p->d_code8, (void *)p->d_hot, (void *)p->d_esc_ptr,
+                    (void *)p->d_esc_val})
         if (q)
             (void)hipFree(q);
     *p = TilePlan{};
@@ -143,8 +149,9 @@
 }
 
 inline bool tile_ordered(int flavor) { return flavor == smvp::kFlavorTjdsS || flavor == smvp::kFlavorTjdsH; }
+inline bool stream_family(int k) { return k == SMVP_CSR_KERNEL_STREAM || k == SMVP_CSR_KERNEL_STREAM_PACKED; }
 inline bool runs_on_tile_plan(int k) { return k != SMVP_CSR_KERNEL_VECTOR && k != SMVP_CSR_KERNEL_COLSWEEP && k != SMVP_CSR_KERNEL_BINNED; }
-inline int owner_flavor(const smvp_csr *h) { return h->tile.d_col16 ? smvp::kFlavorCsr16 : h->flavor; }
+inline int owner_flavor(const smvp_csr *h) { return h->tile.d_code8 ? smvp::kFlavorCsr16P : h->tile.d_col16 ? smvp::kFlavorCsr16 : h->flavor; }
 inline double csr_matrix_bytes(const smvp_csr *h) { return 12.0 * h->nnz + 4.0 * (h->rows + 1.0); }
 inline int sweep_strip_rows(const SweepPlan &s) { return (s.parts == smvp::kSweepXcdParts ? s.rb : s.rb * s.parts) / smvp::kSweepWaves; }
 
@@ -322,7 +329,7 @@
 
 int try_column_offsets(smvp_csr *h)
 {
-    if (h->flavor != smvp::kFlavorCsr || h->kernel != SMVP_CSR_KERNEL_STREAM || h->vpt < 4 || h->nnz <= 0 ||
+    if (h->flavor != smvp::kFlavorCsr || !stream_family(h->kernel) || h->vpt < 4 || h->nnz <= 0 ||
         smvp::option("csr_col16", 1) == 0)
         return SMVP_OK;
     std::vector<int> tiles;
@@ -358,10 +365,24 @@
 
 constexpr double kReadOnceMinBytes = 1024.0 * 1024 * 1024;
 
-int build_tile_plan_parts(smvp_csr *h)
+constexpr double kPackedMaxEscapeShare = 0.55;
+
+inline double tile_product_bytes(const smvp_csr *h) { return 12.0 * (double)h->nnz + 12.0 * h->rows + 8.0 * h->cols; }
+
+int attach_packed_values(smvp_csr *h, bool bounded)
+{
+    TilePlan &t = h->tile;
+    if (!t.d_col16 || h->vpt * smvp::kStreamBlock != smvp::kCol16LaneOrderTile)
+        return smvp::fail(SMVP_ERR_UNSUPPORTED, "the packed values need 2048-entry tiles whose columns fit 16-bit offsets: this matrix's do not");
+    return smvp::build_packed_values(h->d_val, h->nnz, t.d_col_base, &t.d_code8, &t.d_hot, &t.d_esc_ptr, &t.d_esc_val, &t.packed_doubles,
+                                     &t.esc_slots, bounded ? (long long)(kPackedMaxEscapeShare * (double)h->nnz) : -1ll, nullptr);
+}
+
+int build_tile_plan_parts(smvp_csr *h, bool packed_bounded)
 {
     TilePlan &t = h->tile;
     free_tile_plan(&t);
+    t.packed_bounded = packed_bounded;
     if (int rc = try_column_offsets(h))
         return rc;
     const int tile = smvp::kStreamBlock * h->vpt;
@@ -384,7 +405,7 @@
         tile_next[(size_t)b] = rp[tile_row[(size_t)b + 1]];
     if (int rc = upload(&t.d_tile_row, tile_row))
         return rc;
-    if (h->kernel == SMVP_CSR_KERNEL_STREAM) {
+    if (stream_family(h->kernel)) {
         if (int rc = upload(&t.d_tile_next, tile_next))
             return rc;
         if (h->rows > 0 && smvp::option("csr_rowrel", 1) != 0) {
@@ -405,10 +426,13 @@
     }
     t.ntiles = ntiles;
     const int alternate = smvp::option("csr_sweep_alternate", -1);
-    const double product_bytes = 12.0 * (double)h->nnz + 12.0 * h->rows + 8.0 * h->cols;
+    const double product_bytes = tile_product_bytes(h);
     t.sweep_alternate = alternate < 0 ? product_bytes > kSweepAlternateMinBytes : alternate != 0;
     const int read_once = smvp::option("csr_read_once", -1);
     t.read_once = h->flavor != smvp::kFlavorCsr ? 0 : read_once < 0 ? product_bytes > kReadOnceMinBytes : read_once != 0;
+    if (h->kernel == SMVP_CSR_KERNEL_STREAM_PACKED)
+        if (int rc = attach_packed_values(h, t.packed_bounded != 0))
+            return rc;
     if (tile_ordered(h->flavor)) {
         std::vector<int> ovf_ptr((size_t)ntiles + 1, 0);
         for (int b = 0; b < ntiles; ++b) {
@@ -443,9 +467,9 @@
     return SMVP_OK;
 }
 
-int build_tile_plan(smvp_csr *h)
-{
-    const int rc = build_tile_plan_parts(h);
+int build_tile_plan(smvp_csr *h, bool packed_bounded = false)
+{
+    const int rc = build_tile_plan_parts(h, packed_bounded);
     if (rc != SMVP_OK)
         free_tile_plan(&h->tile);
     return rc;
@@ -472,6 +496,8 @@
     if (kernel == SMVP_CSR_KERNEL_STREAM && param != 0 && param != 256 && param != 1024 && param != 2048)
         return false;
     if (kernel == SMVP_CSR_KERNEL_STREAM_CARRY && param != 0 && param != 1024 && param != 2048)
+        return false;
+    if (kernel == SMVP_CSR_KERNEL_STREAM_PACKED && param != 0 && param != smvp::kCol16LaneOrderTile)
         return false;
     if (kernel == SMVP_CSR_KERNEL_COLSWEEP && !sweep_param_ok(param))
         return false;
@@ -483,6 +509,8 @@
     if (kernel == SMVP_CSR_KERNEL_VECTOR) {
         h->lanes_per_row = param > 0 ? param : pow2_at_least(mean);
     } else {
+        if (kernel == SMVP_CSR_KERNEL_STREAM_PACKED)
+            param = smvp::kCol16LaneOrderTile;
         int tile = param > 0 ? param : 0;
         h->tile_chosen = param > 0;
         if (tile == 0) {
@@ -495,6 +523,29 @@
     return true;
 }
 
+int auto_packed_values(smvp_csr *h)
+{
+    const int wanted = smvp::option("csr_packed", -1);
+    if (wanted == 0 || h->flavor != smvp::kFlavorCsr || h->plain_only || h->nnz <= 0)
+        return SMVP_OK;
+    const bool tiles_suit = h->tile.d_col16 && h->vpt * smvp::kStreamBlock == smvp::kCol16LaneOrderTile;
+    if (wanted < 0 && !(tiles_suit && tile_product_bytes(h) > kReadOnceMinBytes))
+        return SMVP_OK;
+    if (tiles_suit) {
+        if (attach_packed_values(h, true) == SMVP_OK && h->tile.d_code8)
+            h->kernel = SMVP_CSR_KERNEL_STREAM_PACKED;
+        else
+            (void)hipGetLastError();
+        return SMVP_OK;
+    }
+    choose_csr_kernel(h, SMVP_CSR_KERNEL_STREAM_PACKED, 0);
+    if (build_tile_plan(h, true) == SMVP_OK && h->tile.d_code8)
+        return SMVP_OK;
+    (void)hipGetLastError();
+    choose_csr_kernel(h, SMVP_CSR_KERNEL_STREAM, 0);
+    return build_tile_plan(h);
+}
+
 }
 
 static int csr_create_impl(smvp_csr_t **out, int device, int rows, int cols, int nnz, const int *row_ptr, const int *col_ind, const double *val,
@@ -526,7 +577,7 @@
 static int plan_csr(smvp_csr *h, int kernel, int param, bool silent_fallback)
 {
     if (!choose_csr_kernel(h, kernel, param))
-        return smvp::fail(SMVP_ERR_INVALID, "entries per tile must be 256 (stream only), 1024 or 2048 for the kernel "
+        return smvp::fail(SMVP_ERR_INVALID, "entries per tile must be 256 (stream only), 1024 or 2048 (stream-packed: 2048) for the kernel "
                                             "this matrix resolves to (column sweep: 256 ... 20480 rows per block, a multiple of 4; binned: the near band, >= 0)");
     const double t0 = wall_ms();
     free_sweep_plan(&h->sweep);
@@ -534,6 +585,15 @@
     int rc = SMVP_OK;
     if (runs_on_tile_plan(h->kernel)) {
         rc = build_tile_plan(h);
+        if (rc == SMVP_OK && kernel == SMVP_CSR_KERNEL_AUTO && h->kernel == SMVP_CSR_KERNEL_STREAM)
+            rc = auto_packed_values(h);
+        if (rc != SMVP_OK && h->kernel == SMVP_CSR_KERNEL_STREAM_PACKED) {
+            const std::string why = smvp_last_error();
+            (void)hipGetLastError();
+            choose_csr_kernel(h, SMVP_CSR_KERNEL_STREAM, 0);
+            const int tile_rc = build_tile_plan(h);
+            rc = silent_fallback ? tile_rc : smvp::fail(rc, "%s", why.c_str());
+        }
     } else {
         free_tile_plan(&h->tile);
         if (h->kernel != SMVP_CSR_KERNEL_VECTOR)
@@ -680,7 +740,7 @@
         return smvp::fail(SMVP_ERR_INVALID, "null handle");
     if (h->flavor != smvp::kFlavorCsr && kernel != SMVP_CSR_KERNEL_STREAM)
         return smvp::fail(SMVP_ERR_UNSUPPORTED, "this matrix flavour runs on the stream kernel only");
-    if (kernel < SMVP_CSR_KERNEL_AUTO || kernel > SMVP_CSR_KERNEL_BINNED)
+    if (kernel < SMVP_CSR_KERNEL_AUTO || kernel > SMVP_CSR_KERNEL_STREAM_PACKED)
         return smvp::fail(SMVP_ERR_INVALID, "unknown CSR kernel %d", kernel);
     if (kernel == SMVP_CSR_KERNEL_VECTOR && param != 0 &&
         (param < 2 || param > 64 || (param & (param - 1)) != 0))
@@ -731,6 +791,7 @@
     l.stamps = stamps;
     l.rows = h->rows, l.nnz = h->nnz, l.ntiles = h->tile.ntiles;
     l.col16 = h->tile.d_col16, l.col_base = h->tile.d_col_base;
+    l.code8 = h->tile.d_code8, l.hot = h->tile.d_hot, l.esc_ptr = h->tile.d_esc_ptr, l.esc_val = h->tile.d_esc_val;
     l.row_rel = h->tile.d_row_rel;
     l.read_once = h->tile.read_once;
     l.unit_x = h->src.unit_operand ? 1 : 0;
@@ -807,7 +868,7 @@
                                       sweep_strip_rows(h->sweep), h->sweep.parts, h->sweep.per_launch, h->sweep.g, h->sweep.d_part, st);
     else if (h->kernel == SMVP_CSR_KERNEL_VECTOR)
         e = smvp::launch_csr_vector(h->lanes_per_row, h->d_row_ptr, h->d_col_ind, h->d_val, d_x, d_y, h->rows, st);
-    else if (h->kernel == SMVP_CSR_KERNEL_STREAM) {
+    else if (stream_family(h->kernel)) {
         smvp::OwnerLaunch l{};
         if (int rc = fill_owner_launch(h, d_x, d_y, stamps, &l))
             return rc;
@@ -963,7 +1024,7 @@
 
 int smvp::csr_stamp_slots(const smvp_csr_t *h)
 {
-    return h && h->kernel == SMVP_CSR_KERNEL_STREAM && h->tile.d_tile_row ? smvp::owner_stamp_slots(h->tile.ntiles, h->flavor) : 0;
+    return h && stream_family(h->kernel) && h->tile.d_tile_row ? smvp::owner_stamp_slots(h->tile.ntiles, h->flavor) : 0;
 }
 
 std::string smvp::csr_owner_kernel_name(const smvp_csr_t *h)
@@ -993,7 +1054,7 @@
                 snprintf(kernel_name, cap, "csr_colsweep<%d>", h->sweep.g);
         else if (h->kernel == SMVP_CSR_KERNEL_VECTOR)
             snprintf(kernel_name, cap, "csr_vector_rows<%d>", h->lanes_per_row);
-        else if (h->kernel == SMVP_CSR_KERNEL_STREAM)
+        else if (stream_family(h->kernel))
             snprintf(kernel_name, cap, "%s", smvp::csr_owner_kernel_name(h).c_str());
         else
             snprintf(kernel_name, cap, "csr_stream_tiles<%d>", h->vpt);
@@ -1043,6 +1104,8 @@
         b += 2.0 * n + 4.0 * (n / 1024 + 1);
     if (h->tile.d_row_rel)
         b += 2.0 * h->rows;
+    if (h->tile.d_code8)
+        b += 1.0 * n + 8.0 * smvp::kHotValues + 4.0 * (4.0 * t + 1) + 8.0 * (double)h->tile.esc_slots;
     if (tile_ordered(h->flavor)) {
         b += 4.0 * (t + 1) + 12.0 * h->tile.ovf_total + 4.0 * (t + 2) + 8.0 * h->tile.cached_total;
         b += h->flavor == smvp::kFlavorTjdsH ? 4.0 * n + 4.0 * (t + 2) + 8.0 * h->tile.runs_total + 2.0 * (n / 32 + 1) : 8.0 * n;
diff --git a/smvp-toolkit_amd/csrc/smvp_error.cpp b/smvp-toolkit_amd/csrc/smvp_error.cpp
--- a/smvp-toolkit_amd/csrc/smvp_error.cpp
+++ b/smvp-toolkit_amd/csrc/smvp_error.cpp
@@ -34,6 +34,7 @@
     {"csr_col16", {-1}},
     {"csr_rowrel", {-1}},
     {"csr_read_once", {-1}},
+    {"csr_packed", {-1}},
     {"csr_sweep_alternate", {-1}},
     {"binned_near", {-1}},
     {"binned_overlap", {-1}},
diff --git a/smvp-toolkit_amd/csrc/smvp_kernels.h b/smvp-toolkit_amd/csrc/smvp_kernels.h
--- a/smvp-toolkit_amd/csrc/smvp_kernels.h
+++ b/smvp-toolkit_amd/csrc/smvp_kernels.h
@@ -58,6 +58,7 @@
 constexpr int kFlavorTjdsS = 3;
 constexpr int kFlavorTjdsH = 4;
 constexpr int kFlavorCsr16 = 5;
+constexpr int kFlavorCsr16P = 6;
 constexpr int kSlotBits = 11;
 
 struct OwnerLaunch {
@@ -74,6 +75,10 @@
     const double *val_cache = nullptr;
     const unsigned short *col16 = nullptr;
     const int *col_base = nullptr;
+    const unsigned char *code8 = nullptr;
+    const double *hot = nullptr;
+    const int *esc_ptr = nullptr;
+    const double *esc_val = nullptr;
     const unsigned short *group_run = nullptr;
     const unsigned *word32 = nullptr;
     int unit_x = 0;
diff --git a/smvp-toolkit_amd/csrc/smvp_owner.hip b/smvp-toolkit_amd/csrc/smvp_owner.hip
--- a/smvp-toolkit_amd/csrc/smvp_owner.hip
+++ b/smvp-toolkit_amd/csrc/smvp_owner.hip
@@ -172,8 +172,9 @@
     }
 #ifdef SMVP_PHASE_STAMPS
     SMVP_OWNER_CSR_FORMS(SMVP_OWNER)
+    SMVP_OWNER_CSR_PACKED_FORMS(SMVP_OWNER)
 #else
-    if (flavor == kFlavorCsr || flavor == kFlavorCsr16)
+    if (flavor == kFlavorCsr || flavor == kFlavorCsr16 || flavor == kFlavorCsr16P)
         return launch_owner_csr(vpt, flavor, l, ex, grid.x, group, stream);
 #endif
     SMVP_OWNER_TJDS_FORMS(SMVP_OWNER)
diff --git a/smvp-toolkit_amd/csrc/smvp_owner_csr.hip b/smvp-toolkit_amd/csrc/smvp_owner_csr.hip
--- a/smvp-toolkit_amd/csrc/smvp_owner_csr.hip
+++ b/smvp-toolkit_amd/csrc/smvp_owner_csr.hip
@@ -23,8 +23,10 @@
 #define SMVP_OWNER_PLAIN(V, F) SMVP_OWNER(csr_stream_owner, V, F)
     if (l.read_once) {
         SMVP_OWNER_CSR_WIDE_FORMS(SMVP_OWNER_ONCE)
+        SMVP_OWNER_CSR_PACKED_FORMS(SMVP_OWNER_ONCE)
     }
     SMVP_OWNER_CSR_FORMS(SMVP_OWNER_PLAIN)
+    SMVP_OWNER_CSR_PACKED_FORMS(SMVP_OWNER_PLAIN)
 #undef SMVP_OWNER_PLAIN
 #undef SMVP_OWNER_ONCE
 #undef SMVP_OWNER
diff --git a/smvp-toolkit_amd/csrc/smvp_owner_kernel.h b/smvp-toolkit_amd/csrc/smvp_owner_kernel.h
--- a/smvp-toolkit_amd/csrc/smvp_owner_kernel.h
+++ b/smvp-toolkit_amd/csrc/smvp_owner_kernel.h
@@ -37,7 +37,20 @@
     ex.unit_x = l.unit_x, ex.word32 = l.word32, ex.group_run = l.group_run, ex.run_ptr = l.run_ptr, ex.run_tab = l.run_tab;
     ex.row_rel = l.row_rel;
     ex.stamps = stamps;
+    if (l.code8)
+        ex.pos = reinterpret_cast<const int *>(l.code8), ex.ovf_ptr = l.esc_ptr, ex.ovf_val = l.esc_val, ex.val_cache = l.hot;
     return ex;
+}
+
+struct PackedArrays {
+    const unsigned char *__restrict__ code8;
+    const int *__restrict__ esc_ptr;
+    const double *__restrict__ esc_val;
+    const double *__restrict__ hot;
+};
+__device__ __forceinline__ PackedArrays packed_arrays_of(const OwnerExtra &ex)
+{
+    return {reinterpret_cast<const unsigned char *>(ex.pos), ex.ovf_ptr, ex.ovf_val, ex.val_cache};
 }
 
 struct OwnerArgs {
@@ -54,7 +67,7 @@
 template <int FLAVOR>
 __device__ __forceinline__ double owner_product_slow(const OwnerArgs &a, long long j)
 {
-    if constexpr (FLAVOR == kFlavorCsr || FLAVOR == kFlavorCsr16)
+    if constexpr (FLAVOR == kFlavorCsr || FLAVOR == kFlavorCsr16 || FLAVOR == kFlavorCsr16P)
         return a.val[j] * a.x[a.col_ind[j]];
     else if constexpr (FLAVOR == kFlavorTjdsK)
         return a.val[a.pos[j]] * a.x[a.col_ind[j]];
@@ -103,8 +116,10 @@
     const OwnerArgs a = {col_ind, val, x, ex.pos, ex.start_pos, ex.ovf_val, ex.ovf_k, FLAVOR == kFlavorTjdsH ? ex.unit_x : 0};
     constexpr int TILE = kStreamBlock * VPT;
     constexpr int QCAP = (TILE + kStreamOver) / kLongRow + 1;
-    constexpr bool CSR = FLAVOR == kFlavorCsr || FLAVOR == kFlavorCsr16;
-    constexpr bool COL16 = FLAVOR == kFlavorCsr16;
+    constexpr bool PACKED = FLAVOR == kFlavorCsr16P;
+    static_assert(!PACKED || VPT == 8, "the packed values are laid out for 2048-entry tiles");
+    constexpr bool CSR = FLAVOR == kFlavorCsr || FLAVOR == kFlavorCsr16 || PACKED;
+    constexpr bool COL16 = FLAVOR == kFlavorCsr16 || PACKED;
     constexpr bool HALF = FLAVOR == kFlavorTjdsH;
     constexpr bool TJDS = FLAVOR == kFlavorTjdsK || FLAVOR == kFlavorTjdsS || HALF;
     constexpr bool SORTED = FLAVOR == kFlavorTjdsS || HALF;
@@ -150,6 +165,11 @@
     double v[VPT];
     const bool full_tile = s + TILE <= (long long)nnz;
     int grp[HALF ? VPT : 1];
+    [[maybe_unused]] bool packed_tile = false;
+    [[maybe_unused]] unsigned code_lo = 0, code_hi = 0;
+    [[maybe_unused]] int esc_at = 0, esc_end = 0;
+    [[maybe_unused]] double hot = 0.0;
+    [[maybe_unused]] double2v ev[PACKED ? 4 : 1];
     int run0 = 0;
     int2 run_tbl = make_int2(0, 0);
     if constexpr (HALF) {
@@ -195,6 +215,29 @@
                 for (int k = 0; k < VPT; k += 2)
                     *reinterpret_cast<int2 *>(&c[k]) = *reinterpret_cast<const int2 *>(a.col_ind + s + lane_entry(k));
             };
+            if constexpr (PACKED) {
+                const PackedArrays pk = packed_arrays_of(ex);
+                const int wv = __builtin_amdgcn_readfirstlane(t >> 6);
+                esc_at = pk.esc_ptr[4 * b + wv];
+                const int esc_next = pk.esc_ptr[4 * b + wv + 1];
+                esc_end = esc_next < 0 ? ~esc_next : esc_next;
+                packed_tile = esc_at >= 0;
+                if (packed_tile) {
+                    const int2v *mine = reinterpret_cast<const int2v *>(pk.code8 + s + ((t >> 6) * (64 * VPT) + (t & 63) * VPT));
+                    const int2v cw = STREAMED ? __builtin_nontemporal_load(mine) : *mine;
+                    code_lo = (unsigned)cw.x, code_hi = (unsigned)cw.y;
+                    hot = pk.hot[t & 63];
+#pragma unroll
+                    for (int i = 0; i < 4; ++i) {
+                        const int at = esc_at + 2 * (t & 63) + 128 * i;
+                        ev[i] = double2v{0.0, 0.0};
+                        if (at < esc_end) {
+                            const double2v *src = reinterpret_cast<const double2v *>(pk.esc_val + at);
+                            ev[i] = STREAMED ? __builtin_nontemporal_load(src) : *src;
+                        }
+                    }
+                }
+            }
             if constexpr (COL16) {
                 const int base = ex.col_base[b];
                 if (base >= 0) {
@@ -227,12 +270,14 @@
                     *reinterpret_cast<int2v *>(&pj[k]) = __builtin_nontemporal_load(reinterpret_cast<const int2v *>(a.pos + s + lane_entry(k)));
             }
             if constexpr (CSR) {
-#pragma unroll
-                for (int k = 0; k < VPT; k += 2) {
-                    if constexpr (STREAMED)
-                        *reinterpret_cast<double2v *>(&v[k]) = __builtin_nontemporal_load(reinterpret_cast<const double2v *>(a.val + s + lane_entry(k)));
-                    else
-                        *reinterpret_cast<double2 *>(&v[k]) = *reinterpret_cast<const double2 *>(a.val + s + lane_entry(k));
+                if (!PACKED || !packed_tile) {
+#pragma unroll
+                    for (int k = 0; k < VPT; k += 2) {
+                        if constexpr (STREAMED)
+                            *reinterpret_cast<double2v *>(&v[k]) = __builtin_nontemporal_load(reinterpret_cast<const double2v *>(a.val + s + lane_entry(k)));
+                        else
+                            *reinterpret_cast<double2 *>(&v[k]) = *reinterpret_cast<const double2 *>(a.val + s + lane_entry(k));
+                    }
                 }
             }
         } else {
@@ -386,6 +431,39 @@
         for (int k = 0; k < VPT; ++k)
             xk[k] = a.x[c[k]];
         const double xo = over0 ? a.x[co] : 0.0;
+        if constexpr (PACKED) {
+            if (packed_tile) {
+                double *part = prod + (t >> 6) * (64 * VPT);
+#pragma unroll
+                for (int i = 0; i < 4; ++i)
+                    *reinterpret_cast<double2v *>(&part[2 * (t & 63) + 128 * i]) = ev[i];
+                __builtin_amdgcn_fence(__ATOMIC_RELEASE, "wavefront");
+                __builtin_amdgcn_wave_barrier();
+                __builtin_amdgcn_fence(__ATOMIC_ACQUIRE, "wavefront");
+                unsigned code[VPT];
+                int before = 0;
+#pragma unroll
+                for (int k = 0; k < VPT; ++k) {
+                    code[k] = ((k < 4 ? code_lo : code_hi) >> (8 * (k & 3))) & 0xffu;
+                    const unsigned long long mask = __ballot(code[k] == (unsigned)kEscapeCode);
+                    before = (int)__builtin_amdgcn_mbcnt_hi((unsigned)(mask >> 32), __builtin_amdgcn_mbcnt_lo((unsigned)mask, (unsigned)before));
+                }
+                const int hot_lo = __double2loint(hot), hot_hi = __double2hiint(hot);
+                int mine = 0;
+#pragma unroll
+                for (int k = 0; k < VPT; ++k) {
+                    const bool escaped = code[k] == (unsigned)kEscapeCode;
+                    const int from = (int)(code[k] & 63u) << 2;
+                    const double hot_k = __hiloint2double(__builtin_amdgcn_ds_bpermute(from, hot_hi), __builtin_amdgcn_ds_bpermute(from, hot_lo));
+                    const double esc_k = part[(before + mine) & (64 * VPT - 1)];
+                    v[k] = escaped ? esc_k : hot_k;
+                    mine += escaped ? 1 : 0;
+                }
+                __builtin_amdgcn_fence(__ATOMIC_RELEASE, "wavefront");
+                __builtin_amdgcn_wave_barrier();
+                __builtin_amdgcn_fence(__ATOMIC_ACQUIRE, "wavefront");
+            }
+        }
 #pragma unroll
         for (int k = 0; k < VPT; ++k)
             p[k] = v[k] * xk[k];
@@ -530,6 +608,7 @@
 
 #define SMVP_OWNER_CSR_WIDE_FORMS(X) X(4, kFlavorCsr) X(8, kFlavorCsr) X(4, kFlavorCsr16) X(8, kFlavorCsr16)
 #define SMVP_OWNER_CSR_FORMS(X) X(1, kFlavorCsr) SMVP_OWNER_CSR_WIDE_FORMS(X)
+#define SMVP_OWNER_CSR_PACKED_FORMS(X) X(8, kFlavorCsr16P)
 #define SMVP_OWNER_TJDS_TILE_FORMS(X) \
     X(1, kFlavorTjdsS) X(4, kFlavorTjdsS) X(8, kFlavorTjdsS) X(1, kFlavorTjdsH) X(4, kFlavorTjdsH) X(8, kFlavorTjdsH)
 #define SMVP_OWNER_TJDS_FORMS(X) X(1, kFlavorTjdsK) X(4, kFlavorTjdsK) X(8, kFlavorTjdsK) SMVP_OWNER_TJDS_TILE_FORMS(X)
diff --git a/smvp-toolkit_amd/csrc/smvp_tile_map.h b/smvp-toolkit_amd/csrc/smvp_tile_map.h
--- a/smvp-toolkit_amd/csrc/smvp_tile_map.h
+++ b/smvp-toolkit_amd/csrc/smvp_tile_map.h
@@ -40,4 +40,7 @@
     return w * chunk + l * vpt + k;
 }
 
+constexpr int kHotValues = 64;
+constexpr int kEscapeCode = 255;
+
 }
diff --git a/smvp-toolkit_amd/python/smvp_toolkit_amd/__init__.py b/smvp-toolkit_amd/python/smvp_toolkit_amd/__init__.py
--- a/smvp-toolkit_amd/python/smvp_toolkit_amd/__init__.py
+++ b/smvp-toolkit_amd/python/smvp_toolkit_amd/__init__.py
@@ -14,6 +14,7 @@
 MM_COULD_NOT_READ_FILE, MM_PREMATURE_EOF, MM_NOT_MTX, MM_NO_HEADER, MM_UNSUPPORTED_TYPE = 11, 12, 13, 14, 15
 CSR_KERNEL_AUTO, CSR_KERNEL_VECTOR, CSR_KERNEL_STREAM, CSR_KERNEL_STREAM_CARRY, CSR_KERNEL_COLSWEEP = 0, 1, 2, 3, 4
 CSR_KERNEL_BINNED = 5
+CSR_KERNEL_STREAM_PACKED = 6
 MEM_HOST, MEM_DEVICE = 0, 1
 SYNTH_MEMPLUS_SHAPED, SYNTH_UNIFORM = 1, 2
 TJDS_MODE_AUTO, TJDS_MODE_ATOMIC, TJDS_MODE_TWO_PHASE, TJDS_MODE_ROW_GATHER = 0, 1, 2, 3
```

Result: faster. 1038 GFLOP/s, median of 6 (+10.0%).
